# kahrendt/microWakeWord

Measured on AMD Instinct MI355X. Metric: spectrogram-windows/sec (train step) on default mixednet, higher is better.
Workload: dtype f32

## Files before the change

microwakeword_amd/csrc/block_engine.hip:

```cpp
#define MWW_BLOCK_TU 1
#include <cstring>

#include "engine.hip.h"
#include "block_launch.hip.h"
#include "kernels_bnre.hip.h"

#ifndef MWW_CONV1_X6_DEFAULT
#define MWW_CONV1_X6_DEFAULT 1
#endif
#ifndef MWW_CONV1_X6_FWD_DEFAULT
#define MWW_CONV1_X6_FWD_DEFAULT 0
#endif
#ifndef MWW_BWD_FIRST_WIDE_DEFAULT
#define MWW_BWD_FIRST_WIDE_DEFAULT 0
#endif
#ifndef MWW_BWD_WIDE_DEFAULT
#define MWW_BWD_WIDE_DEFAULT 1
#endif
#ifndef MWW_DP_COMMIT_LATE_BLOCK_DEFAULT
#define MWW_DP_COMMIT_LATE_BLOCK_DEFAULT 1
#endif
#ifndef MWW_DP_COMMIT_LATE_LAST_DEFAULT
#define MWW_DP_COMMIT_LATE_LAST_DEFAULT 0
#endif
#ifndef MWW_DP_COMMIT_LATE_FIRST_DEFAULT
#define MWW_DP_COMMIT_LATE_FIRST_DEFAULT 1
#endif

namespace mww {

__global__ void bn_fwd_finalize_kernel(BnFwdFinalizeArgs a);
__global__ void bn_eval_prepare_kernel(BnEvalPrepareArgs a);
__global__ void bn_bwd_finalize_kernel(BnBwdFinalizeArgs a);

namespace {

float* bn_slot(Layer& l, int i) { return l.bn + (size_t)i * l.cout; }
float b_inv_n(const Layer& l, int B) { return 1.0f / ((float)B * (float)l.tout); }
bool b_handover(const mww_ctx* c) { return c->bn_inline && !(c->hook && c->sync_bn); }

struct BlockModel : Model {
  mww_mixednet_desc d;
  std::vector<Layer> L;
  int64_t o_conv1 = 0;
  int grid_fwd = 0, grid_bwd = 0;
  float* a0 = nullptr;
  float* gbuf[2] = {nullptr, nullptr};
  bool conv1_x6 = MWW_CONV1_X6_DEFAULT != 0;
  bool conv1_x6_fwd = MWW_CONV1_X6_FWD_DEFAULT != 0;
  bool bwd_first_wide = MWW_BWD_FIRST_WIDE_DEFAULT != 0;
  bool bwd_wide = MWW_BWD_WIDE_DEFAULT != 0;
  int dp_commit_late = -1;
  bool pw_bf16 = false;
  bool st_bf16 = false;
  int ablate = 0;
  unsigned long long* phase_clk = nullptr;

  ~BlockModel() override {
    for (Layer& l : L) {
      if (gbuf[0] || gbuf[1]) l.g = nullptr;
      tensor_free(&l);
    }
    void* own[] = {gbuf[0], gbuf[1], a0, phase_clk};
    for (void* p : own) if (p) (void)hipFree(p);
  }
  int layout(mww_ctx* c) override;
  int alloc(mww_ctx* c, std::vector<BnSlots>* bn) override;
  int enqueue_forward(mww_ctx* c, int B, bool training, bool update_moving, bool loss, bool metrics) override;
  int enqueue_backward(mww_ctx* c, int B, bool fuse_adam) override;
  int enqueue_bn_collect(mww_ctx* c, int B) override;
  std::vector<int> stat_widths() const override {
    std::vector<int> w;
    for (const Layer& l : L) w.push_back(l.cout);
    return w;
  }
  bool lazy_ok(const mww_ctx*, int B) const override {
    const int per_fwd = (B + std::min(B, grid_fwd) - 1) / std::min(B, grid_fwd);
    const int per_bwd = (B + std::min(B, grid_bwd) - 1) / std::min(B, grid_bwd);
    return per_fwd <= kXMaxSamples && per_bwd <= kXMaxSamples;
  }
  unsigned replay_key(bool* handover) const override { *handover = true; return 0; }
  bool eval_fold_cached() const override { return true; }
  int debug_tensor(mww_ctx* c, const char* name, int B, DebugTensor* t) override;
  int set_option(mww_ctx* c, const OptionRow& o, int64_t v) override;

  int launch_fwd_first(mww_ctx* c, int k1, int c1, int cout, int k, int st, const FwdFirstArgs& a, int grid);
  int launch_bwd_first(mww_ctx* c, int k1, int c1, int cout, int k, int st, const BwdFirstArgs& a, int grid);
  int launch_fwd_block(mww_ctx* c, int cin, int cout, int k, const FwdBlockArgs& a, int grid);
  int launch_bwd_block(mww_ctx* c, int cin, int cout, int k, bool last, const BwdBlockArgs& a, int grid);
  int fwd_block_grid(const mww_ctx* c, const Layer& l, int B);
  void block_segments(int gbwd, int b0, int b1, GradReduceArgs* ga);
};

int BlockModel::launch_fwd_first(mww_ctx* c, int k1, int c1, int cout, int k, int st, const FwdFirstArgs& a, int grid) {
  if (k_launch_fwd_first(c->stream, st_bf16 ? 2 : (pw_bf16 ? 1 : 0), k1, c1, cout, k, st, a, grid, conv1_x6_fwd)) return MWW_OK;
  return fail(MWW_ERR_UNSUPPORTED, "no first-block kernel for this (conv1 kernel, filters, pointwise, depthwise) shape");
}

int BlockModel::launch_bwd_first(mww_ctx* c, int k1, int c1, int cout, int k, int st, const BwdFirstArgs& a, int grid) {
  const bool late = dp_commit_late < 0 ? MWW_DP_COMMIT_LATE_FIRST_DEFAULT != 0 : dp_commit_late != 0;
  if (bwd_wide && !pw_bf16 && !st_bf16 && k_launch_bwd_firstw(c->stream, k1, c1, cout, k, st, a, grid, conv1_x6 && bwd_first_wide, late)) return MWW_OK;
  if (k_launch_bwd_first(c->stream, st_bf16 ? 2 : (pw_bf16 ? 1 : 0), k1, c1, cout, k, st, a, grid, conv1_x6, late)) return MWW_OK;
  return fail(MWW_ERR_UNSUPPORTED, "no first-block backward kernel for this shape");
}

int BlockModel::launch_fwd_block(mww_ctx* c, int cin, int cout, int k, const FwdBlockArgs& a, int grid) {
  if (k_launch_fwd_block(c->stream, st_bf16 ? 2 : (pw_bf16 ? 1 : 0), cin, cout, k, a, grid)) return MWW_OK;
  return fail(MWW_ERR_UNSUPPORTED, "no block kernel for this (cin, cout, depthwise) shape");
}

int BlockModel::launch_bwd_block(mww_ctx* c, int cin, int cout, int k, bool last, const BwdBlockArgs& a, int grid) {
  const int mode = st_bf16 ? 2 : (pw_bf16 ? 1 : 0);
  const bool late = dp_commit_late < 0 ? (last ? MWW_DP_COMMIT_LATE_LAST_DEFAULT : MWW_DP_COMMIT_LATE_BLOCK_DEFAULT) != 0 : dp_commit_late != 0;
  if (bwd_wide && k_launch_bwd_blockw(c->stream, mode, cin, cout, k, last, a, grid, late)) return MWW_OK;
  if (k_launch_bwd_block(c->stream, st_bf16 ? 2 : (pw_bf16 ? 1 : 0), cin, cout, k, last, a, grid)) return MWW_OK;
  return fail(MWW_ERR_UNSUPPORTED, "no block backward kernel for this shape");
}

}

bool shape_supported(const mww_mixednet_desc& d, std::string* why, bool bf16) {
  if (d.n_blocks < 2 || d.n_blocks > MWW_MAX_BLOCKS) { *why = "the block kernels serve 2.." + std::to_string(MWW_MAX_BLOCKS) + " blocks"; return false; }
  bool ok = false;
#define X(K1, C1, CO, K, S) ok = ok || (d.conv1_kernel == K1 && d.conv1_filters == C1 && d.block_filters[0] == CO && d.block_kernel[0] == K && d.conv1_stride == S);
  if (bf16) { MWW_FIRST_SHAPES_BF16(X) } else { MWW_FIRST_SHAPES(X) }
#undef X
  if (!ok) { *why = "first block (conv1 kernel/filters/stride, pointwise filters, depthwise kernel) not instantiated"; return false; }
  for (int i = 1; i < d.n_blocks; ++i) {
    ok = false;
#define X(CI, CO, K) ok = ok || (d.block_filters[i - 1] == CI && d.block_filters[i] == CO && d.block_kernel[i] == K);
    if (bf16) { MWW_BLOCK_SHAPES_BF16(X) } else { MWW_BLOCK_SHAPES(X) }
#undef X
    if (!ok) { *why = "block " + std::to_string(i) + " (cin, cout, depthwise kernel) not instantiated"; return false; }
  }
  const int cl = d.block_filters[d.n_blocks - 1];
  if (cl != 32 && cl != 48 && cl != 64) { *why = "head kernel needs 32, 48 or 64 channels"; return false; }
  int t = d.frames >= d.conv1_kernel && d.conv1_stride > 0 ? (d.frames - d.conv1_kernel) / d.conv1_stride + 1 : 0;
  for (int i = 0; i < d.n_blocks; ++i) t -= d.block_kernel[i] - 1;
  if (t > head_frame_limit(cl)) {
    *why = "head kernel holds at most " + std::to_string(head_frame_limit(cl)) + " final frames at " + std::to_string(cl) + " channels (" + std::to_string(t) + " here)";
    return false;
  }
  return true;
}

namespace {

int BlockModel::fwd_block_grid(const mww_ctx* c, const Layer& l, int B) {
  const int per_cu = l.cin > 48 ? 2 : (l.k > 13 ? 3 : 4);
  const long long items = (long long)B * ((l.tout + TT - 1) / TT);
  return (int)std::min<long long>(items, std::min(grid_fwd, c->n_cu * per_cu));
}

int BlockModel::enqueue_forward(mww_ctx* c, int B, bool training, bool update_moving, bool loss, bool metrics) {
  Launcher lp{c};
  const int nb = d.n_blocks;
  if (!training && !c->bn_eval_ready) {
    for (int i = 0; i < nb; ++i) {
      Layer& l = L[i];
      BnEvalPrepareArgs a{fwd_params(c) + l.o_gamma, fwd_params(c) + l.o_beta, eval_bn_state(c) + l.o_mm, eval_bn_state(c) + l.o_mv,
                          bn_slot(l, BN_SCALE), bn_slot(l, BN_SHIFT), l.cout};
      lp.begin("bn_eval_prepare", i);
      hipLaunchKernelGGL(bn_eval_prepare_kernel, dim3(1), dim3(64), 0, c->stream, a);
      lp.end();
    }
  }
  const bool inl = training && b_handover(c);
  auto fold_of = [&](Layer& pl) {
    BnFoldArgs f;
    memset(&f, 0, sizeof(f));
    if (!inl) return f;
    f.acc = fwd_rows(c, pl).acc;
    f.inv_n = b_inv_n(pl, B);
    f.update_moving = update_moving ? 1 : 0;
    f.gamma = fwd_params(c) + pl.o_gamma;
    f.beta = fwd_params(c) + pl.o_beta;
    f.moving_mean = c->bn_state + pl.o_mm;
    f.moving_var = c->bn_state + pl.o_mv;
    f.scale = bn_slot(pl, BN_SCALE);
    f.shift = bn_slot(pl, BN_SHIFT);
    f.mean = bn_slot(pl, BN_MEAN);
    f.rstd = bn_slot(pl, BN_RSTD);
    return f;
  };
  for (int i = 0; i < nb; ++i) {
    Layer& l = L[i];
    const int grid = i == 0 ? std::min(B, grid_fwd) : fwd_block_grid(c, l, B);
    const StatAcc sacc = inl ? fwd_rows(c, l) : StatAcc{nullptr, nullptr};
    if (i == 0) {
      FwdFirstArgs a{c->x, fwd_params(c) + o_conv1, fwd_params(c) + l.o_dw_w, fwd_params(c) + l.o_dw_b, fwd_params(c) + l.o_pw_w,
                     l.p, l.stat_part, B, d.frames, l.tout, 0, sacc, x_gather(c), training ? a0 : nullptr};
      lp.begin("fwd_block", i);
      int rc = launch_fwd_first(c, d.conv1_kernel, d.conv1_filters, l.cout, l.k, d.conv1_stride, a, grid);
      lp.end();
      if (rc) return rc;
    } else {
      Layer& pl = L[i - 1];
      FwdBlockArgs a{pl.p, bn_slot(pl, BN_SCALE), bn_slot(pl, BN_SHIFT), fwd_params(c) + l.o_dw_w, fwd_params(c) + l.o_dw_b,
                     fwd_params(c) + l.o_pw_w, l.p, l.stat_part, B, l.tin, l.tout, ablate, phase_clk + (size_t)(2 * i) * 2048 * kClkSlots,
                     sacc, fold_of(pl)};
      lp.begin("fwd_block", i);
      int rc = launch_fwd_block(c, l.cin, l.cout, l.k, a, grid);
      lp.end();
      if (rc) return rc;
    }
    if (training && !inl) {
      StatSource ss;
      int rcs = exchange_stats(c, lp, "bn_stat_exchange", i, l.stat_part, grid, l.cout, 0, b_inv_n(l, B), &ss);
      if (rcs) return rcs;
      BnFwdFinalizeArgs f{ss.part, ss.G, l.cout, ss.inv_n, fwd_params(c) + l.o_gamma,
                          fwd_params(c) + l.o_beta, c->bn_state + l.o_mm, c->bn_state + l.o_mv, bn_slot(l, BN_SCALE),
                          bn_slot(l, BN_SHIFT), bn_slot(l, BN_MEAN), bn_slot(l, BN_RSTD), update_moving ? 1 : 0};
      lp.begin("bn_fwd_finalize", i);
      hipLaunchKernelGGL(bn_fwd_finalize_kernel, dim3(l.cout), dim3(kThreads), 0, c->stream, f);
      lp.end();
    }
  }
  Layer& ll = L[nb - 1];
  const BnFoldArgs hfold = fold_of(ll);
  if (inl) c->fpar ^= 1;
  const bool tail_late = loss && inl && c->tail_roles;
  const StatAcc hgacc = tail_late ? bwd_rows(c, ll) : StatAcc{nullptr, nullptr};
  int rc = enqueue_block_head(c, B, ll, ll.tout, ll.cout, st_bf16, hfold, hgacc, loss, metrics);
  if (rc) return rc;
  c->tail_src = DenseSource{ll.p, bn_slot(ll, BN_SCALE), bn_slot(ll, BN_SHIFT), nullptr, nullptr, nullptr, nullptr, 0, 0, st_bf16 ? 1 : 0};
  if (tail_late) {
    c->tail_in_reduce = true;
    c->tail_metrics = metrics;
    return MWW_OK;
  }
  if (loss && !(c->hook && c->sync_bn)) {
    c->tail_pending = true;
    c->tail_metrics = metrics;
    return MWW_OK;
  }
  return enqueue_side_work(c, B, metrics, loss, c->tail_src);
}

int BlockModel::enqueue_bn_collect(mww_ctx* c, int B) {
  const bool inl = b_handover(c);
  std::vector<BnreRow> rows(L.size());
  memset(rows.data(), 0, rows.size() * sizeof(BnreRow));
  for (size_t i = 0; i < L.size(); ++i) {
    Layer& l = L[i];
    BnreRow& r = rows[i];
    const float inv_n = b_inv_n(l, B);
    r.C = l.cout;
    r.groups = 1;
    r.o_mm = (int)l.o_mm;
    r.o_mv = (int)l.o_mv;
    if (inl) {
      r.form = BNRE_ROWS;
      r.acc[0] = l.facc[0];
      r.acc[1] = l.facc[1];
      r.inv_n = inv_n;
    } else {
      const int grid = i == 0 ? std::min(B, grid_fwd) : fwd_block_grid(c, l, B);
      const StatSource ss = forward_stat_source(c, (int)i, l.stat_part, grid, l.cout, inv_n);
      r.form = BNRE_PART_BLOCK;
      r.part = ss.part;
      r.G = ss.G;
      r.inv_n = ss.inv_n;
    }
  }
  return enqueue_bnre_collect(c, rows);
}

void BlockModel::block_segments(int gbwd, int b0, int b1, GradReduceArgs* ga) {
  memset(ga, 0, sizeof(*ga));
  for (int i = b0; i < b1; ++i) {
    Layer& l = L[i];
    GradSegment s;
    s.part = l.grad_part;
    s.G = gbwd;
    s.stride = l.grad_part_stride;
    s.n = l.grad_part_stride;
    s.dst = (int)(i == 0 ? o_conv1 : l.o_dw_w);
    ga->seg[ga->nseg++] = s;
  }
}

int BlockModel::enqueue_backward(mww_ctx* c, int B, bool fuse_adam) {
  Launcher lp{c};
  const int nb = d.n_blocks;
  const int gbwd = std::min(B, grid_bwd);
  const int ghead = std::min(B, c->grid_head);
  const bool inl = b_handover(c);
  const int split = nb >= 3 ? nb - 2 : 0;
  const bool bucketed = fuse_adam && c->hook && c->reduce_grads && !c->sync_bn && inl && c->tail_in_reduce && c->grad_buckets == 2 && split > 0;
  for (int i = nb - 1; i >= 0; --i) {
    Layer& l = L[i];
    const bool last = (i == nb - 1);
    const bool fold_here = inl && (!last || c->tail_in_reduce);
    StatSource ss{nullptr, 0, 0.f, 1.0f};
    if (!fold_here) {
      int rcs = exchange_stats(c, lp, "bn_gstat_exchange", i, l.gstat_part, last ? ghead : gbwd, l.cout, 1, b_inv_n(l, B), &ss);
      if (rcs) return rcs;
    }
    BnBwdFinalizeArgs f{ss.part, ss.G, l.cout, ss.inv_n,
                        fwd_params(c) + l.o_gamma, bn_slot(l, BN_RSTD), bn_slot(l, BN_C1), bn_slot(l, BN_MG),
                        bn_slot(l, BN_MGX), c->grads + l.o_gamma, c->grads + l.o_beta, ss.dscale};
    BnGradFoldArgs gf;
    memset(&gf, 0, sizeof(gf));
    if (fold_here) {
      gf.acc = bwd_rows(c, l).acc;
      gf.inv_n = b_inv_n(l, B);
      gf.dscale = 1.0f;
      gf.gamma = fwd_params(c) + l.o_gamma;
      gf.c1 = bn_slot(l, BN_C1);
      gf.mg = bn_slot(l, BN_MG);
      gf.mgx = bn_slot(l, BN_MGX);
      gf.dgamma = c->grads + l.o_gamma;
      gf.dbeta = c->grads + l.o_beta;
    }
    if (fold_here) {
    } else if (last && c->tail_pending) {
      c->tail_pending = false;
      int rch = enqueue_head_tail(c, B, f);
      if (rch) return rch;
    } else {
      lp.begin("bn_bwd_finalize", i);
      hipLaunchKernelGGL(bn_bwd_finalize_kernel, dim3(l.cout), dim3(kThreads), 0, c->stream, f);
      lp.end();
    }
    if (i > 0) {
      Layer& pl = L[i - 1];
      BwdBlockArgs a;
      a.in = pl.p;
      a.in_scale = bn_slot(pl, BN_SCALE);
      a.in_shift = bn_slot(pl, BN_SHIFT);
      a.in_mean = bn_slot(pl, BN_MEAN);
      a.in_rstd = bn_slot(pl, BN_RSTD);
      a.pk = l.p;
      a.gk = l.g;
      a.k_mean = bn_slot(l, BN_MEAN);
      a.k_rstd = bn_slot(l, BN_RSTD);
      a.k_c1 = bn_slot(l, BN_C1);
      a.k_mg = bn_slot(l, BN_MG);
      a.k_mgx = bn_slot(l, BN_MGX);
      a.k_scale = bn_slot(l, BN_SCALE);
      a.k_shift = bn_slot(l, BN_SHIFT);
      a.wd = fwd_params(c) + c->o_dense_w;
      a.dz = c->dz;
      a.dw_w = fwd_params(c) + l.o_dw_w;
      a.dw_b = fwd_params(c) + l.o_dw_b;
      a.pw_w = fwd_params(c) + l.o_pw_w;
      a.g_out = pl.g;
      a.gstat_part = pl.gstat_part;
      a.grad_part = l.grad_part;
      a.B = B;
      a.Tin = l.tin;
      a.Tout = l.tout;
      a.ablate = ablate;
      a.phase_clk = phase_clk + (size_t)(2 * i + 1) * 2048 * kClkSlots;
      a.gacc = inl ? bwd_rows(c, pl) : StatAcc{nullptr, nullptr};
      a.gfold = gf;
      lp.begin("bwd_block", i);
      int rc = launch_bwd_block(c, l.cin, l.cout, l.k, last, a, gbwd);
      lp.end();
      if (rc) return rc;
      if (bucketed && i == split) {
        GradReduceArgs gb;
        block_segments(gbwd, split, nb, &gb);
        rc = enqueue_grad_assembly(c, B, gb, fuse_adam, l.o_dw_w, c->P, false);
        if (rc) return rc;
      }
    } else {
      if (last) return fail(MWW_ERR_UNSUPPORTED, "single-block models are not supported");
      BwdFirstArgs a{c->x, a0, l.p, l.g, bn_slot(l, BN_MEAN), bn_slot(l, BN_RSTD), bn_slot(l, BN_C1),
                     bn_slot(l, BN_MG), bn_slot(l, BN_MGX), fwd_params(c) + l.o_dw_w, fwd_params(c) + l.o_dw_b,
                     fwd_params(c) + l.o_pw_w, l.grad_part, B, d.frames, l.tout, gf, x_gather(c), ablate,
                     phase_clk + (size_t)(2 * i + 1) * 2048 * kClkSlots};
      lp.begin("bwd_block", i);
      int rc = launch_bwd_first(c, d.conv1_kernel, d.conv1_filters, l.cout, l.k, d.conv1_stride, a, gbwd);
      lp.end();
      if (rc) return rc;
    }
  }
  if (inl) c->gpar ^= 1;
  GradReduceArgs ga;
  block_segments(gbwd, 0, bucketed ? split : nb, &ga);
  return enqueue_grad_assembly(c, B, ga, fuse_adam, 0, bucketed ? L[split].o_dw_w : c->P, true);
}

int BlockModel::layout(mww_ctx* c) {
  int64_t off = 0, soff = 0;
  o_conv1 = off;
  off += (int64_t)d.conv1_kernel * MWW_FEATURE_BINS * d.conv1_filters;
  int t = (d.frames - d.conv1_kernel) / d.conv1_stride + 1, ch = d.conv1_filters;
  L.resize(d.n_blocks);
  for (int i = 0; i < d.n_blocks; ++i) {
    Layer& l = L[i];
    l.cin = ch;
    l.cout = d.block_filters[i];
    l.k = d.block_kernel[i];
    l.tin = t;
    l.tout = t - (l.k - 1);
    if (l.tout <= 0) return fail(MWW_ERR_INVALID, "spectrogram too short for the kernel sizes");
    l.o_dw_w = off; off += (int64_t)l.k * l.cin;
    l.o_dw_b = off; off += l.cin;
    l.o_pw_w = off; off += (int64_t)l.cin * l.cout;
    l.o_gamma = off; off += l.cout;
    l.o_beta = off; off += l.cout;
    l.o_mm = soff; soff += l.cout;
    l.o_mv = soff; soff += l.cout;
    t = l.tout;
    ch = l.cout;
  }
  c->t_last = t;
  c->c_last = ch;
  c->o_dense_w = off; off += (int64_t)t * ch;
  c->o_dense_b = off; off += 1;
  c->P = off;
  c->S = soff;
  c->dwd_stride = t * ch + 4;
  grid_fwd = c->n_cu * 4;
  grid_bwd = c->n_cu * 2;
  bool wide64 = false;
  for (int i = 0; i < d.n_blocks; ++i) wide64 = wide64 || d.block_filters[i] > 48;
  if (wide64) {
    grid_fwd = c->n_cu * 2;
    grid_bwd = c->n_cu;
  }
  return MWW_OK;
}

int BlockModel::alloc(mww_ctx* c, std::vector<BnSlots>* bn) {
  const size_t mb = (size_t)d.max_batch;
  const int gmax_f = c->n_cu * 4, gmax_b = c->n_cu * 2;
  MWW_TRY(dev_alloc(&a0, mb * L[0].tin * d.conv1_filters));
#ifndef MWW_G_PINGPONG
#define MWW_G_PINGPONG 1
#endif
  if (MWW_G_PINGPONG) {
    size_t need[2] = {0, 0};
    for (int i = 0; i < d.n_blocks; ++i) need[i & 1] = std::max(need[i & 1], mb * L[i].tout * L[i].cout);
    for (int par = 0; par < 2; ++par)
      if (need[par]) MWW_TRY(dev_alloc(&gbuf[par], need[par]));
  }
  for (int i = 0; i < d.n_blocks; ++i) {
    Layer& l = L[i];
    MWW_TRY(dev_alloc(&l.p, mb * l.tout * l.cout));
    if (MWW_G_PINGPONG) l.g = gbuf[i & 1];
    else MWW_TRY(dev_alloc(&l.g, mb * l.tout * l.cout));
    l.grad_part_stride = (l.k + 1) * l.cin + l.cin * l.cout;
    if (i == 0) l.grad_part_stride += d.conv1_kernel * MWW_FEATURE_BINS * d.conv1_filters;
    MWW_TRY(tensor_alloc(&l, l.cout, gmax_f, std::max(gmax_b, c->n_cu * 4), (size_t)gmax_b * l.grad_part_stride));
    bn->push_back(BnSlots{l.o_gamma, l.o_beta, l.o_mv, l.cout});
  }
  MWW_TRY(dev_alloc(&phase_clk, (size_t)2 * MWW_MAX_BLOCKS * 2048 * kClkSlots));
  return MWW_OK;
}

int BlockModel::set_option(mww_ctx* c, const OptionRow& o, int64_t v) {
  if (o.owner != OPT_BLOCK) return MWW_OK;
  const std::string name = o.name;
  if (name == "pointwise_bf16" || name == "storage_bf16") {
    std::string why;
    if (v && !shape_supported(d, &why, true)) return fail(MWW_ERR_UNSUPPORTED, "no bf16 mode for this topology: " + why);
    if (name == "pointwise_bf16") { pw_bf16 = v != 0; if (!v) st_bf16 = false; }
    else { st_bf16 = v != 0; if (v) pw_bf16 = true; }
  }
  const std::pair<const char*, bool BlockModel::*> flags[] = {{"bwd_wide", &BlockModel::bwd_wide}, {"conv1_x6", &BlockModel::conv1_x6},
                                                              {"conv1_x6_fwd", &BlockModel::conv1_x6_fwd}, {"bwd_first_wide", &BlockModel::bwd_first_wide}};
  const std::pair<const char*, int BlockModel::*> ints[] = {{"ablate", &BlockModel::ablate}, {"dp_commit_late", &BlockModel::dp_commit_late},
                                                            {"grid_fwd", &BlockModel::grid_fwd}, {"grid_bwd", &BlockModel::grid_bwd}};
  for (auto& f : flags) if (name == f.first) this->*f.second = v != 0;
  for (auto& f : ints) if (name == f.first) this->*f.second = (int)v;
  return MWW_OK;
}

int BlockModel::debug_tensor(mww_ctx* c, const char* name, int B, DebugTensor* t) {
  const int nb = d.n_blocks;
  auto idx = [&](const char* prefix) -> int {
    const size_t pl = strlen(prefix);
    if (strncmp(name, prefix, pl) != 0) return -1;
    const int k = atoi(name + pl);
    return (k >= 1 && k <= nb && name[pl] >= '0' && name[pl] <= '9') ? k - 1 : -1;
  };
  int k;
  if ((k = idx("p")) >= 0 || (k = idx("g")) >= 0) {
    t->src = name[0] == 'p' ? L[k].p : L[k].g;
    t->n = (int64_t)B * L[k].tout * L[k].cout;
    t->bf16 = st_bf16;
  }
  else if ((k = idx("bn")) >= 0) { t->src = L[k].bn; t->n = (int64_t)9 * L[k].cout; }
  else if (!strcmp(name, "a0")) { t->src = a0; t->n = (int64_t)B * L[0].tin * d.conv1_filters; }
  else if (!strncmp(name, "clkf", 4) || !strncmp(name, "clkb", 4)) {
    const int kk = atoi(name + 4);
    if (kk < 1 || kk > nb) return fail(MWW_ERR_INVALID, "bad layer");
    t->src = reinterpret_cast<const float*>(phase_clk + (size_t)(2 * (kk - 1) + (name[3] == 'b' ? 1 : 0)) * 2048 * kClkSlots);
    t->n = 2048 * kClkSlots * 2;
  }
  else return 0;
  return 1;
}

}

int plan_mixednet(const mww_mixednet_desc& d, Model** out) {
  if (d.n_blocks < 2 || d.n_blocks > MWW_MAX_BLOCKS) return fail(MWW_ERR_INVALID, "n_blocks must be in [2, 8]");
  if (d.conv1_stride < 1 || d.frames < d.conv1_kernel) return fail(MWW_ERR_INVALID, "bad first-conv stride / kernel");
  if (d.conv1_filters <= 0) return fail(MWW_ERR_UNSUPPORTED, "first_conv_filters == 0 is not implemented");
  if (d.max_batch <= 0 || d.frames <= 0) return fail(MWW_ERR_INVALID, "frames and max_batch must be positive");
  std::string why;
  if (!shape_supported(d, &why)) return fail(MWW_ERR_UNSUPPORTED, why);
  BlockModel* m = new BlockModel();
  m->d = d;
  *out = m;
  return MWW_OK;
}

}
```

microwakeword_amd/csrc/bwd_first_body.inc:

```
  constexpr int CIN = C1;
  constexpr int CPI = pitch(CIN), CPO = pitch(COUT);
  constexpr int RA = TT + K - 1;
  constexpr int TAIL = S > 1 ? K - 1 : 0;
  constexpr int TAILK = (TAIL + 3) / 4 * 4;
  constexpr int XR = (TT + TAILK - 1) * S + K1;
  constexpr int NT1 = C1 / 16;
  constexpr int M1 = K1 * FBINS;
  constexpr int MT1 = (M1 + 15) / 16;
  constexpr int MPW = (MT1 + 3) / 4;
  constexpr int MT = CIN / 16, NT = COUT / 16, KSO = COUT / 4;
  constexpr int NCH = nchunks(CIN), L = chunk_len(CIN);
  constexpr int QI = CIN / 4;
  constexpr int RAP = halo_rows_padded(CIN, K), TTP = tile_rows_padded(CIN);
  constexpr int OFF_A = 0, OFF_DP = OFF_A + RAP * CPI, OFF_U = OFF_DP + TT * CPO, OFF_DU = OFF_U + TTP * CPI;
  constexpr int PB = 96, PLB = XR * PB, GPB = 2 * CIN, GPL = TT * GPB;
  static_assert(!X6 || (S == 1 && CIN == 32 && (K1 * FBINS) % 8 == 0 && 3 * GPL <= (TT * CPO + TTP * CPI) * 4 && TTP == TT), "the x6 form serves the stride-1 first convolutions");
  constexpr int OFF_G0 = OFF_DU + RAP * CPI, OFF_END = X6 ? OFF_G0 : OFF_G0 + (TTP + TAILK) * CPI;
  static_assert(TAIL <= NCH && TTP + TAIL <= RAP, "tail rows");
  constexpr int PX = FBINS + 1;
  static_assert(OFF_END >= 4 * CIN * COUT && OFF_END >= NCH * (K + 1) * CIN, "scratch aliasing");
  static_assert(TT >= K - 1, "shape");

  float* sA = smem + OFF_A;
  float* sDP = smem + OFF_DP;
  float* sU = smem + OFF_U;
  float* sDU = smem + OFF_DU;
  float* sG0 = smem + OFF_G0;

  const int tid = threadIdx.x, lane = tid & 63, wave = tid >> 6, r16 = lane & 15, g = lane >> 4;
  const int c = tid % CIN, chunk = tid / CIN;
  const bool dw_active = chunk < NCH;
  const int Ta = (a.T - K1) / S + 1;
  MWW_PC_DECL
  MWW_PC_AT(0);

  const bool tailmode = TAIL > 0 && Ta > TT && Ta <= TT + TAIL;
  const int ntiles = tailmode ? 1 : (Ta + TT - 1) / TT;
  const int nsamp = (int)blockIdx.x < a.B ? (a.B - (int)blockIdx.x + (int)gridDim.x - 1) / (int)gridDim.x : 0;
  const int nitems = nsamp * ntiles;
  XStage<XR, PX, MWW_AUX_LD_XB> xs;
  DpStage<COUT, false, SB> dps;
  constexpr int NA = (RA * QI + kThreads - 1) / kThreads;
  float4 pre_a[NA];
  auto issue_a = [&](int it, bool live) {
    const int s = live ? it / ntiles : nsamp - 1, b = blockIdx.x + s * gridDim.x, t0 = (it % ntiles) * TT;
    const int nrx = live ? ((tailmode ? Ta : min(TT, Ta - t0)) - 1) * S + K1 : 0;
    xs.issue(a.x, a.xg, sXg, s, b, a.T, t0 * S, nrx, tid);
    const BufRsrc ra = tile_rsrc(a.a0 + ((size_t)b * Ta + t0) * CIN, live ? min(RA, Ta - t0) * QI * 16 : 0);
#pragma unroll
    for (int j = 0; j < NA; ++j) pre_a[j] = tile_load4<MWW_AUX_LD_A0>(ra, (tid + j * kThreads) * 16);
  };
  auto issue_b = [&](int it, bool live) {
    const int b = blockIdx.x + (it / ntiles) * gridDim.x, t0 = (it % ntiles) * TT;
    const int nvk = live ? max(0, min(TT, a.Tout - t0)) * (COUT / 4) : 0;
    const size_t koff = ((size_t)b * a.Tout + t0) * COUT;
    dps.issue(elem_ptr<SB>(a.pk, koff), elem_ptr<SB>(a.gk, koff), nvk, tid);
  };
  int offm[MPW];
  bool okm[MPW];
  int xoff[MPW], goff[NT1];
  if constexpr (X6) {
    const int rowl = 4 * g + (r16 >> 2), cg = 4 * (r16 & 3);
#pragma unroll
    for (int mi = 0; mi < MPW; ++mi) {
      const int m = min((wave * MPW + mi) * 16 + cg, M1 - 4);
      xoff[mi] = (rowl + m / FBINS) * PB + (m % FBINS) * 2;
    }
#pragma unroll
    for (int nt = 0; nt < NT1; ++nt) goff[nt] = rowl * GPB + ((nt * 16 + cg) ^ ((rowl & 4) ? 16 : 0)) * 2;
  } else {
#pragma unroll
  for (int mi = 0; mi < MPW; ++mi) {
    const int m = (wave * MPW + mi) * 16 + r16;
    okm[mi] = m < M1;
    offm[mi] = okm[mi] ? (m / FBINS) * PX + (m % FBINS) : 0;
  }
  }
  if (a.xg.win) xgather_setup(a.xg, sXg, nsamp, tid);
  stagger_start<MWW_STAGGER_BWD>();
  if (nitems > 0) {
    issue_a(0, true);
    issue_b(0, true);
  }

  WeightStage<CIN, COUT, 0, pitch_wt(CIN, BF)> wst;
  wst.load(a.pw_w, nullptr, tid);
  float dww[K], accw[K];
  float accb = 0.f, dwb = 0.f;
#pragma unroll
  for (int i = 0; i < K; ++i) {
    dww[i] = dw_active ? a.dw_w[i * CIN + c] : 0.f;
    accw[i] = 0.f;
  }
  if (dw_active) dwb = a.dw_b[c];
  for (int i = tid; i < COUT; i += kThreads) {
    const float krs = a.k_rstd[i];
    const float kmean = a.k_mean[i];
    float c1, mg, mgx;
    if (a.gfold.acc) {
      bn_grad_fold_channel(a.gfold, COUT, i, krs, c1, mg, mgx);
    } else {
      c1 = a.k_c1[i];
      mg = a.k_mg[i];
      mgx = a.k_mgx[i];
    }
    const float kA = -c1 * krs * mgx;
    sKp[0 * COUT + i] = c1;
    sKp[1 * COUT + i] = kA;
    sKp[2 * COUT + i] = -c1 * mg - kA * kmean;
    sKp[5 * COUT + i] = 0.f;
    sKp[6 * COUT + i] = 0.f;
  }
  wst.store(sWt, nullptr, tid);
  for (int i = RA * CPI + tid; i < RAP * CPI; i += kThreads) {
    sA[i] = 0.f;
    sDU[i] = 0.f;
  }
  if constexpr (!X6)
    for (int i = TTP * CPI + tid; i < (TTP + TAILK) * CPI; i += kThreads) sG0[i] = 0.f;
#pragma unroll
  for (int i = 0; i < K; ++i) pin(dww[i]);
  pin(dwb);
  f32x4 dwacc[MT][NT];
#pragma unroll
  for (int mt = 0; mt < MT; ++mt)
#pragma unroll
    for (int nt = 0; nt < NT; ++nt) dwacc[mt][nt] = zero4();
  f32x4 w1acc[MPW][NT1];
#pragma unroll
  for (int mi = 0; mi < MPW; ++mi)
#pragma unroll
    for (int nt = 0; nt < NT1; ++nt) w1acc[mi][nt] = zero4();
  __syncthreads();

  MWW_PC_AT(1);
  MWW_PC_START(MWW_ABLATE(a, 16) && tid == 0);
  for (int it = 0; it < nitems; ++it) {
    rotate_priority(it, 2);
    const int t0 = (it % ntiles) * TT;
    const int nrows_new = max(0, min(TT, a.Tout - t0));
    const int rows_da = min(TT, Ta - t0);
    if constexpr (X6) xs.template commit_planes<PB, PLB>(reinterpret_cast<unsigned*>(sX), a.xg, sXg, it / ntiles, t0 * S, tid);
    else xs.commit(sX, a.xg, sXg, it / ntiles, t0 * S, tid);
#pragma unroll
    for (int j = 0; j < NA; ++j) {
      const int i = tid + j * kThreads;
      if (i < RA * QI) {
        const int r = i / QI, q = i - r * QI;
        *reinterpret_cast<float4*>(sA + r * CPI + q * 4) = pre_a[j];
      }
    }
    MWW_PC_MARK(0);
    if constexpr (!LATE) dps.commit(sDP, sKp, 0.f, nrows_new * (COUT / 4), tid);
    carry_du<K, CPI>(sDU, t0 == 0, tid);
    if constexpr (LATE) issue_a(it + 1, it + 1 < nitems);
    MWW_PC_MARK(LATE ? 0 : 8);
    __syncthreads();
    MWW_PC_MARK(1);
    if constexpr (!LATE) {
      if (it + 1 < nitems) {
        issue_a(it + 1, true);
        issue_b(it + 1, true);
      }
    }
    if (dw_active) {
      if (chunk * L < nrows_new) {
        float o[L];
        dw_chunk<K, L>(sA, CPI, chunk * L, c, dww, dwb, o);
#pragma unroll
        for (int t = 0; t < L; ++t) {
          const int tl = chunk * L + t;
          sU[tl * CPI + c] = (tl < nrows_new) ? o[t] : 0.f;
        }
      } else {
#pragma unroll
        for (int t = 0; t < L; ++t) sU[(chunk * L + t) * CPI + c] = 0.f;
      }
    }
    MWW_PC_MARK(2);
    if constexpr (LATE) {
      dps.commit(sDP, sKp, 0.f, nrows_new * (COUT / 4), tid);
      issue_b(it + 1, it + 1 < nitems);
      MWW_PC_MARK(8);
    }
    __syncthreads();
    MWW_PC_MARK(3);
    pointwise_backward_tile<CIN, COUT, K, BF>(sU, sDP, sDU, wave, r16, g, sWt, dwacc, wave * 16 < nrows_new);
    MWW_PC_MARK(4);
    __syncthreads();
    MWW_PC_MARK(5);
    if (dw_active) {
      float wdu[L + K - 1], wa[L + K - 1];
#pragma unroll
      for (int j = 0; j < L + K - 1; ++j) wdu[j] = sDU[(chunk * L + j) * CPI + c];
#pragma unroll
      for (int j = 0; j < L + K - 1; ++j) wa[j] = sA[(chunk * L + j) * CPI + c];
      lds_reads_first();
#pragma unroll
      for (int t = 0; t < L; ++t) {
        const int sl = chunk * L + t;
        float acc = 0.f;
#pragma unroll
        for (int i = 0; i < K; ++i) acc = fmaf(dww[K - 1 - i], wdu[t + i], acc);
        const float gv = (sl < rows_da && wa[t] > 0.f) ? acc : 0.f;
        if constexpr (X6) {
          unsigned h0, h1, h2;
          split3(gv, h0, h1, h2);
          unsigned short* gp = reinterpret_cast<unsigned short*>(sDP) + sl * CIN + (c ^ ((sl & 4) ? 16 : 0));
          gp[0] = (unsigned short)(h0 >> 16);
          gp[GPL / 2] = (unsigned short)(h1 >> 16);
          gp[GPL] = (unsigned short)(h2 >> 16);
        } else {
          sG0[sl * CPI + c] = gv;
        }
      }
      if (chunk * L < nrows_new) {
#pragma unroll
        for (int t = 0; t < L; ++t) {
          const float dut = wdu[K - 1 + t];
          accb += dut;
#pragma unroll
          for (int i = 0; i < K; ++i) accw[i] = fmaf(dut, wa[t + i], accw[i]);
        }
      }
      if constexpr (TAIL > 0) {
        if (tailmode && chunk < TAIL) {
          const int sl = TT + chunk;
          float acc = 0.f;
#pragma unroll
          for (int j = 0; j < K; ++j) acc = fmaf(dww[K - 1 - j], sl + j < RAP ? sDU[(sl + j) * CPI + c] : 0.f, acc);
          sG0[sl * CPI + c] = (sl < Ta && sA[sl * CPI + c] > 0.f) ? acc : 0.f;
        }
      }
    }
    MWW_PC_MARK(6);
    __syncthreads();
    if constexpr (X6) {
      const char* xb = reinterpret_cast<const char*>(sX);
      const char* gb = reinterpret_cast<const char*>(sDP);
#pragma unroll
      for (int kb = 0; kb < TT / 32; ++kb)
#pragma unroll
        for (int nt = 0; nt < NT1; ++nt) {
          u32x4v gq[3];
#pragma unroll
          for (int p = 0; p < 3; ++p) {
            const u32x2v lo = lds_read_tr16(gb + goff[nt] + p * GPL + (32 * kb) * GPB), hi = lds_read_tr16(gb + goff[nt] + p * GPL + (32 * kb + 16) * GPB);
            gq[p] = u32x4v{lo.x, lo.y, hi.x, hi.y};
          }
#pragma unroll
          for (int mi = 0; mi < MPW; ++mi) {
            u32x4v xq[3];
#pragma unroll
            for (int p = 0; p < 3; ++p) {
              const u32x2v lo = lds_read_tr16(xb + xoff[mi] + p * PLB + (32 * kb) * S * PB), hi = lds_read_tr16(xb + xoff[mi] + p * PLB + (32 * kb + 16) * S * PB);
              xq[p] = u32x4v{lo.x, lo.y, hi.x, hi.y};
            }
            w1acc[mi][nt] = mfma_x6(xq, gq, w1acc[mi][nt]);
          }
        }
    } else {
      float av[2][MPW], bv[2][NT1];
      auto load_w1 = [&](int kk, int sl) {
        const int s = kk * 4 + g;
#pragma unroll
        for (int nt = 0; nt < NT1; ++nt) bv[sl][nt] = sG0[s * CPI + nt * 16 + r16];
#pragma unroll
        for (int mi = 0; mi < MPW; ++mi) {
          const float v = sX[s * S * PX + offm[mi]];
          av[sl][mi] = okm[mi] ? v : 0.f;
        }
      };
      load_w1(0, 0);
#pragma unroll
      for (int kk = 0; kk < TT / 4; ++kk) {
        if (kk + 1 < TT / 4) load_w1(kk + 1, (kk + 1) & 1);
#pragma unroll
        for (int mi = 0; mi < MPW; ++mi)
#pragma unroll
          for (int nt = 0; nt < NT1; ++nt) w1acc[mi][nt] = mfma4(av[kk & 1][mi], bv[kk & 1][nt], w1acc[mi][nt]);
      }
      __builtin_amdgcn_sched_group_barrier(0x100, MPW + NT1, 0);
      sched_read_mfma_groups<TT / 4 - 1, MPW + NT1, MPW * NT1>();
      sched_read_mfma_groups<1, 0, MPW * NT1>();
      if constexpr (TAIL > 0) {
        if (tailmode) {
#pragma unroll
          for (int ks = 0; ks < TAILK / 4; ++ks) {
            load_w1(TT / 4 + ks, 0);
#pragma unroll
            for (int mi = 0; mi < MPW; ++mi)
#pragma unroll
              for (int nt = 0; nt < NT1; ++nt) w1acc[mi][nt] = mfma4(av[0][mi], bv[0][nt], w1acc[mi][nt]);
          }
        }
      }
    }
    MWW_PC_MARK(7);
    __syncthreads();
    MWW_PC_MARK(5);
  }
  MWW_PC_AT(2);
  float* gdst = a.grad_part + (size_t)blockIdx.x * (M1 * C1 + (K + 1) * CIN + CIN * COUT);
#pragma unroll
  for (int mi = 0; mi < MPW; ++mi)
#pragma unroll
    for (int nt = 0; nt < NT1; ++nt)
#pragma unroll
      for (int r = 0; r < 4; ++r) {
        const int m = (wave * MPW + mi) * 16 + g * 4 + r;
        if (m < M1) gdst[m * C1 + nt * 16 + r16] = w1acc[mi][nt][r];
      }
  write_block_grad_partials<CIN, COUT, K>(smem, gdst + M1 * C1, dwacc, accw, accb, dw_active, c, chunk, tid, wave, r16, g);
  MWW_PC_AT(3);
  MWW_PC_DUMP(a.phase_clk ? a.phase_clk + (size_t)blockIdx.x * kClkSlots : nullptr);
```

microwakeword_amd/csrc/common.hip.h:

```cpp
#pragma once
#include <hip/hip_runtime.h>
#include <stdint.h>

namespace mww {

typedef float f32x4 __attribute__((ext_vector_type(4)));

constexpr int kThreads = 256;
constexpr int TT = 64;
constexpr int FBINS = 40;
constexpr float kBnEps = 1e-3f;
constexpr float kBnMomentum = 0.99f;
constexpr float kKerasEps = 1e-7f;

constexpr int kHeadTraining = 1, kHeadClippedLoss = 2;
__device__ __forceinline__ float bce_value(float z, float pr, float yy, bool clipped_form) {
  if (!clipped_form) return fmaxf(z, 0.f) - z * yy + log1pf(expf(-fabsf(z)));
  const float pc = fminf(fmaxf(pr, kKerasEps), 1.0f - kKerasEps);
  return -(yy * logf(pc) + (1.0f - yy) * logf(1.0f - pc));
}
__device__ __forceinline__ float bce_dz(float pr, float yy, bool clipped_form) {
  if (clipped_form && ((pr < kKerasEps) || (pr > 1.0f - kKerasEps))) return 0.f;
  return pr - yy;
}

__device__ __forceinline__ f32x4 mfma4(float a, float b, f32x4 c) {
  return __builtin_amdgcn_mfma_f32_16x16x4f32(a, b, c, 0, 0, 0);
}

typedef __bf16 bf16x4 __attribute__((ext_vector_type(4)));
typedef short s16x4 __attribute__((ext_vector_type(4)));

__device__ __forceinline__ f32x4 mfma_bf16(bf16x4 a, bf16x4 b, f32x4 c) {
  return __builtin_amdgcn_mfma_f32_16x16x16bf16_1k(__builtin_bit_cast(s16x4, a), __builtin_bit_cast(s16x4, b), c, 0, 0, 0);
}

__device__ __forceinline__ bf16x4 to_bf16x4(float a, float b, float c, float d) {
  bf16x4 v = {(__bf16)a, (__bf16)b, (__bf16)c, (__bf16)d};
  return v;
}

typedef __bf16 bf16x8 __attribute__((ext_vector_type(8)));
typedef unsigned u32x4v __attribute__((ext_vector_type(4)));
typedef unsigned u32x2v __attribute__((ext_vector_type(2)));
__device__ __forceinline__ f32x4 mfma_bf16k32(u32x4v a, u32x4v b, f32x4 c) {
  return __builtin_amdgcn_mfma_f32_16x16x32_bf16(__builtin_bit_cast(bf16x8, a), __builtin_bit_cast(bf16x8, b), c, 0, 0, 0);
}
__device__ __forceinline__ void split3(float v, unsigned& h0, unsigned& h1, unsigned& h2) {
  h0 = __float_as_uint(v) & 0xffff0000u;
  const float r1 = v - __uint_as_float(h0);
  h1 = __float_as_uint(r1) & 0xffff0000u;
  const float r2 = r1 - __uint_as_float(h1);
  h2 = __float_as_uint(r2) & 0xffff0000u;
}
__device__ __forceinline__ unsigned pack_hi2(unsigned a, unsigned b) { return (a >> 16) | b; }
__device__ __forceinline__ void split3x8(const float (&v)[8], u32x4v (&q)[3]) {
  unsigned h[3][8];
#pragma unroll
  for (int e = 0; e < 8; ++e) split3(v[e], h[0][e], h[1][e], h[2][e]);
#pragma unroll
  for (int p = 0; p < 3; ++p)
#pragma unroll
    for (int d = 0; d < 4; ++d) q[p][d] = pack_hi2(h[p][2 * d], h[p][2 * d + 1]);
}
__device__ __forceinline__ f32x4 mfma_x6(const u32x4v (&xs)[3], const u32x4v (&ws)[3], f32x4 acc) {
  acc = mfma_bf16k32(xs[2], ws[0], acc);
  acc = mfma_bf16k32(xs[1], ws[1], acc);
  acc = mfma_bf16k32(xs[0], ws[2], acc);
  acc = mfma_bf16k32(xs[1], ws[0], acc);
  acc = mfma_bf16k32(xs[0], ws[1], acc);
  acc = mfma_bf16k32(xs[0], ws[0], acc);
  return acc;
}
__device__ __forceinline__ void pin4(u32x4v& v) { asm volatile("" : "+v"(v)); }
__device__ __forceinline__ u32x2v lds_read_tr16(const void* lds_ptr) {
  typedef short s16x4t __attribute__((ext_vector_type(4)));
  const s16x4t v = __builtin_amdgcn_ds_read_tr16_b64_v4i16((__attribute__((address_space(3))) s16x4t*)(lds_ptr));
  return __builtin_bit_cast(u32x2v, v);
}

__device__ __forceinline__ f32x4 zero4() {
  f32x4 z = {0.f, 0.f, 0.f, 0.f};
  return z;
}

__host__ __device__ constexpr int pitch(int c) { return c + 4; }
#ifndef MWW_FWD_PITCH_A
#define MWW_FWD_PITCH_A 1
#endif
#ifndef MWW_FWD_PITCH_U
#define MWW_FWD_PITCH_U 1
#endif
__host__ __device__ constexpr int pitch_fa(int c) { return (MWW_FWD_PITCH_A && c == 48) ? 48 : c + 4; }
__host__ __device__ constexpr int pitch_fu(int c, bool bf) { return (MWW_FWD_PITCH_U && !bf) ? c + 2 : c + 4; }

__host__ __device__ constexpr int pitch_wt(int c, bool bf) { return bf ? c + 4 : (c % 32 == 16 ? c : c + 16); }

__host__ __device__ constexpr int nchunks(int c) { return kThreads / c; }
__host__ __device__ constexpr int chunk_len(int c) { return (TT + nchunks(c) - 1) / nchunks(c); }
__host__ __device__ constexpr int tile_rows_padded(int c) { return nchunks(c) * chunk_len(c); }
__host__ __device__ constexpr int halo_rows_padded(int c, int k) { return tile_rows_padded(c) + k - 1; }

typedef __amdgpu_buffer_rsrc_t BufRsrc;
typedef unsigned u32x4 __attribute__((ext_vector_type(4)));
typedef unsigned u32x2 __attribute__((ext_vector_type(2)));

__device__ __forceinline__ BufRsrc tile_rsrc(const void* base, int bytes) {
  const int n = __builtin_amdgcn_readfirstlane(bytes > 0 ? bytes : 0);
  return __builtin_amdgcn_make_buffer_rsrc(const_cast<void*>(base), (short)0, n, 0x00020000);
}
#ifndef MWW_AUX_ST_P
#define MWW_AUX_ST_P 16
#endif
#ifndef MWW_AUX_ST_G
#define MWW_AUX_ST_G 16
#endif
#ifndef MWW_AUX_ST_A0
#define MWW_AUX_ST_A0 2
#endif
#ifndef MWW_AUX_LD_FP
#define MWW_AUX_LD_FP 0
#endif
#ifndef MWW_AUX_LD_BP
#define MWW_AUX_LD_BP 2
#endif
#ifndef MWW_AUX_LD_A0
#define MWW_AUX_LD_A0 2
#endif
#ifndef MWW_AUX_LD_PK
#define MWW_AUX_LD_PK 2
#endif
#ifndef MWW_AUX_LD_GK
#define MWW_AUX_LD_GK 2
#endif
#ifndef MWW_AUX_LD_XF
#define MWW_AUX_LD_XF 0
#endif
#ifndef MWW_AUX_LD_XB
#define MWW_AUX_LD_XB 0
#endif
#ifndef MWW_AUX_LD_HP
#define MWW_AUX_LD_HP 0
#endif
#ifndef MWW_AUX_ST_GP
#define MWW_AUX_ST_GP 1
#endif
#ifndef MWW_AUX_GR_ST_P
#define MWW_AUX_GR_ST_P 1
#endif
#ifndef MWW_AUX_GR_ST_G
#define MWW_AUX_GR_ST_G 0
#endif
#ifndef MWW_AUX_GR_LD_GOLD
#define MWW_AUX_GR_LD_GOLD 0
#endif
#ifndef MWW_AUX_GR_ST_GP
#define MWW_AUX_GR_ST_GP 0
#endif
#ifndef MWW_AUX_GR_LD_DP
#define MWW_AUX_GR_LD_DP 0
#endif
template <int WT>
__device__ __forceinline__ void store_stream(float* p, float v) {
  if constexpr (WT != 0) __hip_atomic_store(p, v, __ATOMIC_RELAXED, __HIP_MEMORY_SCOPE_AGENT);
  else *p = v;
}
template <int AUX = 0>
__device__ __forceinline__ float4 tile_load4(BufRsrc r, int byte_off) {
  const u32x4 v = __builtin_amdgcn_raw_buffer_load_b128(r, byte_off, 0, AUX);
  return make_float4(__uint_as_float(v.x), __uint_as_float(v.y), __uint_as_float(v.z), __uint_as_float(v.w));
}
template <int AUX = 0>
__device__ __forceinline__ uint2 tile_load2(BufRsrc r, int byte_off) {
  const u32x2 v = __builtin_amdgcn_raw_buffer_load_b64(r, byte_off, 0, AUX);
  uint2 o;
  o.x = v.x;
  o.y = v.y;
  return o;
}
template <int AUX = 0>
__device__ __forceinline__ float tile_load1(BufRsrc r, int byte_off) {
  return __uint_as_float(__builtin_amdgcn_raw_buffer_load_b32(r, byte_off, 0, AUX));
}
template <int AUX = 0>
__device__ __forceinline__ void tile_store1(BufRsrc r, int byte_off, float v) {
  __builtin_amdgcn_raw_buffer_store_b32(__float_as_uint(v), r, byte_off, 0, AUX);
}
template <bool SB, int AUX = 0>
__device__ __forceinline__ float4 tile_load4s(BufRsrc r, int group) {
  if constexpr (!SB) {
    return tile_load4<AUX>(r, group * 16);
  } else {
    const uint2 v = tile_load2<AUX>(r, group * 8);
    return make_float4(__uint_as_float(v.x << 16), __uint_as_float(v.x & 0xffff0000u), __uint_as_float(v.y << 16),
                       __uint_as_float(v.y & 0xffff0000u));
  }
}
template <bool SB, int AUX = 0>
__device__ __forceinline__ void tile_store1s(BufRsrc r, int elem, float v) {
  if constexpr (!SB) {
    tile_store1<AUX>(r, elem * 4, v);
  } else {
    const __bf16 h = (__bf16)v;
    __builtin_amdgcn_raw_buffer_store_b16(__builtin_bit_cast(unsigned short, h), r, elem * 2, 0, AUX);
  }
}
template <bool SB>
__device__ __forceinline__ float load_elem(const float* base, size_t elem) {
  if constexpr (!SB) {
    return base[elem];
  } else {
    const unsigned dw = reinterpret_cast<const unsigned*>(base)[elem >> 1];
    return __uint_as_float((elem & 1) ? (dw & 0xffff0000u) : (dw << 16));
  }
}
__host__ __device__ constexpr int elem_bytes(bool sb) { return sb ? 2 : 4; }
template <bool SB>
__device__ __forceinline__ const float* elem_ptr(const float* base, size_t elem) {
  return reinterpret_cast<const float*>(reinterpret_cast<const char*>(base) + elem * (SB ? 2 : 4));
}
template <bool SB>
__device__ __forceinline__ float* elem_ptr(float* base, size_t elem) {
  return reinterpret_cast<float*>(reinterpret_cast<char*>(base) + elem * (SB ? 2 : 4));
}

constexpr int kOobOffset = 0x40000000;

__device__ __forceinline__ void lds_reads_first() {
  __builtin_amdgcn_sched_group_barrier(0x100, 64, 0);
  __builtin_amdgcn_sched_group_barrier(0x002, 2048, 0);
}

__device__ __forceinline__ void rotate_priority(int item, int levels) {
  const int p = ((int)(blockIdx.x >> 8) + item) & (levels - 1);
  if (levels == 2) {
    if (p) __builtin_amdgcn_s_setprio(1);
    else __builtin_amdgcn_s_setprio(0);
  } else {
    if (p == 0) __builtin_amdgcn_s_setprio(0);
    else if (p == 1) __builtin_amdgcn_s_setprio(1);
    else if (p == 2) __builtin_amdgcn_s_setprio(2);
    else __builtin_amdgcn_s_setprio(3);
  }
}

#ifndef MWW_STAGGER_BWD
#define MWW_STAGGER_BWD 47
#endif
#ifndef MWW_STAGGER_FWD
#define MWW_STAGGER_FWD 0
#endif
#ifndef MWW_STAGGER_GRAPH
#define MWW_STAGGER_GRAPH 0
#endif
#ifndef MWW_G_FWD_DIRECT
#define MWW_G_FWD_DIRECT 1
#endif
#ifndef MWW_G_WGRAD_EVEN
#define MWW_G_WGRAD_EVEN 1
#endif
#ifndef MWW_G_STEM_BREG
#define MWW_G_STEM_BREG 0
#endif
#ifndef MWW_G_WGRAD_XG_NARROW
#define MWW_G_WGRAD_XG_NARROW 0
#endif
template <int UNITS>
__device__ __forceinline__ void stagger_start() {
  if constexpr (UNITS > 0) {
    const int pos = (int)(blockIdx.x >> 8);
    for (int i = 0; i < pos; ++i) __builtin_amdgcn_s_sleep(UNITS);
  }
}

__device__ __forceinline__ void pin(float& v) { asm volatile("" : "+v"(v)); }
__device__ __forceinline__ void pin(int& v) { asm volatile("" : "+v"(v)); }

#ifdef MWW_PROFILE
#define MWW_ABLATE(a, bits) ((a).ablate & (bits))
#else
#define MWW_ABLATE(a, bits) 0
#endif
#ifdef MWW_PROFILE
#define MWW_PC_DECL PhaseClock pc;
#define MWW_PC_START(en) pc.start(en)
#define MWW_PC_MARK(i) pc.mark(i)
#define MWW_PC_DUMP(p) do { if (p) pc.dump(p); } while (0)
#define MWW_PC_AT(i) pc.at(i)
#else
#define MWW_PC_AT(i) ((void)0)
#define MWW_PC_DECL
#define MWW_PC_START(en) ((void)0)
#define MWW_PC_MARK(i) ((void)0)
#define MWW_PC_DUMP(p) ((void)0)
#endif
constexpr int kClkPhases = 9;
constexpr int kClkSlots = kClkPhases + 4;
struct PhaseClock {
  unsigned long long last = 0, acc[kClkPhases] = {0, 0, 0, 0, 0, 0, 0, 0, 0}, stamp[4] = {0, 0, 0, 0};
  bool on = false;
  __device__ __forceinline__ void at(int i) { stamp[i] = __builtin_amdgcn_s_memtime(); }
  __device__ __forceinline__ void start(bool enable) {
    on = enable;
    if (on) last = __builtin_amdgcn_s_memtime();
  }
  __device__ __forceinline__ void mark(int slot) {
    if (on) {
      const unsigned long long t = __builtin_amdgcn_s_memtime();
      acc[slot] += t - last;
      last = t;
    }
  }
  __device__ __forceinline__ void dump(unsigned long long* dst) const {
    if (on) {
      for (int i = 0; i < kClkPhases; ++i) dst[i] = acc[i];
      for (int i = 0; i < 4; ++i) dst[kClkPhases + i] = stamp[i];
    }
  }
};

__device__ __forceinline__ void fast_divmod(int a, int b, int& q, int& r) {
  q = (int)((float)a * __frcp_rn((float)b));
  r = a - q * b;
  if (r >= b) {
    ++q;
    r -= b;
  } else if (r < 0) {
    --q;
    r += b;
  }
}
__device__ __forceinline__ int fast_div(int a, int b) {
  int q, r;
  fast_divmod(a, b, q, r);
  return q;
}

__device__ __forceinline__ int uniform_int(int v) { return __builtin_amdgcn_readfirstlane(v); }
__device__ __forceinline__ long long uniform_i64(long long v) {
  const unsigned lo = (unsigned)__builtin_amdgcn_readfirstlane((int)(unsigned)(unsigned long long)v);
  const unsigned hi = (unsigned)__builtin_amdgcn_readfirstlane((int)(unsigned)((unsigned long long)v >> 32));
  return (long long)(((unsigned long long)hi << 32) | lo);
}
__device__ __forceinline__ const void* uniform_ptr(const void* p) {
  return reinterpret_cast<const void*>((uintptr_t)uniform_i64((long long)(uintptr_t)p));
}

__device__ __forceinline__ float sum_over_groups(float v) {
  v += __shfl_xor(v, 16);
  v += __shfl_xor(v, 32);
  return v;
}

__device__ __forceinline__ float wave_sum(float v) {
  v += __shfl_xor(v, 1);
  v += __shfl_xor(v, 2);
  v += __shfl_xor(v, 4);
  v += __shfl_xor(v, 8);
  v += __shfl_xor(v, 16);
  v += __shfl_xor(v, 32);
  return v;
}

constexpr int kStatRows = 8;

struct StatAcc {
  double* acc;
  double* clear;
};

__device__ __forceinline__ void publish_stat(const StatAcc& s, float* row, int C2, int tid, float v) {
  if (s.acc) {
    unsafeAtomicAdd(s.acc + (size_t)(blockIdx.x % kStatRows) * C2 + tid, (double)v);
    for (int r = blockIdx.x; r < kStatRows; r += gridDim.x)
      __hip_atomic_store(s.clear + (size_t)r * C2 + tid, 0.0, __ATOMIC_RELAXED, __HIP_MEMORY_SCOPE_AGENT);
  } else {
    row[tid] = v;
  }
}

struct BnFoldArgs {
  const double* acc;
  float inv_n;
  int update_moving;
  const float* gamma;
  const float* beta;
  float* moving_mean;
  float* moving_var;
  float* scale;
  float* shift;
  float* mean;
  float* rstd;
};

__device__ __forceinline__ void bn_fold_channel(const BnFoldArgs& f, int C, int ch, float& sc, float& sh, float& meanf, float& rstd) {
  double s1 = 0.0, s2 = 0.0;
  double v1[kStatRows], v2[kStatRows];
#pragma unroll
  for (int j = 0; j < kStatRows; ++j) {
    v1[j] = f.acc[(size_t)j * 2 * C + ch];
    v2[j] = f.acc[(size_t)j * 2 * C + C + ch];
  }
  const float gam = f.gamma[ch], bet = f.beta[ch];
  float mm_old = 0.f, mv_old = 0.f;
  if (blockIdx.x == 0 && f.update_moving) {
    mm_old = f.moving_mean[ch];
    mv_old = f.moving_var[ch];
  }
#pragma unroll
  for (int j = 0; j < kStatRows; ++j) {
    s1 += v1[j];
    s2 += v2[j];
  }
  const double m = s1 * (double)f.inv_n;
  double var = s2 * (double)f.inv_n - m * m;
  if (var < 0.0) var = 0.0;
  meanf = (float)m;
  const float varf = (float)var;
  rstd = 1.0f / sqrtf(varf + kBnEps);
  sc = gam * rstd;
  sh = bet - meanf * sc;
  if (blockIdx.x == 0) {
    f.scale[ch] = sc;
    f.shift[ch] = sh;
    f.mean[ch] = meanf;
    f.rstd[ch] = rstd;
    if (f.update_moving) {
      f.moving_mean[ch] = mm_old * kBnMomentum + meanf * (1.0f - kBnMomentum);
      f.moving_var[ch] = mv_old * kBnMomentum + varf * (1.0f - kBnMomentum);
    }
  }
}

struct BnGradFoldArgs {
  const double* acc;
  float inv_n;
  float dscale;
  const float* gamma;
  float* c1;
  float* mg;
  float* mgx;
  float* dgamma;
  float* dbeta;
};

__device__ __forceinline__ void bn_grad_fold_channel(const BnGradFoldArgs& f, int C, int ch, float rstd, float& c1, float& mg, float& mgx) {
  double s1 = 0.0, s2 = 0.0;
  double v1[kStatRows], v2[kStatRows];
#pragma unroll
  for (int j = 0; j < kStatRows; ++j) {
    v1[j] = f.acc[(size_t)j * 2 * C + ch];
    v2[j] = f.acc[(size_t)j * 2 * C + C + ch];
  }
  const float gam = f.gamma[ch];
#pragma unroll
  for (int j = 0; j < kStatRows; ++j) {
    s1 += v1[j];
    s2 += v2[j];
  }
  c1 = gam * rstd;
  mg = (float)(s1 * (double)f.inv_n);
  mgx = (float)(s2 * (double)f.inv_n);
  if (blockIdx.x == 0) {
    f.dbeta[ch] = (float)s1 * f.dscale;
    f.dgamma[ch] = (float)s2 * f.dscale;
    f.c1[ch] = c1;
    f.mg[ch] = mg;
    f.mgx[ch] = mgx;
  }
}

}
```

microwakeword_amd/csrc/engine.hip.h:

```cpp
#pragma once
#include <hip/hip_runtime.h>

#include <map>
#include <string>
#include <utility>
#include <vector>

#include "../../include/mww.h"
#include "kernels_bwd.hip.h"
#include "kernels_data.hip.h"

namespace mww {

struct MetricState;
struct BnreRow;

int fail(int code, const std::string& msg);

#define HIPCHK(expr)                                                                              \
  do {                                                                                            \
    hipError_t e_ = (expr);                                                                       \
    if (e_ != hipSuccess)                                                                         \
      return fail(MWW_ERR_HIP, std::string(#expr) + ": " + hipGetErrorString(e_));                \
  } while (0)
#define MWW_TRY(call)                                                                             \
  do {                                                                                            \
    int rc_ = (call);                                                                             \
    if (rc_) return rc_;                                                                          \
  } while (0)

struct Tensor {
  float* p = nullptr;
  float* g = nullptr;
  float* stat_part = nullptr;
  float* gstat_part = nullptr;
  float* grad_part = nullptr;
  float* bn = nullptr;
  double* facc[2] = {nullptr, nullptr};
  double* gacc[2] = {nullptr, nullptr};
};
int tensor_alloc(Tensor* t, int cout, size_t rows_fwd, size_t rows_bwd, size_t grad_part);
void tensor_free(Tensor* t);

struct Layer : Tensor {
  int cin, cout, k, tin, tout;
  int64_t o_dw_w, o_dw_b, o_pw_w, o_gamma, o_beta, o_mm, o_mv;
  int grad_part_stride = 0;
};

struct GOp : Tensor {
  int n_src = 0, src[MWW_MAX_OP_SOURCES] = {0, 0, 0}, toff[MWW_MAX_OP_SOURCES] = {0, 0, 0};
  int sc0[MWW_MAX_OP_SOURCES] = {0, 0, 0}, scn[MWW_MAX_OP_SOURCES] = {0, 0, 0};
  bool src_first[MWW_MAX_OP_SOURCES] = {false, false, false}, src_last[MWW_MAX_OP_SOURCES] = {false, false, false};
  int k = 1, dil = 1, cin = 0, cout = 0, groups = 1, slots = 0, tin = 0, tout = 0;
  int kind = MWW_OP_CONV, stride = 1, norm = MWW_NORM_BN, act = MWW_ACT_RELU;
  int res_src = -1, res_drop = 0;
  std::vector<int> adders;
  int64_t o_w = 0, o_gamma = 0, o_beta = 0, o_mm = 0, o_mv = 0;
  bool needs_dx = false;
  bool twin_next = false;
  int planes = 1, pc = 0;
  size_t lds_fwd = 0, lds_dx = 0, lds_wg = 0;
  int first_consumer = -1;
};

struct ProfileEntry {
  std::string name;
  hipEvent_t a, b;
};

struct RcclApi {
  void* so = nullptr;
  struct UniqueId { char internal[128]; };
  int (*GetUniqueId)(UniqueId*) = nullptr;
  int (*CommInitRank)(void**, int, UniqueId, int) = nullptr;
  int (*AllReduce)(const void*, void*, size_t, int, int, void*, hipStream_t) = nullptr;
  int (*CommDestroy)(void*) = nullptr;
  int (*CommCount)(void*, int*) = nullptr;
  const char* (*GetErrorString)(int) = nullptr;
};

constexpr int kRing = 8;
constexpr int kDenseChunks = 32;

struct DenseSource {
  const float *p = nullptr, *scale = nullptr, *shift = nullptr, *keep = nullptr, *rp = nullptr, *rscale = nullptr, *rshift = nullptr;
  int rT = 0, rdrop = 0, bf16 = 0;
};

enum OptionOwner { OPT_CORE, OPT_BLOCK, OPT_GRAPH };
struct OptionRow { const char* name; OptionOwner owner; int64_t lo, hi; int hi_cu; const char* range_error; };

struct DebugTensor { const float* src = nullptr; int64_t n = 0; bool bf16 = false; int planes = 1, pc = 0, cout = 0; long long pstride = 0; };

struct BnSlots { int64_t o_gamma, o_beta, o_mv; int n; };

struct Model {
  Model() = default;
  Model(const Model&) = delete;
  virtual ~Model() {}
  virtual int layout(mww_ctx* c) = 0;
  virtual int alloc(mww_ctx* c, std::vector<BnSlots>* bn) = 0;
  virtual int enqueue_forward(mww_ctx* c, int B, bool training, bool update_moving, bool loss, bool metrics) = 0;
  virtual int enqueue_backward(mww_ctx* c, int B, bool fuse_adam) = 0;
  virtual int enqueue_bn_collect(mww_ctx* c, int B) = 0;
  virtual std::vector<int> stat_widths() const = 0;
  virtual bool lazy_ok(const mww_ctx* c, int B) const = 0;
  virtual bool step_counter(unsigned long long* n) { return false; }
  virtual unsigned replay_key(bool* handover) const = 0;
  virtual bool eval_fold_cached() const { return false; }
  virtual int debug_tensor(mww_ctx* c, const char* name, int B, DebugTensor* t) = 0;
  virtual int set_option(mww_ctx* c, const OptionRow& o, int64_t v) = 0;
  virtual int set_dropout_mask(mww_ctx* c, const uint8_t* keep, int B);
};

}

struct mww_ctx {
  mww::Model* model = nullptr;
  int frames = 0, max_batch = 0;
  int device = 0;
  hipStream_t stream = nullptr;
  bool own_stream = false;
  int n_cu = 256;
  int grid_head = 0;
  int64_t P = 0, S = 0;
  int64_t o_dense_w = 0, o_dense_b = 0;
  int t_last = 0, c_last = 0, dwd_stride = 0;
  int metric_launches = 0;
  mww_allreduce_fn hook = nullptr;
  void* hook_user = nullptr;
  int world = 1;
  bool sync_bn = false, reduce_grads = false;
  struct RcclState* rccl = nullptr;
  float* sync_buf = nullptr;
  std::vector<int64_t> sync_off;
  float *params = nullptr, *grads = nullptr, *adam_m = nullptr, *adam_v = nullptr, *mask = nullptr;
  bool weight_qat = false;
  const float* shadow_held = nullptr;
  float* shadow = nullptr;
  int *qat_start = nullptr, *qat_elem = nullptr, *qat_copy = nullptr;
  int qat_channels = 0, qat_n_copy = 0;
  float* ema = nullptr;
  double ema_decay = 0.0;
  int64_t ema_every = 1, ema_updates = 0;
  bool ema_forward = false, ema_src = false;
  float* ema_bn = nullptr;
  bool ema_bn_valid = false;
  double* bnre_acc = nullptr;
  int64_t bnre_batches = -1;
  mww::BnreRow* bnre_table = nullptr;
  int bnre_table_rows = 0;
  std::vector<char> bnre_table_host;
  double sam_rho = 0.0, clip_norm = 0.0;
  float* sam_w = nullptr;
  double* norm_scalars = nullptr;
  bool norms_valid = false;
  unsigned char* direct = nullptr;
  std::vector<unsigned char> direct_host;
  bool exchange_pending = false;
  int grad_buckets = 1;
  float* bn_state = nullptr;
  float *x = nullptr, *y = nullptr, *sw = nullptr, *z = nullptr, *prob = nullptr, *dz = nullptr, *loss_part = nullptr;
  float* dwd_part = nullptr;
  mww::MetricState* metrics = nullptr;
  char* mail_host[mww::kRing] = {};
  char* mail_dev[mww::kRing] = {};
  hipEvent_t mail_ev[mww::kRing] = {};
  int mail_cur = 0;
  bool mail_open = false;
  size_t mail_off_masks = 0, mail_off_y = 0, mail_off_sw = 0, mail_off_hyper = 0, mail_bytes = 0;
  int targets_in_mail = 0;
  hipStream_t copy_stream = nullptr;
  char* mail_hbm[mww::kRing] = {};
  hipEvent_t ev_copy[mww::kRing] = {};
  hipStream_t side = nullptr;
  hipEvent_t ev_fork = nullptr, ev_join = nullptr;
  bool side_pending = false;
  int asm_split = 2;
  bool fused_input = true;
  bool x_lazy = false;
  int lazy_slot = -1;
  mww::AssembleArgs lazy_a;
  const float* y_cur = nullptr;
  const float* sw_cur = nullptr;
  bool bn_inline = true;
  int fpar = 0, gpar = 0;
  bool tail_pending = false, tail_metrics = false;
  bool tail_in_reduce = false;
  mww::DenseSource tail_src;
  bool tail_roles = true;
  void* store[MWW_MAX_STORES] = {};
  int store_dtype[MWW_MAX_STORES] = {};
  int64_t store_elems[MWW_MAX_STORES] = {};
  int64_t step = 0;
  int have_batch = 0, have_targets = 0;
  bool use_graphs = false, profile = false;
  bool use_side = false;
  bool bce_clipped = false;
  bool bn_eval_ready = false;
  std::vector<mww::ProfileEntry> prof;
  struct GraphEntry { int B, flags, mail; unsigned core, model; hipGraphExec_t exec; };
  std::vector<GraphEntry> graphs;
};

namespace mww {

struct Launcher {
  mww_ctx* c;
  hipEvent_t ea = nullptr;
  const char* name = nullptr;
  size_t idx = 0;
  void begin(const char* n, int layer = -1) {
    if (!c->profile) return;
    name = n;
    idx = c->prof.size();
    ProfileEntry e;
    e.name = n;
    if (layer >= 0) e.name += std::to_string(layer + 1);
    (void)hipEventCreate(&e.a);
    (void)hipEventCreate(&e.b);
    (void)hipEventRecord(e.a, c->stream);
    c->prof.push_back(e);
  }
  void end() {
    if (!c->profile || idx >= c->prof.size()) return;
    (void)hipEventRecord(c->prof[idx].b, c->stream);
  }
  void cancel() {
    if (!c->profile) return;
    (void)hipEventDestroy(c->prof.back().a);
    (void)hipEventDestroy(c->prof.back().b);
    c->prof.pop_back();
  }
};

enum { BN_SCALE = 0, BN_SHIFT, BN_MEAN, BN_RSTD, BN_C1, BN_MG, BN_MGX };

inline StatAcc fwd_rows(const mww_ctx* c, const Tensor& t) { return StatAcc{t.facc[c->fpar], t.facc[c->fpar ^ 1]}; }
inline StatAcc bwd_rows(const mww_ctx* c, const Tensor& t) { return StatAcc{t.gacc[c->gpar], t.gacc[c->gpar ^ 1]}; }

inline float* fwd_source(const mww_ctx* c) { return c->ema_src ? c->ema : c->params; }
inline float* fwd_params(const mww_ctx* c) { return c->weight_qat ? c->shadow : fwd_source(c); }
inline float* eval_bn_state(const mww_ctx* c) { return (c->ema_src && c->ema_bn_valid) ? c->ema_bn : c->bn_state; }

template <typename T>
int dev_alloc(T** p, size_t n) {
  HIPCHK(hipMalloc((void**)p, std::max<size_t>(n, 1) * sizeof(T)));
  HIPCHK(hipMemset(*p, 0, std::max<size_t>(n, 1) * sizeof(T)));
  return MWW_OK;
}
int create_context(Model* m, int frames, int max_batch, int device, void* stream, mww_ctx** out);
const float* mail_hyper(mww_ctx* c);
int materialise_x(mww_ctx* c);
XGather x_gather(mww_ctx* c);
int enqueue_side_work(mww_ctx* c, int B, bool metrics, bool loss, const DenseSource& last);
struct StatSource { const float* part; int G; float inv_n; float dscale; };
int exchange_stats(mww_ctx* c, Launcher& lp, const char* what, int layer, const float* part, int G, int C, int bwd, float local_inv_n, StatSource* out);
StatSource forward_stat_source(const mww_ctx* c, int layer, const float* part, int G, int C, float local_inv_n);
int enqueue_bnre_collect(mww_ctx* c, std::vector<BnreRow>& rows);
int enqueue_grad_assembly(mww_ctx* c, int B, GradReduceArgs& ga, bool fuse_adam, int64_t lo = 0, int64_t hi = -1, bool last_range = true);
int head_frame_limit(int ch);
int enqueue_block_head(mww_ctx* c, int B, const Tensor& last, int T, int C, bool bf16, const BnFoldArgs& fold, const StatAcc& gacc, bool loss, bool metrics);
int enqueue_head_tail(mww_ctx* c, int B, const BnBwdFinalizeArgs& fin);

bool shape_supported(const mww_mixednet_desc& d, std::string* why, bool bf16 = false);
int plan_mixednet(const mww_mixednet_desc& d, Model** out);

int plan_convnet(const mww_convnet_desc& d, Model** out);

}
```

microwakeword_amd/csrc/kernels_bwd.hip.h:

```cpp
#pragma once
#include "kernels_fwd.hip.h"

namespace mww {

struct BwdBlockArgs {
  const float* in;
  const float* in_scale;
  const float* in_shift;
  const float* in_mean;
  const float* in_rstd;
  const float* pk;
  const float* gk;
  const float* k_mean;
  const float* k_rstd;
  const float* k_c1;
  const float* k_mg;
  const float* k_mgx;
  const float* k_scale;
  const float* k_shift;
  const float* wd;
  const float* dz;
  const float* dw_w;
  const float* dw_b;
  const float* pw_w;
  float* g_out;
  float* gstat_part;
  float* grad_part;
  int B, Tin, Tout;
  int ablate;
  unsigned long long* phase_clk;
  StatAcc gacc;
  BnGradFoldArgs gfold;
};

template <int COUT, bool LAST, bool SB = false>
struct DpStage {
  static constexpr int QO = COUT / 4, CPO = pitch(COUT), N = (TT * QO + kThreads - 1) / kThreads;
  float4 pk[N], gg[N];

  __device__ __forceinline__ void issue(const float* pk_base, const float* g_base, int nvalid, int tid) {
    constexpr bool SG = SB && !LAST;
    const BufRsrc rp = tile_rsrc(pk_base, nvalid * 4 * elem_bytes(SB)), rg = tile_rsrc(g_base, nvalid * 4 * elem_bytes(SG));
#pragma unroll
    for (int j = 0; j < N; ++j) {
      pk[j] = tile_load4s<SB, MWW_AUX_LD_PK>(rp, tid + j * kThreads);
      gg[j] = tile_load4s<SG, MWW_AUX_LD_GK>(rg, tid + j * kThreads);
    }
  }

  __device__ __forceinline__ void commit(float* sDP, const float* sKp, float dzb, int nvalid, int tid) const {
#pragma unroll
    for (int j = 0; j < N; ++j) {
      const int i = tid + j * kThreads;
      if (i < TT * QO) {
        const int r = i / QO, q = i - r * QO;
        float4 dp = make_float4(0.f, 0.f, 0.f, 0.f);
        if (i < nvalid) {
          const float4 p = pk[j];
          const float4 c1 = *reinterpret_cast<const float4*>(sKp + 0 * COUT + q * 4);
          const float4 kA = *reinterpret_cast<const float4*>(sKp + 1 * COUT + q * 4);
          const float4 kB = *reinterpret_cast<const float4*>(sKp + 2 * COUT + q * 4);
          float4 g = gg[j];
          if (LAST) {
            const float4 sc = *reinterpret_cast<const float4*>(sKp + 5 * COUT + q * 4);
            const float4 sh = *reinterpret_cast<const float4*>(sKp + 6 * COUT + q * 4);
            g.x = fmaf(p.x, sc.x, sh.x) > 0.f ? dzb * g.x : 0.f;
            g.y = fmaf(p.y, sc.y, sh.y) > 0.f ? dzb * g.y : 0.f;
            g.z = fmaf(p.z, sc.z, sh.z) > 0.f ? dzb * g.z : 0.f;
            g.w = fmaf(p.w, sc.w, sh.w) > 0.f ? dzb * g.w : 0.f;
          }
          dp.x = fmaf(g.x, c1.x, fmaf(p.x, kA.x, kB.x));
          dp.y = fmaf(g.y, c1.y, fmaf(p.y, kA.y, kB.y));
          dp.z = fmaf(g.z, c1.z, fmaf(p.z, kA.z, kB.z));
          dp.w = fmaf(g.w, c1.w, fmaf(p.w, kA.w, kB.w));
        }
        *reinterpret_cast<float4*>(sDP + r * CPO + q * 4) = dp;
      }
    }
  }
};

template <int CIN, int COUT, int KD, int PWT = pitch(CIN)>
struct WeightStage {
  static constexpr int CPI = PWT, NW = (CIN * COUT + kThreads - 1) / kThreads, ND = KD > 0 ? (KD * CIN + kThreads - 1) / kThreads : 1;
  float w[NW], d[ND];
  __device__ __forceinline__ void load(const float* pw_w, const float* dw_w, int tid) {
#pragma unroll
    for (int j = 0; j < NW; ++j) w[j] = (tid + j * kThreads < CIN * COUT) ? pw_w[tid + j * kThreads] : 0.f;
#pragma unroll
    for (int j = 0; j < ND; ++j) d[j] = (KD > 0 && tid + j * kThreads < KD * CIN) ? dw_w[tid + j * kThreads] : 0.f;
  }
  __device__ __forceinline__ void store(float* sWt, float* sDW, int tid) const {
#pragma unroll
    for (int j = 0; j < NW; ++j) {
      const int i = tid + j * kThreads;
      if (i < CIN * COUT) sWt[(i % COUT) * CPI + i / COUT] = w[j];
    }
    if (KD > 0) {
#pragma unroll
      for (int j = 0; j < ND; ++j)
        if (tid + j * kThreads < KD * CIN) sDW[tid + j * kThreads] = d[j];
    }
  }
};

template <int K, int CPI>
__device__ __forceinline__ void carry_du(float* sDU, bool first_tile, int tid) {
  for (int i = tid; i < (K - 1) * CPI; i += kThreads) sDU[i] = first_tile ? 0.f : sDU[TT * CPI + i];
}

template <int REPS, int READS, int MFMAS>
__device__ __forceinline__ void sched_read_mfma_groups() {
  if constexpr (REPS > 0) {
    if constexpr (READS > 0) __builtin_amdgcn_sched_group_barrier(0x100, READS, 0);
    __builtin_amdgcn_sched_group_barrier(0x008, MFMAS, 0);
    sched_read_mfma_groups<REPS - 1, READS, MFMAS>();
  }
}

template <int CIN, int COUT, int K, bool BF>
__device__ __forceinline__ void pointwise_backward_tile(const float* sU, const float* sDP, float* sDU, int wave, int r16,
                                                        int g, const float* sWt,
                                                        f32x4 (&dwacc)[CIN / 16][COUT / 16], bool live) {
  constexpr int CPI = pitch(CIN), CPO = pitch(COUT), MT = CIN / 16, NT = COUT / 16, KSO = COUT / 4;
  constexpr int PWT = pitch_wt(CIN, BF);
  f32x4 du[MT];
#pragma unroll
  for (int mt = 0; mt < MT; ++mt) du[mt] = zero4();
  if (!live) {
  } else if constexpr (!BF) {
    {
      float av[2][MT], bv[2][NT];
      auto load_dw = [&](int kk, int s) {
        const int row = wave * 16 + kk + 4 * g;
#pragma unroll
        for (int mt = 0; mt < MT; ++mt) av[s][mt] = sU[row * CPI + mt * 16 + r16];
#pragma unroll
        for (int nt = 0; nt < NT; ++nt) bv[s][nt] = sDP[row * CPO + nt * 16 + r16];
      };
      float a2[2], b2[2][MT];
      auto load_du = [&](int kk, int s) {
        a2[s] = sDP[(wave * 16 + r16) * CPO + kk * 4 + g];
#pragma unroll
        for (int mt = 0; mt < MT; ++mt) b2[s][mt] = sWt[(kk * 4 + g) * PWT + mt * 16 + r16];
      };
      load_dw(0, 0);
#pragma unroll
      for (int kk = 0; kk < 4; ++kk) {
        if (kk + 1 < 4) load_dw(kk + 1, (kk + 1) & 1);
        else load_du(0, 0);
#pragma unroll
        for (int mt = 0; mt < MT; ++mt)
#pragma unroll
          for (int nt = 0; nt < NT; ++nt) dwacc[mt][nt] = mfma4(av[kk & 1][mt], bv[kk & 1][nt], dwacc[mt][nt]);
      }
#pragma unroll
      for (int kk = 0; kk < KSO; ++kk) {
        if (kk + 1 < KSO) load_du(kk + 1, (kk + 1) & 1);
#pragma unroll
        for (int mt = 0; mt < MT; ++mt) du[mt] = mfma4(a2[kk & 1], b2[kk & 1][mt], du[mt]);
      }
      __builtin_amdgcn_sched_group_barrier(0x100, MT + NT, 0);
      sched_read_mfma_groups<3, MT + NT, MT * NT>();
      sched_read_mfma_groups<1, 1 + MT, MT * NT>();
      sched_read_mfma_groups<KSO - 1, 1 + MT, MT>();
      sched_read_mfma_groups<1, 0, MT>();
    }
  } else {
    const int row = wave * 16 + 4 * g;
    bf16x4 av[MT], bv[NT];
#pragma unroll
    for (int mt = 0; mt < MT; ++mt) {
      const float* col = sU + row * CPI + mt * 16 + r16;
      av[mt] = to_bf16x4(col[0], col[CPI], col[2 * CPI], col[3 * CPI]);
    }
#pragma unroll
    for (int nt = 0; nt < NT; ++nt) {
      const float* col = sDP + row * CPO + nt * 16 + r16;
      bv[nt] = to_bf16x4(col[0], col[CPO], col[2 * CPO], col[3 * CPO]);
    }
#pragma unroll
    for (int mt = 0; mt < MT; ++mt)
#pragma unroll
      for (int nt = 0; nt < NT; ++nt) dwacc[mt][nt] = mfma_bf16(av[mt], bv[nt], dwacc[mt][nt]);
#pragma unroll
    for (int kk = 0; kk < COUT / 16; ++kk) {
      const float4 v = *reinterpret_cast<const float4*>(sDP + (wave * 16 + r16) * CPO + kk * 16 + 4 * g);
      const bf16x4 a4 = to_bf16x4(v.x, v.y, v.z, v.w);
#pragma unroll
      for (int mt = 0; mt < MT; ++mt) {
        const float* col = sWt + (kk * 16 + 4 * g) * PWT + mt * 16 + r16;
        du[mt] = mfma_bf16(a4, to_bf16x4(col[0], col[PWT], col[2 * PWT], col[3 * PWT]), du[mt]);
      }
    }
  }
#pragma unroll
  for (int mt = 0; mt < MT; ++mt)
#pragma unroll
    for (int r = 0; r < 4; ++r) sDU[(K - 1 + wave * 16 + g * 4 + r) * CPI + mt * 16 + r16] = du[mt][r];
}

template <int CIN, int COUT, int K>
__device__ __forceinline__ void write_block_grad_partials(float* scratch, float* dst, const f32x4 (&dwacc)[CIN / 16][COUT / 16],
                                                          const float (&accw)[K], float accb, bool dw_active, int c,
                                                          int chunk, int tid, int wave, int r16, int g) {
  constexpr int MT = CIN / 16, NT = COUT / 16, NCH = nchunks(CIN);
  __syncthreads();
#pragma unroll
  for (int mt = 0; mt < MT; ++mt)
#pragma unroll
    for (int nt = 0; nt < NT; ++nt)
#pragma unroll
      for (int r = 0; r < 4; ++r)
        scratch[(wave * CIN + mt * 16 + g * 4 + r) * COUT + nt * 16 + r16] = dwacc[mt][nt][r];
  __syncthreads();
  for (int e = tid; e < CIN * COUT; e += kThreads)
    store_stream<MWW_AUX_ST_GP>(dst + (K + 1) * CIN + e, (scratch[e] + scratch[CIN * COUT + e]) + (scratch[2 * CIN * COUT + e] + scratch[3 * CIN * COUT + e]));
  __syncthreads();
  if (dw_active) {
#pragma unroll
    for (int i = 0; i < K; ++i) scratch[(chunk * (K + 1) + i) * CIN + c] = accw[i];
    scratch[(chunk * (K + 1) + K) * CIN + c] = accb;
  }
  __syncthreads();
  for (int e = tid; e < (K + 1) * CIN; e += kThreads) {
    float v = 0.f;
#pragma unroll
    for (int j = 0; j < NCH; ++j) v += scratch[j * (K + 1) * CIN + e];
    store_stream<MWW_AUX_ST_GP>(dst + e, v);
  }
  __syncthreads();
}


template <int CIN, int COUT, int K>
struct BwdBlockLds {
  static constexpr int CPI = pitch(CIN), CPO = pitch(COUT);
  static constexpr int RAP = halo_rows_padded(CIN, K), TTP = tile_rows_padded(CIN);
  static constexpr int OFF_END = RAP * CPI + TT * CPO + TTP * CPI + RAP * CPI;
  static constexpr int up4(int v) { return (v + 3) / 4 * 4; }
  static constexpr int KP = OFF_END, WT = KP + up4(7 * COUT), DW = WT + COUT * pitch_wt(CIN, false), ACT = DW + up4(K * CIN), END = ACT + 2 * CIN;
};
template <int K1, int C1, int COUT, int K, int S>
struct BwdFirstLds {
  static constexpr int CIN = C1, CPI = pitch(CIN), CPO = pitch(COUT);
  static constexpr int RAP = halo_rows_padded(CIN, K), TTP = tile_rows_padded(CIN);
  static constexpr int TAIL = S > 1 ? K - 1 : 0;
  static constexpr int TAILK = (TAIL + 3) / 4 * 4;
  static constexpr int OFF_END = RAP * CPI + TT * CPO + TTP * CPI + RAP * CPI + (TTP + TAILK) * CPI;
  static constexpr int XR = (TT + TAILK - 1) * S + K1, PX = FBINS + 1;
  static constexpr int up4(int v) { return (v + 3) / 4 * 4; }
  static constexpr int KP = OFF_END, WT = KP + up4(7 * COUT), X = WT + COUT * pitch_wt(CIN, false), XG = X + up4(XR * PX);
  static constexpr int END = XG + up4((int)(sizeof(XShared) + 3) / 4);
};

template <int CIN, int COUT, int K, bool LAST, bool BF, bool SB = false>
__global__ __launch_bounds__(kThreads, ((CIN > 48 || BwdBlockLds<CIN, COUT, K>::END * 4 > 80 * 1024) ? 1 : 2)) void bwd_block_kernel(BwdBlockArgs a) {
  typedef BwdBlockLds<CIN, COUT, K> Lds;
  __shared__ __attribute__((aligned(16))) float smem[Lds::OFF_END];
  __shared__ __attribute__((aligned(16))) float sKp[7 * COUT];
  __shared__ __attribute__((aligned(16))) float sWt[COUT * pitch_wt(CIN, BF)];
  __shared__ __attribute__((aligned(16))) float sDW[K * CIN];
  __shared__ __attribute__((aligned(16))) float sAct[2 * CIN];
#include "bwd_block_body.inc"
}

struct BwdFirstArgs {
  const float* x;
  const float* a0;
  const float* pk;
  const float* gk;
  const float* k_mean;
  const float* k_rstd;
  const float* k_c1;
  const float* k_mg;
  const float* k_mgx;
  const float* dw_w;
  const float* dw_b;
  const float* pw_w;
  float* grad_part;
  int B, T, Tout;
  BnGradFoldArgs gfold;
  XGather xg;
  int ablate;
  unsigned long long* phase_clk;
};

template <int K1, int C1, int COUT, int K, int S, bool BF, bool SB = false, bool X6 = false, bool LATE = false>
__global__ __launch_bounds__(kThreads, (S > 1 ? 1 : 2)) void bwd_first_kernel(BwdFirstArgs a) {
  typedef BwdFirstLds<K1, C1, COUT, K, S> Lds;
  __shared__ __attribute__((aligned(16))) float sX[X6 ? 3 * Lds::XR * 96 / 4 : Lds::XR * Lds::PX];
  __shared__ XShared sXg;
  __shared__ __attribute__((aligned(16))) float smem[X6 ? Lds::OFF_END - (Lds::TTP + Lds::TAILK) * Lds::CPI : Lds::OFF_END];
  __shared__ __attribute__((aligned(16))) float sKp[7 * COUT];
  __shared__ __attribute__((aligned(16))) float sWt[COUT * pitch_wt(C1, BF)];
#include "bwd_first_body.inc"
}

struct BnBwdFinalizeArgs {
  const float* gstat_part;
  int G, C;
  float inv_n;
  const float* gamma;
  const float* rstd;
  float* c1;
  float* mg;
  float* mgx;
  float* dgamma;
  float* dbeta;
  float dscale;
};

__device__ __forceinline__ void bn_bwd_finalize_body(const BnBwdFinalizeArgs& a, int c, double* sAcc, double* sOut, int tid) {
  float gam = 0.f, rs = 0.f;
  if (tid == 0) {
    gam = a.gamma[c];
    rs = a.rstd[c];
  }
  const double r = reduce_partials_256(a.gstat_part, a.G, a.C, c, sAcc, tid);
  if ((tid & 127) == 0) sOut[tid >> 7] = r;
  __syncthreads();
  if (tid == 0) {
    const double s1 = sOut[0], s2 = sOut[1];
    a.dbeta[c] = (float)s1 * a.dscale;
    a.dgamma[c] = (float)s2 * a.dscale;
    a.c1[c] = gam * rs;
    a.mg[c] = (float)(s1 * (double)a.inv_n);
    a.mgx[c] = (float)(s2 * (double)a.inv_n);
  }
}

#ifndef MWW_BLOCK_TU
__global__ __launch_bounds__(kThreads) void bn_bwd_finalize_kernel(BnBwdFinalizeArgs a) {
  __shared__ __attribute__((aligned(16))) double sAcc[256 + 16];
  __shared__ double sOut[2];
// ... 44 lines not shown
```

microwakeword_amd/csrc/kernels_bwdw.hip.h:

```cpp
#pragma once
#include "kernels_bwd.hip.h"

#ifndef MWW_WIDE_RELANE_K
#define MWW_WIDE_RELANE_K 15
#endif
#ifndef MWW_WIDE_TWO_GROUPS_UPTO
#define MWW_WIDE_TWO_GROUPS_UPTO 19
#endif

namespace mww {

template <int C, int NTH>
struct WidePitch;
template <>
struct WidePitch<48, 512> {
  static constexpr int P = 48, D = 1, PW = 52;
};
template <>
struct WidePitch<64, 512> {
  static constexpr int P = 72, D = 2, PW = 68;
};

template <int C, bool LAST, bool SB, int NTH, int P>
struct DpStageW {
  static constexpr int Q = C / 4, N = (TT * Q + NTH - 1) / NTH;
  float4 pk[N], gg[N];

  __device__ __forceinline__ void issue(const float* pk_base, const float* g_base, int nvalid, int tid) {
    constexpr bool SG = SB && !LAST;
    const BufRsrc rp = tile_rsrc(pk_base, nvalid * 4 * elem_bytes(SB)), rg = tile_rsrc(g_base, nvalid * 4 * elem_bytes(SG));
#pragma unroll
    for (int j = 0; j < N; ++j) {
      pk[j] = tile_load4s<SB, MWW_AUX_LD_PK>(rp, tid + j * NTH);
      gg[j] = tile_load4s<SG, MWW_AUX_LD_GK>(rg, tid + j * NTH);
    }
  }

  __device__ __forceinline__ void commit(float* sDP, const float* sKp, float dzb, int nvalid, int tid) const {
#pragma unroll
    for (int j = 0; j < N; ++j) {
      const int i = tid + j * NTH;
      if (i < TT * Q) {
        const int r = i / Q, q = i - r * Q;
        float4 dp = make_float4(0.f, 0.f, 0.f, 0.f);
        if (i < nvalid) {
          const float4 p = pk[j];
          const float4 c1 = *reinterpret_cast<const float4*>(sKp + 0 * C + q * 4);
          const float4 kA = *reinterpret_cast<const float4*>(sKp + 1 * C + q * 4);
          const float4 kB = *reinterpret_cast<const float4*>(sKp + 2 * C + q * 4);
          float4 g = gg[j];
          if (LAST) {
            const float4 sc = *reinterpret_cast<const float4*>(sKp + 5 * C + q * 4);
            const float4 sh = *reinterpret_cast<const float4*>(sKp + 6 * C + q * 4);
            g.x = fmaf(p.x, sc.x, sh.x) > 0.f ? dzb * g.x : 0.f;
            g.y = fmaf(p.y, sc.y, sh.y) > 0.f ? dzb * g.y : 0.f;
            g.z = fmaf(p.z, sc.z, sh.z) > 0.f ? dzb * g.z : 0.f;
            g.w = fmaf(p.w, sc.w, sh.w) > 0.f ? dzb * g.w : 0.f;
          }
          dp.x = fmaf(g.x, c1.x, fmaf(p.x, kA.x, kB.x));
          dp.y = fmaf(g.y, c1.y, fmaf(p.y, kA.y, kB.y));
          dp.z = fmaf(g.z, c1.z, fmaf(p.z, kA.z, kB.z));
          dp.w = fmaf(g.w, c1.w, fmaf(p.w, kA.w, kB.w));
        }
        *reinterpret_cast<float4*>(sDP + r * P + q * 4) = dp;
      }
    }
  }
};

template <int NTW, int NBLK, int BLK, int D, int PA, int PB = PA>
__device__ __forceinline__ void wide_dw_rows(const float* sU, const float* sDP, int row0, int nrows, int mcol, int ncol0,
                                             int r16, int g, f32x4 (&acc)[NTW]) {
  constexpr int KSB = BLK / 4;
  static_assert(BLK % (4 * D) == 0, "a block holds whole groups of 4 D rows");
  const float* pu = sU + (row0 + D * g) * PA + mcol + r16;
  const float* pd = sDP + (row0 + D * g) * PB + ncol0 + r16;
#pragma unroll
  for (int blk = 0; blk < NBLK; ++blk) {
    if (row0 + blk * BLK < nrows) {
      float av[2], bv[2][NTW];
      auto ld = [&](int kk, int s) {
        const int ro = blk * BLK + (kk / D) * 4 * D + (kk % D);
        av[s] = pu[ro * PA];
#pragma unroll
        for (int nt = 0; nt < NTW; ++nt) bv[s][nt] = pd[ro * PB + nt * 16];
      };
      ld(0, 0);
#pragma unroll
      for (int kk = 0; kk < KSB; ++kk) {
        if (kk + 1 < KSB) ld(kk + 1, (kk + 1) & 1);
#pragma unroll
        for (int nt = 0; nt < NTW; ++nt) acc[nt] = mfma4(av[kk & 1], bv[kk & 1][nt], acc[nt]);
      }
      __builtin_amdgcn_sched_group_barrier(0x100, 1 + NTW, 0);
      sched_read_mfma_groups<KSB - 1, 1 + NTW, NTW>();
      sched_read_mfma_groups<1, 0, NTW>();
    }
  }
}

template <int C, int NMU, int K, int P, int PW, int PD = P>
__device__ __forceinline__ void wide_du_tiles(const float* sDP, const float* sWt, float* sDU, int rt, int nrows, int mcol0,
                                              int r16, int g) {
  f32x4 du[NMU];
#pragma unroll
  for (int mu = 0; mu < NMU; ++mu) du[mu] = zero4();
  if (rt * 16 < nrows) {
    const float* pa = sDP + (rt * 16 + r16) * P + 4 * g;
    const float* pb = sWt + (4 * g) * PW + mcol0 + r16;
    float4 a4[2];
    a4[0] = *reinterpret_cast<const float4*>(pa);
#pragma unroll
    for (int kb = 0; kb < C / 16; ++kb) {
      if (kb + 1 < C / 16) a4[(kb + 1) & 1] = *reinterpret_cast<const float4*>(pa + (kb + 1) * 16);
      float bv[4][NMU];
#pragma unroll
      for (int s = 0; s < 4; ++s)
#pragma unroll
        for (int mu = 0; mu < NMU; ++mu) bv[s][mu] = pb[(kb * 16 + s) * PW + mu * 16];
      const float4 av = a4[kb & 1];
      const float as[4] = {av.x, av.y, av.z, av.w};
#pragma unroll
      for (int s = 0; s < 4; ++s)
#pragma unroll
        for (int mu = 0; mu < NMU; ++mu) du[mu] = mfma4(as[s], bv[s][mu], du[mu]);
    }
  }
  float* pd = sDU + (K - 1 + rt * 16 + g * 4) * PD + mcol0 + r16;
#pragma unroll
  for (int mu = 0; mu < NMU; ++mu)
#pragma unroll
    for (int r = 0; r < 4; ++r) pd[r * PD + mu * 16] = du[mu][r];
}

template <int NTW, int NBLK, int PA, int PB = PA>
__device__ __forceinline__ void wide_dw_rows_bf16(const float* sU, const float* sDP, int row0, int nrows, int mcol, int ncol0,
                                                  int r16, int g, f32x4 (&acc)[NTW]) {
  const float* pu = sU + (row0 + g) * PA + mcol + r16;
  const float* pd = sDP + (row0 + g) * PB + ncol0 + r16;
#pragma unroll
  for (int blk = 0; blk < NBLK; ++blk) {
    if (row0 + blk * 16 < nrows) {
      const float* cu = pu + blk * 16 * PA;
      const bf16x4 av = to_bf16x4(cu[0], cu[4 * PA], cu[8 * PA], cu[12 * PA]);
      bf16x4 bv[NTW];
#pragma unroll
      for (int nt = 0; nt < NTW; ++nt) {
        const float* cd = pd + blk * 16 * PB + nt * 16;
        bv[nt] = to_bf16x4(cd[0], cd[4 * PB], cd[8 * PB], cd[12 * PB]);
      }
#pragma unroll
      for (int nt = 0; nt < NTW; ++nt) acc[nt] = mfma_bf16(av, bv[nt], acc[nt]);
    }
  }
}

template <int C, int NMU, int K, int P, int PW, int PD = P>
__device__ __forceinline__ void wide_du_tiles_bf16(const float* sDP, const float* sWt, float* sDU, int rt, int nrows, int mcol0,
                                                   int r16, int g) {
  f32x4 du[NMU];
#pragma unroll
  for (int mu = 0; mu < NMU; ++mu) du[mu] = zero4();
  if (rt * 16 < nrows) {
    const float* pa = sDP + (rt * 16 + r16) * P + 4 * g;
    const float* pb = sWt + (4 * g) * PW + mcol0 + r16;
#pragma unroll
    for (int kb = 0; kb < C / 16; ++kb) {
      const float4 v = *reinterpret_cast<const float4*>(pa + kb * 16);
      const bf16x4 a4 = to_bf16x4(v.x, v.y, v.z, v.w);
#pragma unroll
      for (int mu = 0; mu < NMU; ++mu) {
        const float* col = pb + kb * 16 * PW + mu * 16;
        du[mu] = mfma_bf16(a4, to_bf16x4(col[0], col[PW], col[2 * PW], col[3 * PW]), du[mu]);
      }
    }
  }
  float* pd = sDU + (K - 1 + rt * 16 + g * 4) * PD + mcol0 + r16;
#pragma unroll
  for (int mu = 0; mu < NMU; ++mu)
#pragma unroll
    for (int r = 0; r < 4; ++r) pd[r * PD + mu * 16] = du[mu][r];
}

template <int K, int L, int I0, int I1, bool REV>
__device__ __forceinline__ void dw_tap_group(const float* src_c, int pitch, const float* taps_c, int tap_pitch, float (&acc)[L]) {
  constexpr int N = I1 - I0;
  float win[L + N - 1], w[N];
#pragma unroll
  for (int j = 0; j < L + N - 1; ++j) win[j] = src_c[(I0 + j) * pitch];
#pragma unroll
  for (int i = 0; i < N; ++i) w[i] = taps_c[(REV ? K - 1 - (I0 + i) : I0 + i) * tap_pitch];
#ifndef MWW_WIDE_NOREADSFIRST
  lds_reads_first();
#endif
#pragma unroll
  for (int t = 0; t < L; ++t)
#pragma unroll
    for (int i = 0; i < N; ++i) acc[t] = fmaf(w[i], win[t + i], acc[t]);
}
template <int K, int L, int I0, int I1>
__device__ __forceinline__ void dw_wgrad_group(const float* src_c, int pitch, const float (&du)[L], float (&accw)[K]) {
  constexpr int N = I1 - I0;
  float win[L + N - 1];
#pragma unroll
  for (int j = 0; j < L + N - 1; ++j) win[j] = src_c[(I0 + j) * pitch];
#ifndef MWW_WIDE_NOREADSFIRST
  lds_reads_first();
#endif
#pragma unroll
  for (int t = 0; t < L; ++t)
#pragma unroll
    for (int i = 0; i < N; ++i) accw[I0 + i] = fmaf(du[t], win[t + i], accw[I0 + i]);
}
template <int K>
struct TapGroups {
#ifdef MWW_WIDE_FEWGROUPS
  static constexpr int N = K <= 15 ? 1 : 2;
#else
  static constexpr int N = K <= 11 ? 1 : (K <= MWW_WIDE_TWO_GROUPS_UPTO ? 2 : 3);
#endif
  static constexpr int lo(int gidx) { return gidx * K / N; }
};
template <int K, int L, bool REV, int G = 0>
__device__ __forceinline__ void dw_all_groups(const float* src_c, int pitch, const float* taps_c, int tap_pitch, float (&acc)[L]) {
  if constexpr (G < TapGroups<K>::N) {
    dw_tap_group<K, L, TapGroups<K>::lo(G), TapGroups<K>::lo(G + 1), REV>(src_c, pitch, taps_c, tap_pitch, acc);
    if constexpr (G + 1 < TapGroups<K>::N) __builtin_amdgcn_sched_barrier(0);
    dw_all_groups<K, L, REV, G + 1>(src_c, pitch, taps_c, tap_pitch, acc);
  }
}
template <int K, int L, int G = 0>
__device__ __forceinline__ void dw_wgrad_all_groups(const float* src_c, int pitch, const float (&du)[L], float (&accw)[K]) {
  if constexpr (G < TapGroups<K>::N) {
    dw_wgrad_group<K, L, TapGroups<K>::lo(G), TapGroups<K>::lo(G + 1)>(src_c, pitch, du, accw);
    if constexpr (G + 1 < TapGroups<K>::N) __builtin_amdgcn_sched_barrier(0);
    dw_wgrad_all_groups<K, L, G + 1>(src_c, pitch, du, accw);
  }
}

template <int C, int NW>
struct WideRoles;
template <>
struct WideRoles<48, 8> {
  static constexpr int NTW = 3, NPART = 2;
  static __device__ __forceinline__ bool has_dw(int w) { return w < 6; }
  static __device__ __forceinline__ int part(int w) { return w / 3; }
  static __device__ __forceinline__ int mt(int w) { return w % 3; }
  static __device__ __forceinline__ int nt0(int) { return 0; }
};
template <>
struct WideRoles<64, 8> {
  static constexpr int NTW = 2, NPART = 1;
  static __device__ __forceinline__ bool has_dw(int) { return true; }
  static __device__ __forceinline__ int part(int) { return 0; }
  static __device__ __forceinline__ int mt(int w) { return w / 2; }
  static __device__ __forceinline__ int nt0(int w) { return 2 * (w % 2); }
};

template <int C, int K, int NTH>
struct BwdWideLds {
  typedef WidePitch<C, NTH> WP;
  static constexpr int NCH = NTH / C, L = (TT + NCH - 1) / NCH, TTP = NCH * L, RAP = TTP + K - 1;
  static constexpr int OFF_P = 0, OFF_DP = OFF_P + RAP * WP::P, OFF_U = OFF_DP + TT * WP::P, OFF_DU = OFF_U + TTP * WP::P;
  static constexpr int OFF_END = OFF_DU + RAP * WP::P;
  static constexpr int BYTES = (OFF_END + 7 * C + C * WP::PW + K * C + 2 * C) * 4;
};

template <int C, int K, int NTH>
constexpr int wide_waves_per_simd() {
  return (BwdWideLds<C, K, NTH>::BYTES <= 80 * 1024 ? 2 : 1) * (NTH / 64) / 4;
}

template <int CIN, int COUT, int K, bool LAST, int NTH, bool BF = false, bool SB = false, bool LATE = false>
__global__ __launch_bounds__(NTH, (wide_waves_per_simd<CIN, K, NTH>())) void bwd_blockw_kernel(BwdBlockArgs a) {
  static_assert(CIN == COUT, "the wide form is instantiated for square blocks");
  constexpr int C = CIN;
  typedef WidePitch<C, NTH> WP;
  typedef BwdWideLds<C, K, NTH> Lds;
  constexpr int NW = NTH / 64;
  typedef WideRoles<C, NW> Roles;
  constexpr int P = WP::P, PW = WP::PW, D = WP::D;
  constexpr int NCH = Lds::NCH, L = Lds::L, TTP = Lds::TTP, RA = TT + K - 1, RAP = Lds::RAP;
  constexpr int Q = C / 4, MT = C / 16;
  static_assert(NCH * L >= TT && TT >= K - 1, "tile geometry");
  static_assert(Lds::OFF_END >= Roles::NPART * C * C && Lds::OFF_END >= NCH * (K + 1) * C, "scratch aliasing");

  __shared__ __attribute__((aligned(16))) float smem[Lds::OFF_END];
  __shared__ __attribute__((aligned(16))) float sKp[7 * C];
  __shared__ __attribute__((aligned(16))) float sWt[C * PW];
  __shared__ __attribute__((aligned(16))) float sDW[K * C];
  __shared__ __attribute__((aligned(16))) float sAct[2 * C];
  float* sP = smem + Lds::OFF_P;
  float* sDP = smem + Lds::OFF_DP;
  float* sU = smem + Lds::OFF_U;
  float* sDU = smem + Lds::OFF_DU;

  const int tid = threadIdx.x, lane = tid & 63, wave = __builtin_amdgcn_readfirstlane(tid >> 6), r16_ = lane & 15, g_ = lane >> 4;
  const int c = tid % C, chunk = tid / C;
  const bool dw_active = chunk < NCH;
  MWW_PC_DECL
  MWW_PC_AT(0);

  const int ntiles = (a.Tin + TT - 1) / TT;
  const int nsamp = (int)blockIdx.x < a.B ? (a.B - (int)blockIdx.x + (int)gridDim.x - 1) / (int)gridDim.x : 0;
  const int nitems = nsamp * ntiles;
  constexpr int NP = (RA * Q + NTH - 1) / NTH;
  float4 pre_p[NP];
  DpStageW<C, LAST, SB, NTH, P> dps;
  float pre_dz = 0.f;
  auto issue_a = [&](int it, bool live) {
    const int b = blockIdx.x + (it / ntiles) * gridDim.x, t0 = (it % ntiles) * TT;
    const int nvp = live ? min(RA, a.Tin - t0) * Q : 0;
    const BufRsrc src = tile_rsrc(elem_ptr<SB>(a.in, ((size_t)b * a.Tin + t0) * C), nvp * 4 * elem_bytes(SB));
#pragma unroll
    for (int j = 0; j < NP; ++j) pre_p[j] = tile_load4s<SB, MWW_AUX_LD_BP>(src, tid + j * NTH);
  };
  auto issue_b = [&](int it, bool live) {
    const int b = blockIdx.x + (it / ntiles) * gridDim.x, t0 = (it % ntiles) * TT;
    const int nvk = live ? max(0, min(TT, a.Tout - t0)) * Q : 0;
    const size_t koff = ((size_t)b * a.Tout + t0) * C;
    dps.issue(elem_ptr<SB>(a.pk, koff), LAST ? a.wd + (size_t)t0 * C : elem_ptr<SB>(a.gk, koff), nvk, tid);
    if (LAST) pre_dz = tile_load1(tile_rsrc(a.dz, live ? a.B * 4 : 0), b * 4);
  };
  stagger_start<MWW_STAGGER_BWD>();
  if (nitems > 0) {
    issue_a(0, true);
    issue_b(0, true);
  }

  constexpr int NWL = (C * C + NTH - 1) / NTH, NDL = (K * C + NTH - 1) / NTH;
  float wl[NWL], dl[NDL];
#pragma unroll
  for (int j = 0; j < NWL; ++j) wl[j] = (tid + j * NTH < C * C) ? a.pw_w[tid + j * NTH] : 0.f;
#pragma unroll
  for (int j = 0; j < NDL; ++j) dl[j] = (tid + j * NTH < K * C) ? a.dw_w[tid + j * NTH] : 0.f;
  float accw[K];
  float accb = 0.f, gs1 = 0.f, gs2 = 0.f, dwb = 0.f;
  float sc_c = 0.f, sh_c = 0.f, mu_c = 0.f, rs_c = 0.f;
#pragma unroll
  for (int i = 0; i < K; ++i) accw[i] = 0.f;
  if (dw_active) {
    dwb = a.dw_b[c];
    sc_c = a.in_scale[c];
    sh_c = a.in_shift[c];
    mu_c = a.in_mean[c];
    rs_c = a.in_rstd[c];
  }
  for (int i = tid; i < C; i += NTH) {
    const float krs = a.k_rstd[i];
    const float kmean = a.k_mean[i];
    const float ksc = LAST ? a.k_scale[i] : 0.f, ksh = LAST ? a.k_shift[i] : 0.f;
    float c1, mg, mgx;
    if (a.gfold.acc) {
      bn_grad_fold_channel(a.gfold, C, i, krs, c1, mg, mgx);
    } else {
      c1 = a.k_c1[i];
      mg = a.k_mg[i];
      mgx = a.k_mgx[i];
    }
    const float kA = -c1 * krs * mgx;
    sKp[0 * C + i] = c1;
    sKp[1 * C + i] = kA;
    sKp[2 * C + i] = -c1 * mg - kA * kmean;
    sKp[5 * C + i] = ksc;
    sKp[6 * C + i] = ksh;
  }
#pragma unroll
  for (int j = 0; j < NWL; ++j) {
    const int i = tid + j * NTH;
    if (i < C * C) sWt[(i % C) * PW + i / C] = wl[j];
  }
#pragma unroll
  for (int j = 0; j < NDL; ++j)
    if (tid + j * NTH < K * C) sDW[tid + j * NTH] = dl[j];
  for (int i = RA * P + tid; i < RAP * P; i += NTH) {
    sP[i] = 0.f;
    sDU[i] = 0.f;
  }
  f32x4 dwacc[Roles::NTW];
#pragma unroll
  for (int nt = 0; nt < Roles::NTW; ++nt) dwacc[nt] = zero4();
  if (chunk == 0) {
    sAct[c] = sc_c;
    sAct[C + c] = sh_c;
  }
  float xk1 = sc_c != 0.f ? rs_c / sc_c : 0.f;
  float xk0 = -(sh_c + mu_c * sc_c) * xk1;
  pin(dwb); pin(xk1); pin(xk0);
  __syncthreads();

  MWW_PC_AT(1);
  MWW_PC_START(MWW_ABLATE(a, 16) && tid == 0);
  for (int it = 0; it < nitems; ++it) {
#ifndef MWW_WIDE_NOPRIO
    rotate_priority(it, 2);
#endif
    const int b = blockIdx.x + (it / ntiles) * gridDim.x, t0 = (it % ntiles) * TT;
    const int nrows_new = max(0, min(TT, a.Tout - t0));
    const int rows_da = min(TT, a.Tin - t0);
#pragma unroll
    for (int j = 0; j < NP; ++j) {
      const int i = tid + j * NTH;
      if (i < RA * Q) {
        const int r = i / Q, q = i - r * Q;
        const float4 s4 = *reinterpret_cast<const float4*>(sAct + q * 4), h4 = *reinterpret_cast<const float4*>(sAct + C + q * 4);
        float4 v = pre_p[j];
        v.x = fmaxf(fmaf(v.x, s4.x, h4.x), 0.f);
        v.y = fmaxf(fmaf(v.y, s4.y, h4.y), 0.f);
        v.z = fmaxf(fmaf(v.z, s4.z, h4.z), 0.f);
        v.w = fmaxf(fmaf(v.w, s4.w, h4.w), 0.f);
        *reinterpret_cast<float4*>(sP + r * P + q * 4) = v;
      }
    }
    MWW_PC_MARK(0);
    if constexpr (!LATE) dps.commit(sDP, sKp, pre_dz, nrows_new * Q, tid);
    for (int i = tid; i < (K - 1) * P; i += NTH) sDU[i] = (t0 == 0) ? 0.f : sDU[TT * P + i];
    if constexpr (LATE) issue_a(it + 1, it + 1 < nitems);
    MWW_PC_MARK(LATE ? 0 : 8);
    __syncthreads();
    MWW_PC_MARK(1);
    if constexpr (!LATE) {
      if (it + 1 < nitems) {
        issue_a(it + 1, true);
        issue_b(it + 1, true);
      }
    }
    if (dw_active) {
      if (chunk * L < nrows_new) {
        float o[L];
#pragma unroll
        for (int t = 0; t < L; ++t) o[t] = dwb;
        dw_all_groups<K, L, false>(sP + chunk * L * P + c, P, sDW + c, C, o);
#pragma unroll
        for (int t = 0; t < L; ++t) {
          const int tl = chunk * L + t;
          sU[tl * P + c] = (tl < nrows_new) ? o[t] : 0.f;
        }
      } else {
#pragma unroll
        for (int t = 0; t < L; ++t) sU[(chunk * L + t) * P + c] = 0.f;
      }
    }
    MWW_PC_MARK(2);
    if constexpr (LATE) {
      dps.commit(sDP, sKp, pre_dz, nrows_new * Q, tid);
      issue_b(it + 1, it + 1 < nitems);
      MWW_PC_MARK(8);
    }
    __syncthreads();
    MWW_PC_MARK(3);
    int r16 = r16_, g = g_;
    if constexpr (MWW_WIDE_RELANE_K > 0 && K >= MWW_WIDE_RELANE_K) {
      int lm = lane;
      pin(lm);
      r16 = lm & 15;
      g = lm >> 4;
    }
    if constexpr (C == 48 && NW == 8) {
      if (wave < 6) {
        if constexpr (BF) {
          wide_dw_rows_bf16<3, 2, P>(sU, sDP, 32 * (wave / 3), nrows_new, 16 * (wave % 3), 0, r16, g, dwacc);
          wide_du_tiles_bf16<C, 1, K, P, PW>(sDP, sWt, sDU, 2 + wave / 3, nrows_new, 16 * (wave % 3), r16, g);
        } else {
          wide_dw_rows<3, 2, 16, D, P>(sU, sDP, 32 * (wave / 3), nrows_new, 16 * (wave % 3), 0, r16, g, dwacc);
          wide_du_tiles<C, 1, K, P, PW>(sDP, sWt, sDU, 2 + wave / 3, nrows_new, 16 * (wave % 3), r16, g);
        }
      } else {
        if constexpr (BF) wide_du_tiles_bf16<C, 3, K, P, PW>(sDP, sWt, sDU, wave - 6, nrows_new, 0, r16, g);
        else wide_du_tiles<C, 3, K, P, PW>(sDP, sWt, sDU, wave - 6, nrows_new, 0, r16, g);
      }
    } else if constexpr (BF) {
      wide_dw_rows_bf16<2, 4, P>(sU, sDP, 0, nrows_new, 16 * (wave / 2), 32 * (wave % 2), r16, g, dwacc);
      wide_du_tiles_bf16<C, 2, K, P, PW>(sDP, sWt, sDU, wave / 2, nrows_new, 32 * (wave % 2), r16, g);
    } else {
      wide_dw_rows<2, 4, 16, D, P>(sU, sDP, 0, nrows_new, 16 * (wave / 2), 32 * (wave % 2), r16, g, dwacc);
      wide_du_tiles<C, 2, K, P, PW>(sDP, sWt, sDU, wave / 2, nrows_new, 32 * (wave % 2), r16, g);
    }
    MWW_PC_MARK(4);
    __syncthreads();
    MWW_PC_MARK(5);
    {
      const int cch = dw_active ? chunk : NCH - 1;
      const BufRsrc gtile = tile_rsrc(elem_ptr<SB>(a.g_out, ((size_t)b * a.Tin + t0) * C), rows_da * C * elem_bytes(SB));
      const int goff = (dw_active ? 0 : kOobOffset / 4) + cch * L * C + c;
      const float* wdu_p = sDU + cch * L * P + c;
      const float* wa_p = sP + cch * L * P + c;
      {
        float da[L], am[L];
#pragma unroll
        for (int t = 0; t < L; ++t) da[t] = 0.f;
        if (cch * L < rows_da) dw_all_groups<K, L, true>(wdu_p, P, sDW + c, C, da);
        __builtin_amdgcn_sched_barrier(0);
#pragma unroll
        for (int t = 0; t < L; ++t) am[t] = wa_p[t * P];
#pragma unroll
        for (int t = 0; t < L; ++t) {
          const int sl = cch * L + t;
          const float gg = (sl < rows_da && am[t] > 0.f) ? da[t] : 0.f;
          tile_store1s<SB, MWW_AUX_ST_G>(gtile, goff + t * C, gg);
          gs1 += gg;
          gs2 = fmaf(gg, fmaf(am[t], xk1, xk0), gs2);
        }
      }
      __builtin_amdgcn_sched_barrier(0);
      if (cch * L < nrows_new) {
        float duk[L];
#pragma unroll
        for (int t = 0; t < L; ++t) duk[t] = wdu_p[(K - 1 + t) * P];
#pragma unroll
        for (int t = 0; t < L; ++t) accb += duk[t];
        dw_wgrad_all_groups<K, L>(wa_p, P, duk, accw);
      }
    }
    MWW_PC_MARK(6);
    __syncthreads();
    MWW_PC_MARK(7);
  }
  MWW_PC_AT(2);

  float* gdst = a.grad_part + (size_t)blockIdx.x * ((K + 1) * C + C * C);
  float* scratch = smem;
  if (Roles::has_dw(wave)) {
    float* sp = scratch + Roles::part(wave) * C * C + (Roles::mt(wave) * 16 + g_ * 4) * C + Roles::nt0(wave) * 16 + r16_;
#pragma unroll
    for (int nt = 0; nt < Roles::NTW; ++nt)
#pragma unroll
      for (int r = 0; r < 4; ++r) sp[r * C + nt * 16] = dwacc[nt][r];
  }
  __syncthreads();
  for (int e = tid; e < C * C; e += NTH) {
    float v = scratch[e];
    if constexpr (Roles::NPART == 2) v += scratch[C * C + e];
    store_stream<MWW_AUX_ST_GP>(gdst + (K + 1) * C + e, v);
  }
  __syncthreads();
  if (dw_active) {
#pragma unroll
    for (int i = 0; i < K; ++i) scratch[(chunk * (K + 1) + i) * C + c] = accw[i];
    scratch[(chunk * (K + 1) + K) * C + c] = accb;
  }
  __syncthreads();
  for (int e = tid; e < (K + 1) * C; e += NTH) {
    float v = 0.f;
#pragma unroll
    for (int j = 0; j < NCH; ++j) v += scratch[j * (K + 1) * C + e];
    store_stream<MWW_AUX_ST_GP>(gdst + e, v);
  }
  __syncthreads();
  if (dw_active) {
    scratch[(chunk * 2 + 0) * C + c] = gs1;
    scratch[(chunk * 2 + 1) * C + c] = gs2;
  }
  __syncthreads();
  if (tid < 2 * C) {
    float v = 0.f;
#pragma unroll
    for (int j = 0; j < NCH; ++j) v += scratch[j * 2 * C + tid];
    publish_stat(a.gacc, a.gstat_part + (size_t)blockIdx.x * 2 * C, 2 * C, tid, v);
  }
  MWW_PC_AT(3);
  MWW_PC_DUMP(a.phase_clk ? a.phase_clk + (size_t)blockIdx.x * kClkSlots : nullptr);
}

template <int K1, int C1, int COUT, int K, int S, int NTH, bool X6 = false>
struct BwdFirstWideLds {
  static constexpr int PI = C1 + 4;
  static constexpr int PO = COUT + 4;
  static constexpr int PG = C1 + 5;
  static constexpr int PW = C1 + 4;
  static constexpr int PX = FBINS + 1;
  static constexpr int NCH = NTH / C1, L = (TT + NCH - 1) / NCH, TTP = NCH * L, RAP = TTP + K - 1;
  static constexpr int TAIL = S > 1 ? K - 1 : 0;
  static constexpr int TAILK = (TAIL + 3) / 4 * 4;
  static constexpr int XR = (TT + TAILK - 1) * S + K1;
  static constexpr int up4(int v) { return (v + 3) / 4 * 4; }
  static constexpr int OFF_A = 0, OFF_DP = OFF_A + up4(RAP * PI), OFF_U = OFF_DP + TT * PO, OFF_DU = OFF_U + up4(TTP * PI);
  static constexpr int PB = 96, PLB = XR * PB, GPB = 2 * C1, GPL = TT * GPB;
  static constexpr int XFLOATS = X6 ? 3 * PLB / 4 : up4(XR * PX);
  static constexpr int OFF_G0 = OFF_DU + up4(RAP * PI), OFF_END = X6 ? OFF_G0 : OFF_G0 + up4((TTP + TAILK) * PG);
  static constexpr int BYTES = (OFF_END + XFLOATS + 7 * COUT + COUT * PW) * 4 + (int)sizeof(XShared);
};

template <int K1, int C1, int COUT, int K, int S, int NTH, bool X6 = false>
constexpr int wide_first_waves_per_simd() {
  return (BwdFirstWideLds<K1, C1, COUT, K, S, NTH, X6>::BYTES <= 80 * 1024 ? 2 : 1) * (NTH / 64) / 4;
}

template <int K1, int C1, int COUT, int K, int S, int NTH, bool X6 = false, bool LATE = false>
__global__ __launch_bounds__(NTH, (wide_first_waves_per_simd<K1, C1, COUT, K, S, NTH, X6>())) void bwd_firstw_kernel(BwdFirstArgs a) {
  typedef BwdFirstWideLds<K1, C1, COUT, K, S, NTH, X6> Lds;
  constexpr bool SB = false;
  constexpr int CIN = C1;
  constexpr int PI = Lds::PI, PO = Lds::PO, PG = Lds::PG, PW = Lds::PW, PX = Lds::PX;
  constexpr int NW = NTH / 64, NCH = Lds::NCH, L = Lds::L, TTP = Lds::TTP, RA = TT + K - 1, RAP = Lds::RAP;
  constexpr int TAIL = Lds::TAIL, XR = Lds::XR;
  constexpr int NT1 = C1 / 16, M1 = K1 * FBINS, MT1 = (M1 + 15) / 16, MPW = (MT1 + NW - 1) / NW;
  constexpr int MT = CIN / 16, NT = COUT / 16, QI = CIN / 4, QO = COUT / 4;
  static_assert(NW == 8 && MT == 2 && NCH * L == TT && TT >= K - 1, "geometry of the wide first-block kernel");
  static_assert(TAIL <= NCH && TTP + TAIL <= RAP, "tail rows");
  static_assert(Lds::OFF_END >= 2 * CIN * COUT && Lds::OFF_END >= NCH * (K + 1) * CIN, "scratch aliasing");
  constexpr int PB = Lds::PB, PLB = Lds::PLB, GPB = Lds::GPB, GPL = Lds::GPL;
  static_assert(!X6 || (S == 1 && CIN == 32 && (K1 * FBINS) % 8 == 0 && 3 * GPL <= (TT * PO + TTP * PI) * 4 && TTP == TT), "the x6 form serves the stride-1 first convolutions");

  __shared__ __attribute__((aligned(16))) float sX[Lds::XFLOATS];
  __shared__ XShared sXg;
  __shared__ __attribute__((aligned(16))) float smem[Lds::OFF_END];
  __shared__ __attribute__((aligned(16))) float sKp[7 * COUT];
  __shared__ __attribute__((aligned(16))) float sWt[COUT * PW];
  float* sA = smem + Lds::OFF_A;
  float* sDP = smem + Lds::OFF_DP;
  float* sU = smem + Lds::OFF_U;
  float* sDU = smem + Lds::OFF_DU;
  float* sG0 = smem + Lds::OFF_G0;

  const int tid = threadIdx.x, lane = tid & 63, wave = __builtin_amdgcn_readfirstlane(tid >> 6), r16 = lane & 15, g = lane >> 4;
  const int c = tid % CIN, chunk = tid / CIN;
  const int Ta = (a.T - K1) / S + 1;

  const bool tailmode = TAIL > 0 && Ta > TT && Ta <= TT + TAIL;
  const int ntiles = tailmode ? 1 : (Ta + TT - 1) / TT;
  const int nsamp = (int)blockIdx.x < a.B ? (a.B - (int)blockIdx.x + (int)gridDim.x - 1) / (int)gridDim.x : 0;
  const int nitems = nsamp * ntiles;
  XStage<XR, PX, MWW_AUX_LD_XB, NTH> xs;
  DpStageW<COUT, false, SB, NTH, PO> dps;
  constexpr int NA = (RA * QI + NTH - 1) / NTH;
  float4 pre_a[NA];
  auto issue_a = [&](int it, bool live) {
    const int s = live ? it / ntiles : nsamp - 1, b = blockIdx.x + s * gridDim.x, t0 = (it % ntiles) * TT;
    const int nrx = live ? ((tailmode ? Ta : min(TT, Ta - t0)) - 1) * S + K1 : 0;
    xs.issue(a.x, a.xg, sXg, s, b, a.T, t0 * S, nrx, tid);
    const BufRsrc ra = tile_rsrc(a.a0 + ((size_t)b * Ta + t0) * CIN, live ? min(RA, Ta - t0) * QI * 16 : 0);
#pragma unroll
    for (int j = 0; j < NA; ++j) pre_a[j] = tile_load4<MWW_AUX_LD_A0>(ra, (tid + j * NTH) * 16);
  };
  auto issue_b = [&](int it, bool live) {
    const int b = blockIdx.x + (it / ntiles) * gridDim.x, t0 = (it % ntiles) * TT;
    const int nvk = live ? max(0, min(TT, a.Tout - t0)) * QO : 0;
    const size_t koff = ((size_t)b * a.Tout + t0) * COUT;
    dps.issue(elem_ptr<SB>(a.pk, koff), elem_ptr<SB>(a.gk, koff), nvk, tid);
  };
  int offm[MPW];
  bool okm[MPW];
  int xoff[MPW], goff[NT1];
  if constexpr (X6) {
    const int rowl = 4 * g + (r16 >> 2), cg = 4 * (r16 & 3);
#pragma unroll
    for (int mi = 0; mi < MPW; ++mi) {
      const int m = min((mi * NW + wave) * 16 + cg, M1 - 4);
      xoff[mi] = (rowl + m / FBINS) * PB + (m % FBINS) * 2;
    }
#pragma unroll
    for (int nt = 0; nt < NT1; ++nt) goff[nt] = rowl * GPB + ((nt * 16 + cg) ^ ((rowl & 4) ? 16 : 0)) * 2;
  } else {
#pragma unroll
  for (int mi = 0; mi < MPW; ++mi) {
    const int m = (mi * NW + wave) * 16 + r16;
    okm[mi] = m < M1;
    offm[mi] = okm[mi] ? (m / FBINS) * PX + (m % FBINS) : 0;
  }
  }
  if (a.xg.win) xgather_setup(a.xg, sXg, nsamp, tid);
  stagger_start<MWW_STAGGER_BWD>();
  if (nitems > 0) {
    issue_a(0, true);
    issue_b(0, true);
  }

  constexpr int NWL = (CIN * COUT + NTH - 1) / NTH;
  float wl[NWL];
#pragma unroll
  for (int j = 0; j < NWL; ++j) wl[j] = (tid + j * NTH < CIN * COUT) ? a.pw_w[tid + j * NTH] : 0.f;
  float accw[K];
  float accb = 0.f;
#pragma unroll
  for (int i = 0; i < K; ++i) accw[i] = 0.f;
  float dwb = a.dw_b[c];
  float dww[K];
#pragma unroll
  for (int i = 0; i < K; ++i) dww[i] = a.dw_w[i * CIN + c];
  for (int i = tid; i < COUT; i += NTH) {
    const float krs = a.k_rstd[i];
    const float kmean = a.k_mean[i];
    float c1, mg, mgx;
    if (a.gfold.acc) {
      bn_grad_fold_channel(a.gfold, COUT, i, krs, c1, mg, mgx);
    } else {
      c1 = a.k_c1[i];
      mg = a.k_mg[i];
      mgx = a.k_mgx[i];
    }
    const float kA = -c1 * krs * mgx;
    sKp[0 * COUT + i] = c1;
    sKp[1 * COUT + i] = kA;
    sKp[2 * COUT + i] = -c1 * mg - kA * kmean;
    sKp[5 * COUT + i] = 0.f;
    sKp[6 * COUT + i] = 0.f;
  }
#pragma unroll
  for (int j = 0; j < NWL; ++j) {
    const int i = tid + j * NTH;
    if (i < CIN * COUT) sWt[(i % COUT) * PW + i / COUT] = wl[j];
  }
  for (int i = RA * PI + tid; i < RAP * PI; i += NTH) {
    sA[i] = 0.f;
    sDU[i] = 0.f;
  }
  if constexpr (!X6)
    for (int i = TT * PG + tid; i < (TTP + Lds::TAILK) * PG; i += NTH) sG0[i] = 0.f;
#pragma unroll
  for (int i = 0; i < K; ++i) pin(dww[i]);
  pin(dwb);
  f32x4 dwacc[NT];
#pragma unroll
  for (int nt = 0; nt < NT; ++nt) dwacc[nt] = zero4();
  f32x4 w1acc[MPW][NT1];
#pragma unroll
  for (int mi = 0; mi < MPW; ++mi)
#pragma unroll
    for (int nt = 0; nt < NT1; ++nt) w1acc[mi][nt] = zero4();
  __syncthreads();

  for (int it = 0; it < nitems; ++it) {
#ifndef MWW_WIDE_NOPRIO
    rotate_priority(it, 2);
#endif
    const int t0 = (it % ntiles) * TT;
    const int nrows_new = max(0, min(TT, a.Tout - t0));
    const int rows_da = min(TT, Ta - t0);
    if constexpr (X6) xs.template commit_planes<PB, PLB>(reinterpret_cast<unsigned*>(sX), a.xg, sXg, it / ntiles, t0 * S, tid);
    else xs.commit(sX, a.xg, sXg, it / ntiles, t0 * S, tid);
#pragma unroll
    for (int j = 0; j < NA; ++j) {
      const int i = tid + j * NTH;
      if (i < RA * QI) {
        const int r = i / QI, q = i - r * QI;
        *reinterpret_cast<float4*>(sA + r * PI + q * 4) = pre_a[j];
      }
    }
    if constexpr (!LATE) dps.commit(sDP, sKp, 0.f, nrows_new * QO, tid);
    for (int i = tid; i < (K - 1) * PI; i += NTH) sDU[i] = (t0 == 0) ? 0.f : sDU[TT * PI + i];
    if constexpr (LATE) issue_a(it + 1, it + 1 < nitems);
    __syncthreads();
    if constexpr (!LATE) {
      if (it + 1 < nitems) {
        issue_a(it + 1, true);
        issue_b(it + 1, true);
      }
    }
    if (chunk * L < nrows_new) {
      float o[L];
      dw_chunk<K, L>(sA, PI, chunk * L, c, dww, dwb, o);
#pragma unroll
      for (int t = 0; t < L; ++t) {
        const int tl = chunk * L + t;
        sU[tl * PI + c] = (tl < nrows_new) ? o[t] : 0.f;
      }
    } else {
#pragma unroll
      for (int t = 0; t < L; ++t) sU[(chunk * L + t) * PI + c] = 0.f;
    }
    if constexpr (LATE) {
      dps.commit(sDP, sKp, 0.f, nrows_new * QO, tid);
      issue_b(it + 1, it + 1 < nitems);
    }
    __syncthreads();
    if (wave < 4) {
      wide_du_tiles<COUT, MT, K, PO, PW, PI>(sDP, sWt, sDU, wave, nrows_new, 0, r16, g);
    } else {
      const int v = wave - 4;
      wide_dw_rows<NT, 2, 16, 4, PI, PO>(sU, sDP, 32 * (v / 2), nrows_new, 16 * (v % 2), 0, r16, g, dwacc);
    }
    __syncthreads();
    {
      float wdu[L + K - 1], wa[L + K - 1];
#pragma unroll
      for (int j = 0; j < L + K - 1; ++j) wdu[j] = sDU[(chunk * L + j) * PI + c];
#pragma unroll
      for (int j = 0; j < L + K - 1; ++j) wa[j] = sA[(chunk * L + j) * PI + c];
      lds_reads_first();
#pragma unroll
      for (int t = 0; t < L; ++t) {
        const int sl = chunk * L + t;
        float acc = 0.f;
#pragma unroll
        for (int i = 0; i < K; ++i) acc = fmaf(dww[K - 1 - i], wdu[t + i], acc);
        const float gv = (sl < rows_da && wa[t] > 0.f) ? acc : 0.f;
        if constexpr (X6) {
          unsigned h0, h1, h2;
          split3(gv, h0, h1, h2);
          unsigned short* gp = reinterpret_cast<unsigned short*>(sDP) + sl * CIN + (c ^ ((sl & 4) ? 16 : 0));
          gp[0] = (unsigned short)(h0 >> 16);
          gp[GPL / 2] = (unsigned short)(h1 >> 16);
          gp[GPL] = (unsigned short)(h2 >> 16);
        } else {
          sG0[sl * PG + c] = gv;
        }
      }
      if (chunk * L < nrows_new) {
#pragma unroll
        for (int t = 0; t < L; ++t) {
          const float dut = wdu[K - 1 + t];
          accb += dut;
#pragma unroll
          for (int i = 0; i < K; ++i) accw[i] = fmaf(dut, wa[t + i], accw[i]);
        }
      }
      if constexpr (TAIL > 0) {
        if (tailmode && chunk < TAIL) {
          const int sl = TT + chunk;
          float acc = 0.f;
#pragma unroll
          for (int j = 0; j < K; ++j) acc = fmaf(dww[K - 1 - j], sl + j < RAP ? sDU[(sl + j) * PI + c] : 0.f, acc);
          sG0[sl * PG + c] = (sl < Ta && sA[sl * PI + c] > 0.f) ? acc : 0.f;
        }
      }
    }
    __syncthreads();
    if constexpr (X6) {
      const char* xb = reinterpret_cast<const char*>(sX);
      const char* gb = reinterpret_cast<const char*>(sDP);
#pragma unroll
      for (int kb = 0; kb < TT / 32; ++kb)
#pragma unroll
        for (int nt = 0; nt < NT1; ++nt) {
          u32x4v gq[3];
#pragma unroll
          for (int p = 0; p < 3; ++p) {
            const u32x2v lo = lds_read_tr16(gb + goff[nt] + p * GPL + (32 * kb) * GPB), hi = lds_read_tr16(gb + goff[nt] + p * GPL + (32 * kb + 16) * GPB);
            gq[p] = u32x4v{lo.x, lo.y, hi.x, hi.y};
          }
#pragma unroll
          for (int mi = 0; mi < MPW; ++mi)
            if (mi * NW + wave < MT1) {
              u32x4v xq[3];
#pragma unroll
              for (int p = 0; p < 3; ++p) {
                const u32x2v lo = lds_read_tr16(xb + xoff[mi] + p * PLB + (32 * kb) * S * PB), hi = lds_read_tr16(xb + xoff[mi] + p * PLB + (32 * kb + 16) * S * PB);
                xq[p] = u32x4v{lo.x, lo.y, hi.x, hi.y};
              }
              w1acc[mi][nt] = mfma_x6(xq, gq, w1acc[mi][nt]);
            }
        }
    } else {
      float av[2][MPW], bv[2][NT1];
      auto load_w1 = [&](int srow, int sl) {
#pragma unroll
        for (int nt = 0; nt < NT1; ++nt) bv[sl][nt] = sG0[srow * PG + nt * 16 + r16];
#pragma unroll
        for (int mi = 0; mi < MPW; ++mi) {
          const float v = sX[srow * S * PX + offm[mi]];
          av[sl][mi] = okm[mi] ? v : 0.f;
        }
      };
      load_w1(16 * g, 0);
#pragma unroll
      for (int kk = 0; kk < TT / 4; ++kk) {
        if (kk + 1 < TT / 4) load_w1(kk + 1 + 16 * g, (kk + 1) & 1);
#pragma unroll
        for (int mi = 0; mi < MPW; ++mi)
          if (mi * NW + wave < MT1) {
#pragma unroll
            for (int nt = 0; nt < NT1; ++nt) w1acc[mi][nt] = mfma4(av[kk & 1][mi], bv[kk & 1][nt], w1acc[mi][nt]);
          }
      }
      if constexpr (TAIL > 0) {
        if (tailmode) {
#pragma unroll
          for (int ks = 0; ks < Lds::TAILK / 4; ++ks) {
            load_w1(TT + 4 * ks + g, 0);
#pragma unroll
            for (int mi = 0; mi < MPW; ++mi)
              if (mi * NW + wave < MT1) {
#pragma unroll
                for (int nt = 0; nt < NT1; ++nt) w1acc[mi][nt] = mfma4(av[0][mi], bv[0][nt], w1acc[mi][nt]);
              }
          }
        }
      }
    }
    __syncthreads();
  }

  float* gdst = a.grad_part + (size_t)blockIdx.x * (M1 * C1 + (K + 1) * CIN + CIN * COUT);
#pragma unroll
  for (int mi = 0; mi < MPW; ++mi)
#pragma unroll
    for (int nt = 0; nt < NT1; ++nt)
#pragma unroll
      for (int r = 0; r < 4; ++r) {
        const int m = (mi * NW + wave) * 16 + g * 4 + r;
        if (m < M1) store_stream<MWW_AUX_ST_GP>(gdst + m * C1 + nt * 16 + r16, w1acc[mi][nt][r]);
      }
  float* gblk = gdst + M1 * C1;
  float* scratch = smem;
  if (wave >= 4) {
    const int v = wave - 4;
    float* sp = scratch + (v / 2) * CIN * COUT + ((v % 2) * 16 + g * 4) * COUT + r16;
#pragma unroll
    for (int nt = 0; nt < NT; ++nt)
#pragma unroll
      for (int r = 0; r < 4; ++r) sp[r * COUT + nt * 16] = dwacc[nt][r];
  }
  __syncthreads();
  for (int e = tid; e < CIN * COUT; e += NTH) store_stream<MWW_AUX_ST_GP>(gblk + (K + 1) * CIN + e, scratch[e] + scratch[CIN * COUT + e]);
  __syncthreads();
#pragma unroll
  for (int i = 0; i < K; ++i) scratch[(chunk * (K + 1) + i) * CIN + c] = accw[i];
  scratch[(chunk * (K + 1) + K) * CIN + c] = accb;
  __syncthreads();
  for (int e = tid; e < (K + 1) * CIN; e += NTH) {
    float v = 0.f;
#pragma unroll
    for (int j = 0; j < NCH; ++j) v += scratch[j * (K + 1) * CIN + e];
    store_stream<MWW_AUX_ST_GP>(gblk + e, v);
  }
}

}
```

microwakeword_amd/csrc/kernels_head.hip.h:

```cpp
#pragma once
#include <type_traits>

#include "common.hip.h"

namespace mww {

struct MetricState {
  unsigned long long hist101[2][101];
  unsigned long long hist200[2][200];
  unsigned long long n, correct, tp5, fp5, fn5, pos, neg;
  double bce_sum;
};

struct HeadArgs {
  const float* p;
  const float* scale;
  const float* shift;
  const float* mean;
  const float* rstd;
  const float* wd;
  const float* bd;
  const float* y;
  const float* sw;
  float* z;
  float* prob;
  float* dz;
  float* loss_part;
  float* gstat_part;
  int B, T;
  float inv_b;
  int training;
  BnFoldArgs fold;
  StatAcc gacc;
};

template <int C, int JMAX, bool SB = false>
__global__ __launch_bounds__(kThreads, 2) void head_kernel(HeadArgs a) {
  constexpr int Q = C / 4;
  constexpr int NRG = kThreads / Q;
  __shared__ __attribute__((aligned(16))) float sRed[8];
  __shared__ __attribute__((aligned(16))) float sBcast[2];
  __shared__ __attribute__((aligned(16))) float sStat[NRG * 2 * C];

  const int tid = threadIdx.x, lane = tid & 63, wave = tid >> 6;
  const int q = tid % Q, rg = tid / Q;
  const bool active = rg < NRG;
  float4 wdv[JMAX];
  {
    const BufRsrc wr = tile_rsrc(a.wd, active ? a.T * C * 4 : 0);
#pragma unroll
    for (int j = 0; j < JMAX; ++j) wdv[j] = tile_load4(wr, ((rg + NRG * j) * C + q * 4) * 4);
  }
  auto fetch = [&](int b, float4 (&dst)[JMAX], float& yy, float& ww) {
    const bool ok = b < a.B;
    const BufRsrc pr = tile_rsrc(elem_ptr<SB>(a.p, (size_t)(ok ? b : 0) * a.T * C), (ok && active) ? a.T * C * elem_bytes(SB) : 0);
#pragma unroll
    for (int j = 0; j < JMAX; ++j) dst[j] = tile_load4s<SB, MWW_AUX_LD_HP>(pr, (rg + NRG * j) * Q + q);
    yy = (ok && a.y != nullptr) ? a.y[b] : 0.f;
    ww = (ok && a.y != nullptr && (a.training & kHeadTraining)) ? a.sw[b] : 0.f;
  };
  float4 raw[JMAX], nxt[JMAX];
  float y_cur = 0.f, w_cur = 0.f, y_nxt = 0.f, w_nxt = 0.f;
  fetch(blockIdx.x, raw, y_cur, w_cur);
  float4 sc = make_float4(0, 0, 0, 0), sh = sc, mu = sc, rs = sc;
  if (a.fold.acc) {
    float* sFold = sStat;
    if (tid < C) bn_fold_channel(a.fold, C, tid, sFold[tid], sFold[C + tid], sFold[2 * C + tid], sFold[3 * C + tid]);
    __syncthreads();
    if (active) {
      sc = *reinterpret_cast<const float4*>(sFold + q * 4);
      sh = *reinterpret_cast<const float4*>(sFold + C + q * 4);
      mu = *reinterpret_cast<const float4*>(sFold + 2 * C + q * 4);
      rs = *reinterpret_cast<const float4*>(sFold + 3 * C + q * 4);
    }
    __syncthreads();
  } else if (active) {
    sc = *reinterpret_cast<const float4*>(a.scale + q * 4);
    sh = *reinterpret_cast<const float4*>(a.shift + q * 4);
    if (a.training & kHeadTraining) {
      mu = *reinterpret_cast<const float4*>(a.mean + q * 4);
      rs = *reinterpret_cast<const float4*>(a.rstd + q * 4);
    }
  }
  const float bias = a.bd[0];
  float4 g1 = make_float4(0, 0, 0, 0), g2 = g1;

  for (int b = blockIdx.x; b < a.B; b += gridDim.x) {
    float dot = 0.f;
    fetch(b + gridDim.x, nxt, y_nxt, w_nxt);
#pragma unroll
    for (int j = 0; j < JMAX; ++j) {
      dot = fmaf(fmaxf(fmaf(raw[j].x, sc.x, sh.x), 0.f), wdv[j].x, dot);
      dot = fmaf(fmaxf(fmaf(raw[j].y, sc.y, sh.y), 0.f), wdv[j].y, dot);
      dot = fmaf(fmaxf(fmaf(raw[j].z, sc.z, sh.z), 0.f), wdv[j].z, dot);
      dot = fmaf(fmaxf(fmaf(raw[j].w, sc.w, sh.w), 0.f), wdv[j].w, dot);
    }
    dot = wave_sum(dot);
    if (lane == 0) sRed[wave] = dot;
    __syncthreads();
    if (tid == 0) {
      const float zz = ((sRed[0] + sRed[1]) + (sRed[2] + sRed[3])) + bias;
      const float pr = 1.0f / (1.0f + expf(-zz));
      a.z[b] = zz;
      a.prob[b] = pr;
      float dzz = 0.f;
      if (a.y != nullptr) {
        const float yy = y_cur;
        const bool clipped_form = (a.training & kHeadClippedLoss) != 0;
        const float bce = bce_value(zz, pr, yy, clipped_form);
        if (a.training & kHeadTraining) {
          const float w = w_cur;
          a.loss_part[b] = w * bce * a.inv_b;
          dzz = w * bce_dz(pr, yy, clipped_form) * a.inv_b;
          a.dz[b] = dzz;
        }
      }
      sBcast[0] = dzz;
    }
    __syncthreads();
    if (a.training & kHeadTraining) {
      const float dzz = sBcast[0];
#pragma unroll
      for (int j = 0; j < JMAX; ++j) {
        const float gx = fmaf(raw[j].x, sc.x, sh.x) > 0.f ? dzz * wdv[j].x : 0.f;
        const float gy = fmaf(raw[j].y, sc.y, sh.y) > 0.f ? dzz * wdv[j].y : 0.f;
        const float gz = fmaf(raw[j].z, sc.z, sh.z) > 0.f ? dzz * wdv[j].z : 0.f;
        const float gw = fmaf(raw[j].w, sc.w, sh.w) > 0.f ? dzz * wdv[j].w : 0.f;
        g1.x += gx; g1.y += gy; g1.z += gz; g1.w += gw;
        g2.x = fmaf(gx, (raw[j].x - mu.x) * rs.x, g2.x);
        g2.y = fmaf(gy, (raw[j].y - mu.y) * rs.y, g2.y);
        g2.z = fmaf(gz, (raw[j].z - mu.z) * rs.z, g2.z);
        g2.w = fmaf(gw, (raw[j].w - mu.w) * rs.w, g2.w);
      }
    }
#pragma unroll
    for (int j = 0; j < JMAX; ++j) raw[j] = nxt[j];
    y_cur = y_nxt;
    w_cur = w_nxt;
  }
  if (a.training & kHeadTraining) {
    if (active) {
      *reinterpret_cast<float4*>(sStat + (rg * 2 + 0) * C + q * 4) = g1;
      *reinterpret_cast<float4*>(sStat + (rg * 2 + 1) * C + q * 4) = g2;
    }
    __syncthreads();
    if (tid < 2 * C) {
      float v = 0.f;
      for (int r = 0; r < NRG; ++r) v += sStat[r * 2 * C + tid];
      publish_stat(a.gacc, a.gstat_part + (size_t)blockIdx.x * 2 * C, 2 * C, tid, v);
    }
  }
}

struct MetricsArgs {
  const float* prob;
  const float* y;
  MetricState* m;
  int B;
  const float* z;
};

template <int NT>
__device__ __forceinline__ void metrics_body(const MetricsArgs& a, unsigned (*sH101)[101], unsigned (*sH200)[200], unsigned* sCnt,
                                             double* sBce, int tid) {
  constexpr int N101 = (202 + NT - 1) / NT, N200 = (400 + NT - 1) / NT;
  unsigned long long old101[N101], old200[N200], old_cnt = 0ull;
  double old_bce = 0.0;
#pragma unroll
  for (int k = 0; k < N101; ++k) old101[k] = tid + k * NT < 202 ? (&a.m->hist101[0][0])[tid + k * NT] : 0ull;
#pragma unroll
  for (int k = 0; k < N200; ++k) old200[k] = tid + k * NT < 400 ? (&a.m->hist200[0][0])[tid + k * NT] : 0ull;
  if (tid < 7) old_cnt = (&a.m->n)[tid];
  if (tid == 0) old_bce = a.m->bce_sum;
  for (int i = tid; i < 202; i += NT) (&sH101[0][0])[i] = 0u;
  for (int i = tid; i < 400; i += NT) (&sH200[0][0])[i] = 0u;
  if (tid < 8) sCnt[tid] = 0u;
  __syncthreads();
  double bce = 0.0;
  int cnt[7] = {0, 0, 0, 0, 0, 0, 0};
  for (int b = tid; b < a.B; b += NT) {
    const float pr = a.prob[b], yy = a.y[b];
    const int lab = yy > 0.5f ? 1 : 0;
    const float p01 = fminf(fmaxf(pr, 0.f), 1.f);
    const int b101 = (int)ceilf(p01 * 100.0f) - 1;
    int b200 = (int)ceilf(p01 * 199.0f) - 1;
    if (b200 < 0) b200 = 0;
    if (b101 >= 0) atomicAdd(&sH101[lab][b101], 1u);
    atomicAdd(&sH200[lab][b200], 1u);
    const bool ppos = pr > 0.5f;
    cnt[0] += 1;
    cnt[1] += (ppos == (lab == 1)) ? 1 : 0;
    cnt[2] += (ppos && lab) ? 1 : 0;
    cnt[3] += (ppos && !lab) ? 1 : 0;
    cnt[4] += (!ppos && lab) ? 1 : 0;
    cnt[5] += lab ? 1 : 0;
    cnt[6] += lab ? 0 : 1;
    bce += (double)bce_value(a.z ? a.z[b] : 0.f, pr, yy, a.z == nullptr);
  }
#pragma unroll
  for (int k = 0; k < 7; ++k) {
    int v = cnt[k];
#pragma unroll
    for (int m = 1; m < 64; m <<= 1) v += __shfl_xor(v, m);
    if ((tid & 63) == 0 && v) atomicAdd(&sCnt[k], (unsigned)v);
  }
#pragma unroll
  for (int m = 1; m < 64; m <<= 1) {
    union { double d; int i[2]; } u;
    u.d = bce;
    u.i[0] = __shfl_xor(u.i[0], m);
    u.i[1] = __shfl_xor(u.i[1], m);
    bce += u.d;
  }
  if ((tid & 63) == 0) sBce[tid >> 6] = bce;
  __syncthreads();
#pragma unroll
  for (int k = 0; k < N101; ++k) {
    const int i = tid + k * NT;
    const unsigned v = i < 202 ? (&sH101[0][0])[i] : 0u;
    if (v) (&a.m->hist101[0][0])[i] = old101[k] + v;
  }
#pragma unroll
  for (int k = 0; k < N200; ++k) {
    const int i = tid + k * NT;
    const unsigned v = i < 400 ? (&sH200[0][0])[i] : 0u;
    if (v) (&a.m->hist200[0][0])[i] = old200[k] + v;
  }
  if (tid < 7 && sCnt[tid]) (&a.m->n)[tid] = old_cnt + sCnt[tid];
  if (tid == 0) {
    double s = 0.0;
    for (int i = 0; i < NT / 64; ++i) s += sBce[i];
    a.m->bce_sum = old_bce + s;
  }
}

__global__ __launch_bounds__(1024) void metrics_kernel(MetricsArgs a) {
  __shared__ unsigned sH101[2][101];
  __shared__ unsigned sH200[2][200];
  __shared__ unsigned sCnt[8];
  __shared__ double sBce[1024];
  metrics_body<1024>(a, sH101, sH200, sCnt, sBce, threadIdx.x);
}

struct DenseGradArgs {
  const float* p;
  const float* scale;
  const float* shift;
  const float* dz;
  float* part;
  int B, n, C, stride, chunk;
  const float* keep;
  const float *rp, *rscale, *rshift;
  int rT, rdrop;
  int p_bf16;
};

__device__ __forceinline__ void dense_grad_body(const DenseGradArgs& a, int bx, int by, int tid) {
  const int e = bx * kThreads + tid;
  const int b0 = by * a.chunk, b1 = min(a.B, b0 + a.chunk);
  if (e < a.n) {
    const int c = e % a.C;
    const float sc = a.scale[c], sh = a.shift[c];
    const float rsc = a.rp ? a.rscale[c] : 0.f, rsh = a.rp ? a.rshift[c] : 0.f;
    const size_t roff = a.rp ? (size_t)a.rdrop * a.C + e : 0, rstride = (size_t)a.rT * a.C;
    float acc = 0.f;
    auto rows = [&](auto stored, auto has_res, auto has_keep) {
      constexpr bool SB = decltype(stored)::value, RES = decltype(has_res)::value, KEEP = decltype(has_keep)::value;
      for (int bb = b0; bb < b1; bb += 8) {
        float v[8], d[8], r[8];
#pragma unroll
        for (int u = 0; u < 8; ++u) {
          const size_t row = (size_t)min(bb + u, b1 - 1);
          v[u] = load_elem<SB>(a.p, row * a.n + e);
          d[u] = a.dz[row];
          r[u] = 0.f;
          if constexpr (RES) r[u] = a.rp[row * rstride + roff];
          if constexpr (KEEP) d[u] *= a.keep[row * a.n + e];
        }
#pragma unroll
        for (int u = 0; u < 8; ++u) {
          if constexpr (RES) r[u] = fmaf(r[u], rsc, rsh);
          if (bb + u >= b1) d[u] = 0.f;
          acc = fmaf(d[u], fmaxf(fmaf(v[u], sc, sh) + r[u], 0.f), acc);
        }
      }
    };
    auto pick_keep = [&](auto stored, auto has_res) {
      if (a.keep) rows(stored, has_res, std::true_type{});
      else rows(stored, has_res, std::false_type{});
    };
    auto pick_res = [&](auto stored) {
      if (a.rp) pick_keep(stored, std::true_type{});
      else pick_keep(stored, std::false_type{});
    };
    if (a.p_bf16) pick_res(std::true_type{});
    else pick_res(std::false_type{});
    a.part[(size_t)by * a.stride + e] = acc;
  } else if (e == a.n) {
    float s = 0.f;
    for (int b = b0; b < b1; ++b) s += a.dz[b];
    a.part[(size_t)by * a.stride + a.n] = s;
  }
}

__global__ __launch_bounds__(kThreads) void dense_grad_kernel(DenseGradArgs a) {
  dense_grad_body(a, blockIdx.x, blockIdx.y, threadIdx.x);
}

}
```

microwakeword_amd/csrc/mww_lib.hip:

```cpp
#include <hip/hip_runtime.h>

#include <dlfcn.h>

#include <cmath>
#include <cstdio>
#include <climits>
#include <cstring>
#include <map>
#include <string>
#include <vector>

#include "engine.hip.h"
#include "kernels_bnre.hip.h"
#include "kernels_data.hip.h"
#include "kernels_ema.hip.h"
#include "kernels_head.hip.h"
#include "kernels_qat.hip.h"
#include "kernels_sam.hip.h"
#include "kernels_tail.hip.h"

using namespace mww;

namespace {
thread_local std::string g_err;
}

int mww::fail(int code, const std::string& msg) {
  g_err = msg;
  return code;
}

namespace {

constexpr int kHeadMaxRows = 24;

int launch_head(mww_ctx* c, int ch, int jmax, bool bf16, const HeadArgs& a, int grid) {
#define X(C, J)                                                                                                \
  if (ch == C && jmax <= J) {                                                                                  \
    if (bf16)                                                                                                  \
      hipLaunchKernelGGL((head_kernel<C, J, true>), dim3(grid), dim3(kThreads), 0, c->stream, a);              \
    else                                                                                                       \
      hipLaunchKernelGGL((head_kernel<C, J>), dim3(grid), dim3(kThreads), 0, c->stream, a);                    \
    return MWW_OK;                                                                                             \
  }
  static_assert(kHeadMaxRows == 24, "the widest instantiation below");
  X(32, 2) X(32, 4) X(32, 8) X(32, 12) X(32, 16) X(32, 24) X(48, 2) X(48, 4) X(48, 8) X(48, 12) X(48, 16) X(48, 24) X(64, 2) X(64, 4) X(64, 8) X(64, 12) X(64, 16) X(64, 24)
#undef X
  return fail(MWW_ERR_UNSUPPORTED, "no head kernel for this (channels, frames) shape");
}

}

namespace mww {

int head_frame_limit(int ch) { return (kThreads / (ch / 4)) * kHeadMaxRows; }

int enqueue_block_head(mww_ctx* c, int B, const Tensor& last, int T, int C, bool bf16, const BnFoldArgs& fold, const StatAcc& gacc, bool loss, bool metrics) {
  float* const bn = last.bn;
  const HeadArgs h{last.p, bn + (size_t)BN_SCALE * C, bn + (size_t)BN_SHIFT * C, bn + (size_t)BN_MEAN * C, bn + (size_t)BN_RSTD * C,
                   fwd_params(c) + c->o_dense_w, fwd_params(c) + c->o_dense_b, (loss || metrics) ? c->y_cur : nullptr, c->sw_cur, c->z, c->prob, c->dz,
                   c->loss_part, last.gstat_part, B, T, 1.0f / (float)B, (loss ? kHeadTraining : 0) | (c->bce_clipped ? kHeadClippedLoss : 0), fold, gacc};
  const int q = C / 4, nrg = kThreads / q;
  Launcher lp{c};
  lp.begin("head");
  int rc = launch_head(c, C, (T + nrg - 1) / nrg, bf16, h, std::min(B, c->grid_head));
  lp.end();
  return rc;
}

const float* mail_hyper(mww_ctx* c) { return reinterpret_cast<const float*>(c->mail_dev[c->mail_cur] + c->mail_off_hyper); }

static int restamp_lazy_slot(mww_ctx* c) {
  if (c->lazy_slot >= 0 && c->lazy_slot != c->mail_cur) HIPCHK(hipEventRecord(c->mail_ev[c->lazy_slot], c->stream));
  return MWW_OK;
}

static int bring_targets(mww_ctx* c) {
  if (c->y_cur == c->y) return MWW_OK;
  const size_t n = (size_t)c->lazy_a.B * sizeof(float);
  HIPCHK(hipMemcpyAsync(c->y, c->y_cur, n, hipMemcpyDeviceToDevice, c->stream));
  HIPCHK(hipMemcpyAsync(c->sw, c->sw_cur, n, hipMemcpyDeviceToDevice, c->stream));
  c->y_cur = c->y;
  c->sw_cur = c->sw;
  return restamp_lazy_slot(c);
}

int materialise_x(mww_ctx* c) {
  int rc = bring_targets(c);
  if (rc || !c->x_lazy) return rc;
  AssembleArgs a = c->lazy_a;
  a.n_targets = 0;
  Launcher lp{c};
  lp.begin("assemble");
  hipLaunchKernelGGL(assemble_kernel, dim3(a.B * a.split), dim3(kThreads), 0, c->stream, a);
  lp.end();
  HIPCHK(hipGetLastError());
  c->x_lazy = false;
  return restamp_lazy_slot(c);
}

XGather x_gather(mww_ctx* c) {
  XGather g;
  memset(&g, 0, sizeof(g));
  if (!c->x_lazy) return g;
  const AssembleArgs& a = c->lazy_a;
  g.win = a.win;
  g.masks = a.masks;
  for (int i = 0; i < MWW_MAX_STORES; ++i) { g.store[i] = a.store[i]; g.dtype[i] = a.dtype[i]; }
  g.ntm = a.ntm;
  g.nfm = a.nfm;
  g.T = a.T;
  return g;
}

static int join_side(mww_ctx* c) {
  if (c->side_pending) {
    HIPCHK(hipStreamWaitEvent(c->stream, c->ev_join, 0));
    c->side_pending = false;
  }
  return MWW_OK;
}

static DenseGradArgs dense_args(mww_ctx* c, int B, const DenseSource& s, float* part, int stride) {
  return DenseGradArgs{s.p, s.scale, s.shift, c->dz, part, B, c->t_last * c->c_last, c->c_last, stride, (B + kDenseChunks - 1) / kDenseChunks,
                       s.keep, s.rp, s.rscale, s.rshift, s.rT, s.rdrop, s.bf16};
}

int enqueue_side_work(mww_ctx* c, int B, bool metrics, bool loss, const DenseSource& last) {
  Launcher lp{c};
  if (metrics || loss) {
    const bool inline_side = c->profile || !c->use_side;
    hipStream_t ss = inline_side ? c->stream : c->side;
    if (!inline_side) {
      HIPCHK(hipEventRecord(c->ev_fork, c->stream));
      HIPCHK(hipStreamWaitEvent(c->side, c->ev_fork, 0));
    }
    const bool one_launch = metrics && loss && inline_side;
    if (metrics && !one_launch) {
      MetricsArgs ma{c->prob, c->y_cur, c->metrics, B, c->bce_clipped ? nullptr : c->z};
      lp.begin("metrics");
      hipLaunchKernelGGL(metrics_kernel, dim3(1), dim3(1024), 0, ss, ma);
      c->metric_launches += 1;
      lp.end();
    }
    if (loss) {
      const DenseGradArgs dg = dense_args(c, B, last, c->dwd_part, c->dwd_stride);
      const int ndchunks = (B + dg.chunk - 1) / dg.chunk;
      if (one_launch) {
        HeadTailArgs ht;
        memset(&ht, 0, sizeof(ht));
        ht.dense = dg;
        ht.met = MetricsArgs{c->prob, c->y_cur, c->metrics, B, c->bce_clipped ? nullptr : c->z};
        ht.n_fin = 0;
        ht.ndx = (dg.n + 1 + kThreads - 1) / kThreads;
        ht.ndy = ndchunks;
        ht.do_metrics = 1;
        c->metric_launches += 1;
        lp.begin("dense_grad+metrics");
        hipLaunchKernelGGL(head_tail_kernel, dim3(ht.ndx * ht.ndy + 1), dim3(kThreads), 0, ss, ht);
        lp.end();
      } else {
        lp.begin("dense_grad");
        hipLaunchKernelGGL(dense_grad_kernel, dim3((dg.n + 1 + kThreads - 1) / kThreads, ndchunks), dim3(kThreads), 0, ss, dg);
        lp.end();
      }
    }
    if (!inline_side) {
      HIPCHK(hipEventRecord(c->ev_join, c->side));
      c->side_pending = true;
    }
  }
  return MWW_OK;
}


int exchange_stats(mww_ctx* c, Launcher& lp, const char* what, int layer, const float* part, int G, int C, int bwd,
                   float local_inv_n, StatSource* out) {
  out->part = part;
  out->G = G;
  out->inv_n = local_inv_n;
  out->dscale = 1.0f;
  if (!(c->hook && c->sync_bn)) return MWW_OK;
  float* buf = c->sync_buf + c->sync_off[layer] + (bwd ? 2 * C : 0);
  StatCollapseArgs a{part, G, C, buf};
  lp.begin(what, layer);
  hipLaunchKernelGGL(stat_collapse_kernel, dim3(C), dim3(kThreads), 0, c->stream, a);
  lp.end();
  if (c->hook(c->hook_user, buf, 2 * C, MWW_EXCHANGE_IN_ORDER) != 0) return fail(MWW_ERR_STATE, "all-reduce hook failed");
  out->part = buf;
  out->G = 1;
  out->inv_n = local_inv_n / (float)c->world;
  out->dscale = 1.0f / (float)c->world;
  return MWW_OK;
}

StatSource forward_stat_source(const mww_ctx* c, int layer, const float* part, int G, int C, float local_inv_n) {
  if (!(c->hook && c->sync_bn)) return StatSource{part, G, local_inv_n, 1.0f};
  return StatSource{c->sync_buf + c->sync_off[layer], 1, local_inv_n / (float)c->world, 1.0f / (float)c->world};
}

int enqueue_bnre_collect(mww_ctx* c, std::vector<BnreRow>& rows) {
  if (rows.empty()) return MWW_OK;
  int blocks = 0;
  for (BnreRow& r : rows) {
    r.nblocks = r.form == BNRE_ROWS ? 1 : (r.groups > 1 ? r.groups : r.C);
    r.block0 = blocks;
    blocks += r.nblocks;
  }
  const size_t bytes = rows.size() * sizeof(BnreRow);
  if (c->bnre_table_host.size() != bytes || memcmp(c->bnre_table_host.data(), rows.data(), bytes) != 0) {
    HIPCHK(hipStreamSynchronize(c->stream));
    if (c->bnre_table_rows < (int)rows.size()) {
      if (c->bnre_table) HIPCHK(hipFree(c->bnre_table));
      c->bnre_table = nullptr;
      c->bnre_table_rows = 0;
      MWW_TRY(dev_alloc(&c->bnre_table, rows.size()));
      c->bnre_table_rows = (int)rows.size();
    }
    c->bnre_table_host.clear();
    HIPCHK(hipMemcpy(c->bnre_table, rows.data(), bytes, hipMemcpyHostToDevice));
    c->bnre_table_host.assign(reinterpret_cast<const char*>(rows.data()), reinterpret_cast<const char*>(rows.data()) + bytes);
  }
  Launcher lp{c};
  lp.begin("bn_reestimate_collect");
  launch_bnre_collect(BnreCollectArgs{c->bnre_table, (int)rows.size(), c->fpar ^ 1, c->bnre_acc}, blocks, c->stream);
  lp.end();
  return MWW_OK;
}

}
namespace {

int enqueue_adam(mww_ctx* c);

int assemble_range(mww_ctx* c, int B, const GradReduceArgs& ga, int64_t lo, int64_t hi, bool tail_dense, bool metrics, bool apply_adam) {
  Launcher lp{c};
  std::vector<FinalSegment> segs;
  for (int i = 0; i < ga.nseg; ++i) {
    const GradSegment& g = ga.seg[i];
    if (g.dst < lo || g.dst >= hi) continue;
    if (g.dst + g.n > hi) return fail(MWW_ERR_STATE, "gradient segment straddles a bucket boundary");
    segs.push_back(FinalSegment{g.part, g.G, g.stride, g.n, g.dst, kSegPartials, 0});
  }
  GradFinalArgs a;
  memset(&a, 0, sizeof(a));
  if (tail_dense && c->o_dense_w >= lo && c->o_dense_w < hi) {
    a.dense = dense_args(c, B, c->tail_src, nullptr, 0);
    segs.push_back(FinalSegment{nullptr, B, 0, c->t_last * c->c_last + 1, (int)c->o_dense_w, kSegDense, 0});
  }
  std::sort(segs.begin(), segs.end(), [](const FinalSegment& x, const FinalSegment& y) { return x.dst < y.dst; });
  std::vector<FinalSegment> all;
  int64_t cur = lo;
  auto fill = [&](int64_t upto) {
    while (cur < upto) {
      const bool dir = c->direct_host[(size_t)cur] != 0;
      int64_t e = cur;
      while (e < upto && (c->direct_host[(size_t)e] != 0) == dir) ++e;
      all.push_back(FinalSegment{nullptr, 1, 0, (int)(e - cur), (int)cur, dir ? kSegDirect : kSegZero, 0});
      cur = e;
    }
  };
  for (const FinalSegment& sgm : segs) {
    if (sgm.dst < cur) return fail(MWW_ERR_STATE, "overlapping gradient segments");
    fill(sgm.dst);
    all.push_back(sgm);
    cur = sgm.dst + sgm.n;
  }
  fill(hi);
  a.met = MetricsArgs{c->prob, c->y_cur, c->metrics, B, c->bce_clipped ? nullptr : c->z};
  a.mask = c->mask;
  a.grad = c->grads;
  a.scale = 1.0f;
  a.adam = AdamArgs{c->params, c->grads, c->adam_m, c->adam_v, mail_hyper(c), (int)c->P, 0.9f, 0.999f, 1e-7f};
  a.apply_adam = apply_adam ? 1 : 0;
  for (size_t first = 0; first < all.size() || (metrics && first == 0); first += kMaxFinalSegments) {
    const int n = (int)std::min<size_t>(kMaxFinalSegments, all.size() - first);
    int nb = 0, ns = 0;
    for (int pass = 0; pass < 2; ++pass)
      for (int i = 0; i < n; ++i) {
        const FinalSegment& sg = all[first + i];
        if ((sg.kind == kSegDense) != (pass == 0)) continue;
        a.seg[ns] = sg;
        a.seg[ns].block0 = nb;
        a.block0[ns] = nb;
        nb += (sg.n + kFinalCols - 1) / kFinalCols;
        ++ns;
      }
    for (int i = ns; i < kMaxFinalSegments; ++i) a.block0[i] = INT_MAX;
    a.nseg = n;
    a.nblocks = nb;
    a.do_metrics = (metrics && first == 0) ? 1 : 0;
    if (nb + a.do_metrics == 0) break;
    c->metric_launches += a.do_metrics;
    lp.begin(apply_adam ? "grad_final+adam" : "grad_final");
    hipLaunchKernelGGL(grad_final_kernel, dim3(nb + a.do_metrics), dim3(kThreads), 0, c->stream, a);
    lp.end();
    if (all.empty()) break;
  }
  return MWW_OK;
}

int exchange_range(mww_ctx* c, int64_t lo, int64_t hi, int flags) {
  if (c->hook(c->hook_user, flags == MWW_EXCHANGE_FLUSH ? nullptr : c->grads + lo, flags == MWW_EXCHANGE_FLUSH ? 0 : hi - lo, flags) != 0)
    return fail(MWW_ERR_STATE, "all-reduce hook failed");
  return MWW_OK;
}

}

namespace mww {

int enqueue_grad_assembly(mww_ctx* c, int B, GradReduceArgs& ga, bool fuse_adam, int64_t lo, int64_t hi, bool last_range) {
  if (hi < 0) hi = c->P;
  int rcj = join_side(c);
  if (rcj) return rcj;
  const bool tail_here = c->tail_in_reduce && c->o_dense_w >= lo && c->o_dense_w < hi;
  if (tail_here) c->tail_in_reduce = false;
  if (!tail_here && c->o_dense_w >= lo && c->o_dense_w < hi) {
    const int dchunk = (B + kDenseChunks - 1) / kDenseChunks;
    GradSegment s;
    s.part = c->dwd_part;
    s.G = (B + dchunk - 1) / dchunk;
    s.stride = c->dwd_stride;
    s.n = c->t_last * c->c_last + 1;
    s.dst = (int)c->o_dense_w;
    ga.seg[ga.nseg++] = s;
  }
  const bool exchange = fuse_adam && c->hook && c->reduce_grads;
  int rc = assemble_range(c, B, ga, lo, hi, tail_here, tail_here && c->tail_metrics, fuse_adam && !exchange);
  if (rc || !exchange) return rc;
  rc = exchange_range(c, lo, hi, last_range ? MWW_EXCHANGE_IN_ORDER : MWW_EXCHANGE_DEFERRED);
  if (!last_range) c->exchange_pending = true;
  if (rc || !last_range) return rc;
  if (c->exchange_pending) {
    rc = exchange_range(c, 0, 0, MWW_EXCHANGE_FLUSH);
    c->exchange_pending = false;
    if (rc) return rc;
  }
  return enqueue_adam(c);
}

}

namespace mww {

int enqueue_head_tail(mww_ctx* c, int B, const BnBwdFinalizeArgs& fin) {
  const int dchunk = (B + kDenseChunks - 1) / kDenseChunks;
  HeadTailArgs ht;
  ht.fin = fin;
  ht.dense = dense_args(c, B, c->tail_src, c->dwd_part, c->dwd_stride);
  ht.met = MetricsArgs{c->prob, c->y_cur, c->metrics, B, c->bce_clipped ? nullptr : c->z};
  ht.n_fin = fin.C;
  ht.ndx = (ht.dense.n + 1 + kThreads - 1) / kThreads;
  ht.ndy = (B + dchunk - 1) / dchunk;
  ht.do_metrics = c->tail_metrics ? 1 : 0;
  c->metric_launches += ht.do_metrics;
  Launcher lp{c};
  lp.begin("head_tail");
  hipLaunchKernelGGL(head_tail_kernel, dim3(ht.n_fin + ht.ndx * ht.ndy + ht.do_metrics), dim3(kThreads), 0, c->stream, ht);
  lp.end();
  return MWW_OK;
}

}
// ... 844 lines not shown
  int B = 0, ntm = 0, nfm = 0;
  mww_prefetch_shape(p, &B, &ntm, &nfm);
  rc = mww_set_targets(c, y, w, B);
  if (!rc) rc = mww_assemble_batch(c, win, masks, B, ntm, nfm);
  if (!rc && out_labels) memcpy(out_labels, y, (size_t)B * sizeof(float));
  if (!rc && out_weights) memcpy(out_weights, w, (size_t)B * sizeof(float));
  mww_prefetch_release(p);
  return rc;
}

int mww_train_step(mww_ctx* c, int B, float lr, int flags) {
  if (!c || B <= 0 || B > c->max_batch) return fail(MWW_ERR_INVALID, "bad batch size");
  if (c->have_batch < B || c->have_targets < B) return fail(MWW_ERR_STATE, "train step needs a batch and targets of at least B rows");
  HIPCHK(hipSetDevice(c->device));
  int rc = batch_ready(c);
  if (rc) return rc;
  const bool apply = !(flags & MWW_STEP_NO_APPLY);
  if (apply) {
    c->step += 1;
    rc = push_hyper(c, adam_alpha(lr, c->step), (c->hook && c->reduce_grads) ? 1.0f / (float)c->world : 1.0f);
    if (rc) return rc;
  }
  const int ema = apply ? ema_due(c) : EMA_NONE;
  unsigned long long counter = 0;
  const bool gen_dropout = c->model->step_counter(&counter);
  if (gen_dropout) {
    rc = mail_begin(c);
    if (rc) return rc;
    unsigned* h = reinterpret_cast<unsigned*>(c->mail_host[c->mail_cur] + c->mail_off_hyper);
    h[2] = (unsigned)(counter & 0xFFFFFFFFull);
    h[3] = (unsigned)(counter >> 32);
  }
  const bool sharp = apply && (c->sam_rho > 0.0 || c->clip_norm > 0.0);
  if (c->use_graphs && !c->profile && !c->hook && !sharp) {
    const int mail = (apply || gen_dropout || c->x_lazy) ? c->mail_cur : -1;
    bool handover = false;
    const unsigned mkey = c->model->replay_key(&handover);
    const bool flips = c->bn_inline && handover;
    const unsigned ckey = (flips ? (4 | c->fpar | (c->gpar << 1)) : 0) | (c->x_lazy ? 8 : 0) | (c->y_cur != c->y ? 16 : 0) | (c->tail_roles ? 32 : 0) | ((unsigned)ema << 6);
    hipGraphExec_t exec = nullptr;
    for (auto& g : c->graphs)
      if (g.B == B && g.flags == flags && g.mail == mail && g.core == ckey && g.model == mkey) exec = g.exec;
    if (exec && flips) {
      c->fpar ^= 1;
      c->gpar ^= 1;
    }
    if (!exec) {
      hipGraph_t graph;
      HIPCHK(hipStreamBeginCapture(c->stream, hipStreamCaptureModeThreadLocal));
      rc = step_sequence(c, B, flags, ema);
      hipError_t e = hipStreamEndCapture(c->stream, &graph);
      if (rc) return rc;
      if (e != hipSuccess) return fail(MWW_ERR_HIP, std::string("hipStreamEndCapture: ") + hipGetErrorString(e));
      HIPCHK(hipGraphInstantiate(&exec, graph, nullptr, nullptr, 0));
      HIPCHK(hipGraphDestroy(graph));
      c->graphs.push_back({B, flags, mail, ckey, mkey, exec});
    }
    HIPCHK(hipGraphLaunch(exec, c->stream));
    if (ema) { c->ema_updates += 1; invalidate_ema_bn(c); }
    return mail_commit(c);
  }
  rc = step_sequence(c, B, flags, ema);
  if (rc) return rc;
  HIPCHK(hipGetLastError());
  if (ema) { c->ema_updates += 1; invalidate_ema_bn(c); }
  return mail_commit(c);
}

int mww_apply_gradients(mww_ctx* c, float lr, float gscale) {
  if (!c) return fail(MWW_ERR_INVALID, "null context");
  HIPCHK(hipSetDevice(c->device));
  c->step += 1;
  int rc = push_hyper(c, adam_alpha(lr, c->step), gscale);
  if (rc) return rc;
  if (c->clip_norm > 0.0) {
    rc = enqueue_final_norm(c, true);
    if (rc) return rc;
  }
  rc = enqueue_adam(c);
  if (rc) return rc;
  const int ema = ema_due(c);
  rc = enqueue_ema(c, ema);
  if (rc) return rc;
  HIPCHK(hipGetLastError());
  if (ema) { c->ema_updates += 1; invalidate_ema_bn(c); }
  return mail_commit(c);
}

int mww_forward(mww_ctx* c, int B, int training, int update_metrics) {
  if (!c || B <= 0 || B > c->max_batch) return fail(MWW_ERR_INVALID, "bad batch size");
  if (c->have_batch < B) return fail(MWW_ERR_STATE, "forward needs a batch of at least B rows");
  if (update_metrics && c->have_targets < B) return fail(MWW_ERR_STATE, "metric update needs targets");
  HIPCHK(hipSetDevice(c->device));
  int rc = batch_ready(c);
  if (rc) return rc;
  EmaSource source(c, training != 0);
  rc = refresh_shadow(c);
  if (rc) return rc;
  rc = c->model->enqueue_forward(c, B, training != 0, false, false, update_metrics != 0);
  if (rc) return rc;
  rc = join_side(c);
  if (rc) return rc;
  HIPCHK(hipGetLastError());
  return mail_commit(c);
}

int mww_bn_reestimate_begin(mww_ctx* c) {
  if (!c) return fail(MWW_ERR_INVALID, "null context");
  if (!c->ema || c->ema_updates == 0) return fail(MWW_ERR_INVALID, "bn_reestimate needs a weight average that has taken an update");
  HIPCHK(hipSetDevice(c->device));
  if (!c->ema_bn) MWW_TRY(dev_alloc(&c->ema_bn, (size_t)c->S));
  if (!c->bnre_acc) MWW_TRY(dev_alloc(&c->bnre_acc, (size_t)c->S));
  HIPCHK(hipMemsetAsync(c->bnre_acc, 0, (size_t)c->S * sizeof(double), c->stream));
  c->bnre_batches = 0;
  return MWW_OK;
}

int mww_bn_reestimate_batch(mww_ctx* c, int B) {
  if (!c || B <= 0 || B > c->max_batch) return fail(MWW_ERR_INVALID, "bad batch size");
  if (c->bnre_batches < 0) return fail(MWW_ERR_STATE, "bn_reestimate: no pass is open (call mww_bn_reestimate_begin; an update of the average closes a pass)");
  if (c->have_batch < B) return fail(MWW_ERR_STATE, "forward needs a batch of at least B rows");
  HIPCHK(hipSetDevice(c->device));
  int rc = batch_ready(c);
  if (rc) return rc;
  EmaSource source(c, true);
  c->ema_src = true;
  rc = refresh_shadow(c);
  if (rc) return rc;
  rc = c->model->enqueue_forward(c, B, true, false, false, false);
  if (rc) return rc;
  rc = join_side(c);
  if (rc) return rc;
  rc = c->model->enqueue_bn_collect(c, B);
  if (rc) return rc;
  HIPCHK(hipGetLastError());
  c->bnre_batches += 1;
  return mail_commit(c);
}

int mww_bn_reestimate_commit(mww_ctx* c) {
  if (!c) return fail(MWW_ERR_INVALID, "null context");
  if (c->bnre_batches <= 0) return fail(MWW_ERR_STATE, "bn_reestimate: commit without a collected batch");
  HIPCHK(hipSetDevice(c->device));
  Launcher lp{c};
  lp.begin("bn_reestimate_commit");
  launch_bnre_commit(BnreCommitArgs{c->bnre_acc, c->ema_bn, (double)c->bnre_batches, (int)c->S}, c->stream);
  lp.end();
  HIPCHK(hipGetLastError());
  c->bnre_batches = -1;
  c->ema_bn_valid = true;
  return MWW_OK;
}

int mww_bn_reestimate_windows(mww_ctx* c, const mww_window* windows, int64_t n, int batch) {
  if (!c || !windows || batch <= 0 || batch > c->max_batch) return fail(MWW_ERR_INVALID, "bad re-estimation arguments");
  if (n <= 0 || n % batch != 0) return fail(MWW_ERR_INVALID, "bn_reestimate: the window count must be a positive multiple of the batch size (every batch weighs the same)");
  if (!c->ema || c->ema_updates == 0) return fail(MWW_ERR_INVALID, "bn_reestimate needs a weight average that has taken an update");
  int rc = mww_assemble_batch(c, windows, nullptr, batch, 0, 0);
  if (!rc) rc = mww_bn_reestimate_begin(c);
  for (int64_t s = 0; s < n && !rc; s += batch) {
    if (s) rc = mww_assemble_batch(c, windows + s, nullptr, batch, 0, 0);
    if (!rc) rc = mww_bn_reestimate_batch(c, batch);
    c->shadow_held = c->ema;
  }
  c->shadow_held = nullptr;
  if (rc) { c->bnre_batches = -1; return rc; }
  return mww_bn_reestimate_commit(c);
}

int mww_get_ema_bn_state(mww_ctx* c, float* h, int64_t n, int* valid) {
  if (!c || !c->ema) return fail(MWW_ERR_INVALID, "no weight average installed: call mww_set_weight_ema first");
  if (n != c->S) return fail(MWW_ERR_INVALID, "BN state size mismatch");
  if (valid) *valid = c->ema_bn_valid ? 1 : 0;
  return h ? copy_out(c, h, c->ema_bn_valid ? c->ema_bn : c->bn_state, (size_t)n * sizeof(float)) : MWW_OK;
}
int mww_set_ema_bn_state(mww_ctx* c, const float* h, int64_t n) {
  if (!c || !c->ema) return fail(MWW_ERR_INVALID, "no weight average installed: call mww_set_weight_ema first");
  if (!h || n != c->S) return fail(MWW_ERR_INVALID, "BN state size mismatch");
  HIPCHK(hipSetDevice(c->device));
  if (!c->ema_bn) MWW_TRY(dev_alloc(&c->ema_bn, (size_t)c->S));
  MWW_TRY(copy_in(c, c->ema_bn, h, (size_t)n * sizeof(float)));
  c->bnre_batches = -1;
  c->ema_bn_valid = true;
  return MWW_OK;
}

int mww_evaluate_windows(mww_ctx* c, const mww_window* windows, const float* labels, int64_t n, int batch) {
  if (!c || !windows || !labels || n < 0 || batch <= 0 || batch > c->max_batch) return fail(MWW_ERR_INVALID, "bad evaluation arguments");
  std::vector<float> ones((size_t)batch, 1.0f);
  int rc = MWW_OK;
  for (int64_t s = 0; s < n && !rc; s += batch) {
    const int b = (int)std::min<int64_t>(batch, n - s);
    rc = mww_set_targets(c, labels + s, ones.data(), b);
    if (!rc) rc = mww_assemble_batch(c, windows + s, nullptr, b, 0, 0);
    if (!rc) rc = mww_forward(c, b, 0, 1);
    c->bn_eval_ready = c->model->eval_fold_cached();
    c->shadow_held = ema_serves(c) ? c->ema : c->params;
  }
  c->bn_eval_ready = false;
  c->shadow_held = nullptr;
  return rc;
}

int mww_read_outputs(mww_ctx* c, int B, float* probs, float* logits, float* loss) {
  if (!c || B <= 0 || B > c->max_batch) return fail(MWW_ERR_INVALID, "bad batch size");
  if (probs) HIPCHK(hipMemcpyAsync(probs, c->prob, (size_t)B * sizeof(float), hipMemcpyDeviceToHost, c->stream));
  if (logits) HIPCHK(hipMemcpyAsync(logits, c->z, (size_t)B * sizeof(float), hipMemcpyDeviceToHost, c->stream));
  std::vector<float> lp;
  if (loss) {
    lp.resize(B);
    HIPCHK(hipMemcpyAsync(lp.data(), c->loss_part, (size_t)B * sizeof(float), hipMemcpyDeviceToHost, c->stream));
  }
  HIPCHK(hipStreamSynchronize(c->stream));
  if (loss) {
    double s = 0.0;
    for (int i = 0; i < B; ++i) s += lp[i];
    *loss = (float)s;
  }
  return MWW_OK;
}

int mww_metrics_read(mww_ctx* c, mww_metrics* out) {
  if (!c || !out) return fail(MWW_ERR_INVALID, "null argument");
  static_assert(sizeof(mww_metrics) == sizeof(MetricState), "metric layouts must match");
  return copy_out(c, out, c->metrics, sizeof(MetricState));
}
int mww_metrics_reset(mww_ctx* c) {
  if (!c) return fail(MWW_ERR_INVALID, "null context");
  HIPCHK(hipMemsetAsync(c->metrics, 0, sizeof(MetricState), c->stream));
  return MWW_OK;
}

void* mww_device_ptr(mww_ctx* c, int which) {
  if (!c) return nullptr;
  switch (which) {
    case MWW_BUF_PARAMS: return c->params;
    case MWW_BUF_GRADS: return c->grads;
    case MWW_BUF_BN_STATE: return c->bn_state;
    case MWW_BUF_X: return c->x;
    case MWW_HANDLE_STREAM: return c->stream;
    default: return nullptr;
  }
}

int64_t mww_debug_read(mww_ctx* c, const char* name, int B, float* host, int64_t cap) {
  if (!c || !name || !host || B <= 0 || B > c->max_batch) return fail(MWW_ERR_INVALID, "bad debug_read arguments");
  DebugTensor t;
  const int found = c->model->debug_tensor(c, name, B, &t);
  if (found < 0) return found;
  if (!found) {
    if (!strcmp(name, "dz")) { t.src = c->dz; t.n = B; }
    else if (!strcmp(name, "x")) { t.src = c->x; t.n = (int64_t)B * c->frames * MWW_FEATURE_BINS; }
    else return fail(MWW_ERR_INVALID, std::string("unknown tensor name: ") + name);
  }
  const int64_t n = t.n;
  if (n > cap) return fail(MWW_ERR_INVALID, "host buffer too small");
  if (t.planes > 1) {
    const int64_t rows = n / t.cout;
    std::vector<float> tmp((size_t)rows * t.pc);
    for (int pl = 0; pl < t.planes; ++pl) {
      int rcp = copy_out(c, tmp.data(), t.src + (size_t)pl * t.pstride, tmp.size() * sizeof(float));
      if (rcp) return rcp;
      for (int64_t r = 0; r < rows; ++r)
        for (int cc = 0; cc < t.pc; ++cc) host[r * t.cout + pl * t.pc + cc] = tmp[(size_t)r * t.pc + cc];
    }
    return n;
  }
  if (t.bf16) {
    std::vector<unsigned short> half((size_t)n);
    int rch = copy_out(c, half.data(), t.src, (size_t)n * sizeof(unsigned short));
    if (rch) return rch;
    for (int64_t i = 0; i < n; ++i) {
      const unsigned bits = (unsigned)half[(size_t)i] << 16;
      memcpy(host + i, &bits, 4);
    }
    return n;
  }
  int rc = copy_out(c, host, t.src, (size_t)n * sizeof(float));
  return rc ? rc : n;
}

namespace {
const OptionRow kOptions[] = {
    {"graphs", OPT_CORE, 1, 0, 0, nullptr},
    {"profile", OPT_CORE, 1, 0, 0, nullptr},
    {"side_stream", OPT_CORE, 1, 0, 0, nullptr},
    {"bn_inline", OPT_CORE, 1, 0, 0, nullptr},
    {"tail_roles", OPT_CORE, 1, 0, 0, nullptr},
    {"bce_from_logits", OPT_CORE, 1, 0, 0, nullptr},
    {"grad_buckets", OPT_CORE, 1, 2, 0, "grad_buckets must be 1 or 2"},
    {"fused_input", OPT_CORE, 1, 0, 0, nullptr},
    {"assemble_split", OPT_CORE, 1, 8, 0, "assemble_split out of range"},
    {"grid_head", OPT_CORE, 1, 4, 1, "grid_head out of range"},
    {"weight_qat", OPT_CORE, 0, 1, 0, "weight_qat must be 0 or 1"},
    {"ema_forward", OPT_CORE, 0, 1, 0, "ema_forward must be 0 or 1"},
    {"ablate", OPT_BLOCK, 1, 0, 0, nullptr},
    {"pointwise_bf16", OPT_BLOCK, 1, 0, 0, nullptr},
    {"storage_bf16", OPT_BLOCK, 1, 0, 0, nullptr},
    {"bwd_wide", OPT_BLOCK, 1, 0, 0, nullptr},
    {"conv1_x6", OPT_BLOCK, 1, 0, 0, nullptr},
    {"conv1_x6_fwd", OPT_BLOCK, 1, 0, 0, nullptr},
    {"bwd_first_wide", OPT_BLOCK, 1, 0, 0, nullptr},
    {"dp_commit_late", OPT_BLOCK, -1, 1, 0, "dp_commit_late must be -1 (per-family defaults), 0 or 1"},
    {"grid_fwd", OPT_BLOCK, 1, 4, 1, "grid_fwd out of range"},
    {"grid_bwd", OPT_BLOCK, 1, 2, 1, "grid_bwd out of range"},
    {"graph_role_split", OPT_GRAPH, 1, 0, 0, nullptr},
    {"graph_static_shapes", OPT_GRAPH, 1, 0, 0, nullptr},
    {"graph_planar", OPT_GRAPH, 1, 0, 0, nullptr},
    {"graph_fwd_wg_per_cu", OPT_GRAPH, 1, 8, 0, "graph_fwd_wg_per_cu must be 1..8"},
    {"graph_bwd_wg_per_cu", OPT_GRAPH, 1, 8, 0, "graph_bwd_wg_per_cu must be 1..8"},
    {"graph_frame_chunks", OPT_GRAPH, 0, 4, 0, "graph_frame_chunks must be 0..4"},
    {"graph_dgrad_share", OPT_GRAPH, 10, 90, 0, "graph_dgrad_share must be 10..90"},
    {"profile_split", OPT_GRAPH, 1, 0, 0, nullptr},
    {"grid_graph", OPT_GRAPH, 0, 4, 1, "grid_graph out of range"},
    {"dropout_seed", OPT_GRAPH, 1, 0, 0, nullptr},
};

int set_core_option(mww_ctx* c, const std::string& name, int64_t v) {
  const std::pair<const char*, bool*> flags[] = {{"graphs", &c->use_graphs}, {"profile", &c->profile}, {"side_stream", &c->use_side}, {"bn_inline", &c->bn_inline},
                                                 {"tail_roles", &c->tail_roles}, {"fused_input", &c->fused_input}};
  const std::pair<const char*, int*> ints[] = {{"grad_buckets", &c->grad_buckets}, {"assemble_split", &c->asm_split}, {"grid_head", &c->grid_head}};
  for (auto& f : flags) if (name == f.first) *f.second = v != 0;
  for (auto& f : ints) if (name == f.first) *f.second = (int)v;
  if (name == "bce_from_logits") c->bce_clipped = v == 0;
  if (name == "weight_qat") {
    if (v && !c->shadow) return fail(MWW_ERR_INVALID, "weight_qat needs a channel map: call mww_set_weight_qat first");
    if (c->weight_qat != (v != 0)) invalidate_ema_bn(c);
    c->weight_qat = v != 0;
  }
  if (name == "ema_forward") {
    if (v && !c->ema) return fail(MWW_ERR_INVALID, "ema_forward needs the weight average: call mww_set_weight_ema first");
    c->ema_forward = v != 0;
  }
  if (name == "profile") {
    for (auto& e : c->prof) { (void)hipEventDestroy(e.a); (void)hipEventDestroy(e.b); }
    c->prof.clear();
  }
  return (name == "fused_input" && !v) ? materialise_x(c) : MWW_OK;
}
}

int mww_set_option(mww_ctx* c, const char* name, int64_t v) {
  if (!c || !name) return fail(MWW_ERR_INVALID, "null argument");
  const OptionRow* o = nullptr;
  for (const OptionRow& r : kOptions)
    if (!strcmp(name, r.name)) o = &r;
  if (!o) return fail(MWW_ERR_INVALID, std::string("unknown option: ") + name);
  if (o->lo <= o->hi && (v < o->lo || v > (o->hi_cu ? (int64_t)c->n_cu * o->hi : o->hi))) return fail(MWW_ERR_INVALID, o->range_error);
  MWW_TRY(o->owner == OPT_CORE ? set_core_option(c, name, v) : c->model->set_option(c, *o, v));
  drop_graphs(c);
  return MWW_OK;
}

int mww_profile_read(mww_ctx* c, char* names, int names_cap, float* ms, int cap) {
  if (!c) return fail(MWW_ERR_INVALID, "null context");
  HIPCHK(hipStreamSynchronize(c->stream));
  int n = 0, pos = 0;
  for (auto& e : c->prof) {
    if (n >= cap) break;
    float t = 0.f;
    (void)hipEventElapsedTime(&t, e.a, e.b);
    ms[n] = t;
    const int len = (int)e.name.size();
    if (names && pos + len + 1 < names_cap) {
      memcpy(names + pos, e.name.c_str(), len);
      names[pos + len] = '\n';
      pos += len + 1;
    }
    ++n;
  }
  if (names && names_cap > 0) names[pos < names_cap ? pos : names_cap - 1] = 0;
  for (auto& e : c->prof) { (void)hipEventDestroy(e.a); (void)hipEventDestroy(e.b); }
  c->prof.clear();
  return n;
}

}

namespace mww {
int ctx_borrow(mww_ctx* c, int* device, hipStream_t* stream, void** stores, int* dtypes, int64_t* elems, int* n_cu) {
  if (!c) return fail(MWW_ERR_INVALID, "no context");
  *device = c->device;
  *stream = c->stream;
  *n_cu = c->n_cu;
  for (int i = 0; i < MWW_MAX_STORES; ++i) { stores[i] = c->store[i]; dtypes[i] = c->store_dtype[i]; elems[i] = c->store_elems[i]; }
  return MWW_OK;
}
int set_error(int code, const char* msg) { return fail(code, msg); }
}
```

Measured before the change: 3.546 million.

## Prefetch next backward layer's first tiles during kernel drain to warm cache

During the final tile of each backward block kernel, the kernel issues buffer loads for the first input and activation tiles that the next backward kernel will read. The loaded values are then retired with empty asm so the compiler keeps the loads. The intent is to warm L2/MALL so the successor kernel's first tile does not stall on DRAM. The head kernel gets the same hook, but it is off by default. This adds extra loads and register pressure in the tail and may add traffic or change occupancy. Profiling stamps are also extended.

```diff
diff --git a/microwakeword_amd/csrc/block_engine.hip b/microwakeword_amd/csrc/block_engine.hip
--- a/microwakeword_amd/csrc/block_engine.hip
+++ b/microwakeword_amd/csrc/block_engine.hip
@@ -25,6 +25,15 @@
 #endif
 #ifndef MWW_DP_COMMIT_LATE_FIRST_DEFAULT
 #define MWW_DP_COMMIT_LATE_FIRST_DEFAULT 1
+#endif
+#ifndef MWW_DRAIN_PREFETCH_HEAD_DEFAULT
+#define MWW_DRAIN_PREFETCH_HEAD_DEFAULT 0
+#endif
+#ifndef MWW_DRAIN_PREFETCH_BLOCK_DEFAULT
+#define MWW_DRAIN_PREFETCH_BLOCK_DEFAULT 1
+#endif
+#ifndef MWW_DRAIN_PREFETCH_FIRST_DEFAULT
+#define MWW_DRAIN_PREFETCH_FIRST_DEFAULT 1
 #endif
 
 namespace mww {
@@ -51,6 +60,7 @@
   bool bwd_first_wide = MWW_BWD_FIRST_WIDE_DEFAULT != 0;
   bool bwd_wide = MWW_BWD_WIDE_DEFAULT != 0;
   int dp_commit_late = -1;
+  int drain_prefetch = -1;
   bool pw_bf16 = false;
   bool st_bf16 = false;
   int ablate = 0;
@@ -89,6 +99,7 @@
   int launch_fwd_block(mww_ctx* c, int cin, int cout, int k, const FwdBlockArgs& a, int grid);
   int launch_bwd_block(mww_ctx* c, int cin, int cout, int k, bool last, const BwdBlockArgs& a, int grid);
   int fwd_block_grid(const mww_ctx* c, const Layer& l, int B);
+  DrainPrefetch drain_prefetch_for(int succ, int B, int gbwd) const;
   void block_segments(int gbwd, int b0, int b1, GradReduceArgs* ga);
 };
 
@@ -145,6 +156,28 @@
 }
 
 namespace {
+
+DrainPrefetch BlockModel::drain_prefetch_for(int succ, int B, int gbwd) const {
+  DrainPrefetch pf;
+  memset(&pf, 0, sizeof(pf));
+  const int nb = d.n_blocks;
+  if (succ < 0) return pf;
+  const int dflt = succ == nb - 1 ? MWW_DRAIN_PREFETCH_HEAD_DEFAULT : (succ == 0 ? MWW_DRAIN_PREFETCH_FIRST_DEFAULT : MWW_DRAIN_PREFETCH_BLOCK_DEFAULT);
+  if (!(drain_prefetch < 0 ? dflt != 0 : drain_prefetch != 0) || pw_bf16 || st_bf16) return pf;
+  const Layer& l = L[succ];
+  const float* in = succ == 0 ? a0 : L[succ - 1].p;
+  const int rows[2] = {tile_rows(TT + l.k - 1, l.tin, 0), succ == nb - 1 ? 0 : tile_rows(TT, l.tout, 0)};
+  const float* base[2] = {in, l.p};
+  const int width[2] = {l.cin, l.cout}, len[2] = {l.tin, l.tout};
+  for (int i = 0; i < 2; ++i) {
+    if (rows[i] <= 0) continue;
+    pf.base[i] = base[i];
+    pf.stride[i] = len[i] * width[i] * 4;
+    pf.bytes[i] = rows[i] * width[i] * 4;
+  }
+  pf.nwin = std::min(B, gbwd);
+  return pf;
+}
 
 int BlockModel::fwd_block_grid(const mww_ctx* c, const Layer& l, int B) {
   const int per_cu = l.cin > 48 ? 2 : (l.k > 13 ? 3 : 4);
@@ -221,7 +254,8 @@
   if (inl) c->fpar ^= 1;
   const bool tail_late = loss && inl && c->tail_roles;
   const StatAcc hgacc = tail_late ? bwd_rows(c, ll) : StatAcc{nullptr, nullptr};
-  int rc = enqueue_block_head(c, B, ll, ll.tout, ll.cout, st_bf16, hfold, hgacc, loss, metrics);
+  const DrainPrefetch hpf = drain_prefetch_for(training && loss ? nb - 1 : -1, B, std::min(B, grid_bwd));
+  int rc = enqueue_block_head(c, B, ll, ll.tout, ll.cout, st_bf16, hfold, hgacc, loss, metrics, &hpf);
   if (rc) return rc;
   c->tail_src = DenseSource{ll.p, bn_slot(ll, BN_SCALE), bn_slot(ll, BN_SHIFT), nullptr, nullptr, nullptr, nullptr, 0, 0, st_bf16 ? 1 : 0};
   if (tail_late) {
@@ -355,6 +389,7 @@
       a.phase_clk = phase_clk + (size_t)(2 * i + 1) * 2048 * kClkSlots;
       a.gacc = inl ? bwd_rows(c, pl) : StatAcc{nullptr, nullptr};
       a.gfold = gf;
+      a.pf = drain_prefetch_for(i - 1, B, gbwd);
       lp.begin("bwd_block", i);
       int rc = launch_bwd_block(c, l.cin, l.cout, l.k, last, a, gbwd);
       lp.end();
@@ -463,7 +498,7 @@
   }
   const std::pair<const char*, bool BlockModel::*> flags[] = {{"bwd_wide", &BlockModel::bwd_wide}, {"conv1_x6", &BlockModel::conv1_x6},
                                                               {"conv1_x6_fwd", &BlockModel::conv1_x6_fwd}, {"bwd_first_wide", &BlockModel::bwd_first_wide}};
-  const std::pair<const char*, int BlockModel::*> ints[] = {{"ablate", &BlockModel::ablate}, {"dp_commit_late", &BlockModel::dp_commit_late},
+  const std::pair<const char*, int BlockModel::*> ints[] = {{"ablate", &BlockModel::ablate}, {"dp_commit_late", &BlockModel::dp_commit_late}, {"drain_prefetch", &BlockModel::drain_prefetch},
                                                             {"grid_fwd", &BlockModel::grid_fwd}, {"grid_bwd", &BlockModel::grid_bwd}};
   for (auto& f : flags) if (name == f.first) this->*f.second = v != 0;
   for (auto& f : ints) if (name == f.first) this->*f.second = (int)v;
diff --git a/microwakeword_amd/csrc/bwd_first_body.inc b/microwakeword_amd/csrc/bwd_first_body.inc
--- a/microwakeword_amd/csrc/bwd_first_body.inc
+++ b/microwakeword_amd/csrc/bwd_first_body.inc
@@ -46,13 +46,13 @@
     const int s = live ? it / ntiles : nsamp - 1, b = blockIdx.x + s * gridDim.x, t0 = (it % ntiles) * TT;
     const int nrx = live ? ((tailmode ? Ta : min(TT, Ta - t0)) - 1) * S + K1 : 0;
     xs.issue(a.x, a.xg, sXg, s, b, a.T, t0 * S, nrx, tid);
-    const BufRsrc ra = tile_rsrc(a.a0 + ((size_t)b * Ta + t0) * CIN, live ? min(RA, Ta - t0) * QI * 16 : 0);
+    const BufRsrc ra = tile_rsrc(a.a0 + ((size_t)b * Ta + t0) * CIN, live ? tile_rows(RA, Ta, t0) * QI * 16 : 0);
 #pragma unroll
     for (int j = 0; j < NA; ++j) pre_a[j] = tile_load4<MWW_AUX_LD_A0>(ra, (tid + j * kThreads) * 16);
   };
   auto issue_b = [&](int it, bool live) {
     const int b = blockIdx.x + (it / ntiles) * gridDim.x, t0 = (it % ntiles) * TT;
-    const int nvk = live ? max(0, min(TT, a.Tout - t0)) * (COUT / 4) : 0;
+    const int nvk = live ? max(0, tile_rows(TT, a.Tout, t0)) * (COUT / 4) : 0;
     const size_t koff = ((size_t)b * a.Tout + t0) * COUT;
     dps.issue(elem_ptr<SB>(a.pk, koff), elem_ptr<SB>(a.gk, koff), nvk, tid);
   };
@@ -137,6 +137,7 @@
   MWW_PC_START(MWW_ABLATE(a, 16) && tid == 0);
   for (int it = 0; it < nitems; ++it) {
     rotate_priority(it, 2);
+    MWW_PC_AT_ONCE(5, it + 1 == nitems);
     const int t0 = (it % ntiles) * TT;
     const int nrows_new = max(0, min(TT, a.Tout - t0));
     const int rows_da = min(TT, Ta - t0);
@@ -151,6 +152,7 @@
       }
     }
     MWW_PC_MARK(0);
+    MWW_PC_AT_ONCE(4, true);
     if constexpr (!LATE) dps.commit(sDP, sKp, 0.f, nrows_new * (COUT / 4), tid);
     carry_du<K, CPI>(sDU, t0 == 0, tid);
     if constexpr (LATE) issue_a(it + 1, it + 1 < nitems);
diff --git a/microwakeword_amd/csrc/common.hip.h b/microwakeword_amd/csrc/common.hip.h
--- a/microwakeword_amd/csrc/common.hip.h
+++ b/microwakeword_amd/csrc/common.hip.h
@@ -225,6 +225,29 @@
 }
 
 constexpr int kOobOffset = 0x40000000;
+
+__host__ __device__ constexpr int tile_rows(int span, int T, int t0) { return span < T - t0 ? span : T - t0; }
+
+struct DrainPrefetch {
+  const void* base[2];
+  int stride[2];
+  int bytes[2];
+  int nwin;
+};
+__device__ __forceinline__ BufRsrc drain_prefetch_rsrc(const DrainPrefetch& pf, int which, int b) {
+  const bool on = pf.base[which] != nullptr && b < pf.nwin;
+  return tile_rsrc(static_cast<const char*>(pf.base[which]) + (size_t)(on ? b : 0) * pf.stride[which], on ? pf.bytes[which] : 0);
+}
+template <int NTH, int N>
+__device__ __forceinline__ void drain_prefetch_issue(BufRsrc r, int tid, float4 (&dst)[N]) {
+#pragma unroll
+  for (int j = 0; j < N; ++j) dst[j] = tile_load4<0>(r, (tid + j * NTH) * 16);
+}
+template <int N>
+__device__ __forceinline__ void drain_prefetch_retire(const float4 (&dst)[N]) {
+#pragma unroll
+  for (int j = 0; j < N; ++j) asm volatile("" ::"v"(dst[j].x), "v"(dst[j].y), "v"(dst[j].z), "v"(dst[j].w));
+}
 
 __device__ __forceinline__ void lds_reads_first() {
   __builtin_amdgcn_sched_group_barrier(0x100, 64, 0);
@@ -287,19 +310,25 @@
 #define MWW_PC_MARK(i) pc.mark(i)
 #define MWW_PC_DUMP(p) do { if (p) pc.dump(p); } while (0)
 #define MWW_PC_AT(i) pc.at(i)
+#define MWW_PC_AT_ONCE(i, cond) pc.at_once(i, cond)
 #else
 #define MWW_PC_AT(i) ((void)0)
+#define MWW_PC_AT_ONCE(i, cond) ((void)0)
 #define MWW_PC_DECL
 #define MWW_PC_START(en) ((void)0)
 #define MWW_PC_MARK(i) ((void)0)
 #define MWW_PC_DUMP(p) ((void)0)
 #endif
 constexpr int kClkPhases = 9;
-constexpr int kClkSlots = kClkPhases + 4;
+constexpr int kClkStamps = 6;
+constexpr int kClkSlots = kClkPhases + kClkStamps;
 struct PhaseClock {
-  unsigned long long last = 0, acc[kClkPhases] = {0, 0, 0, 0, 0, 0, 0, 0, 0}, stamp[4] = {0, 0, 0, 0};
+  unsigned long long last = 0, acc[kClkPhases] = {0, 0, 0, 0, 0, 0, 0, 0, 0}, stamp[kClkStamps] = {0, 0, 0, 0, 0, 0};
   bool on = false;
   __device__ __forceinline__ void at(int i) { stamp[i] = __builtin_amdgcn_s_memtime(); }
+  __device__ __forceinline__ void at_once(int i, bool cond) {
+    if (cond && stamp[i] == 0) stamp[i] = __builtin_amdgcn_s_memtime();
+  }
   __device__ __forceinline__ void start(bool enable) {
     on = enable;
     if (on) last = __builtin_amdgcn_s_memtime();
@@ -314,7 +343,7 @@
   __device__ __forceinline__ void dump(unsigned long long* dst) const {
     if (on) {
       for (int i = 0; i < kClkPhases; ++i) dst[i] = acc[i];
-      for (int i = 0; i < 4; ++i) dst[kClkPhases + i] = stamp[i];
+      for (int i = 0; i < kClkStamps; ++i) dst[kClkPhases + i] = stamp[i];
     }
   }
 };
diff --git a/microwakeword_amd/csrc/engine.hip.h b/microwakeword_amd/csrc/engine.hip.h
--- a/microwakeword_amd/csrc/engine.hip.h
+++ b/microwakeword_amd/csrc/engine.hip.h
@@ -261,7 +261,8 @@
 int enqueue_bnre_collect(mww_ctx* c, std::vector<BnreRow>& rows);
 int enqueue_grad_assembly(mww_ctx* c, int B, GradReduceArgs& ga, bool fuse_adam, int64_t lo = 0, int64_t hi = -1, bool last_range = true);
 int head_frame_limit(int ch);
-int enqueue_block_head(mww_ctx* c, int B, const Tensor& last, int T, int C, bool bf16, const BnFoldArgs& fold, const StatAcc& gacc, bool loss, bool metrics);
+int enqueue_block_head(mww_ctx* c, int B, const Tensor& last, int T, int C, bool bf16, const BnFoldArgs& fold, const StatAcc& gacc, bool loss, bool metrics,
+                       const DrainPrefetch* pf = nullptr);
 int enqueue_head_tail(mww_ctx* c, int B, const BnBwdFinalizeArgs& fin);
 
 bool shape_supported(const mww_mixednet_desc& d, std::string* why, bool bf16 = false);
diff --git a/microwakeword_amd/csrc/kernels_bwd.hip.h b/microwakeword_amd/csrc/kernels_bwd.hip.h
--- a/microwakeword_amd/csrc/kernels_bwd.hip.h
+++ b/microwakeword_amd/csrc/kernels_bwd.hip.h
@@ -31,6 +31,7 @@
   unsigned long long* phase_clk;
   StatAcc gacc;
   BnGradFoldArgs gfold;
+  DrainPrefetch pf;
 };
 
 template <int COUT, bool LAST, bool SB = false>
diff --git a/microwakeword_amd/csrc/kernels_bwdw.hip.h b/microwakeword_amd/csrc/kernels_bwdw.hip.h
--- a/microwakeword_amd/csrc/kernels_bwdw.hip.h
+++ b/microwakeword_amd/csrc/kernels_bwdw.hip.h
@@ -33,6 +33,15 @@
     for (int j = 0; j < N; ++j) {
       pk[j] = tile_load4s<SB, MWW_AUX_LD_PK>(rp, tid + j * NTH);
       gg[j] = tile_load4s<SG, MWW_AUX_LD_GK>(rg, tid + j * NTH);
+    }
+  }
+
+  __device__ __forceinline__ void issue_prefetch(BufRsrc rp, int tid) {
+    const BufRsrc none = tile_rsrc(nullptr, 0);
+#pragma unroll
+    for (int j = 0; j < N; ++j) {
+      pk[j] = tile_load4<0>(rp, (tid + j * NTH) * 16);
+      gg[j] = tile_load4<0>(none, (tid + j * NTH) * 16);
     }
   }
 
@@ -310,18 +319,29 @@
   float pre_dz = 0.f;
   auto issue_a = [&](int it, bool live) {
     const int b = blockIdx.x + (it / ntiles) * gridDim.x, t0 = (it % ntiles) * TT;
-    const int nvp = live ? min(RA, a.Tin - t0) * Q : 0;
+    const int nvp = live ? tile_rows(RA, a.Tin, t0) * Q : 0;
     const BufRsrc src = tile_rsrc(elem_ptr<SB>(a.in, ((size_t)b * a.Tin + t0) * C), nvp * 4 * elem_bytes(SB));
 #pragma unroll
     for (int j = 0; j < NP; ++j) pre_p[j] = tile_load4s<SB, MWW_AUX_LD_BP>(src, tid + j * NTH);
   };
   auto issue_b = [&](int it, bool live) {
     const int b = blockIdx.x + (it / ntiles) * gridDim.x, t0 = (it % ntiles) * TT;
-    const int nvk = live ? max(0, min(TT, a.Tout - t0)) * Q : 0;
+    const int nvk = live ? tile_rows(TT, a.Tout, t0) * Q : 0;
     const size_t koff = ((size_t)b * a.Tout + t0) * C;
     dps.issue(elem_ptr<SB>(a.pk, koff), LAST ? a.wd + (size_t)t0 * C : elem_ptr<SB>(a.gk, koff), nvk, tid);
     if (LAST) pre_dz = tile_load1(tile_rsrc(a.dz, live ? a.B * 4 : 0), b * 4);
   };
+  constexpr bool PF = !BF && !SB;
+  auto prefetch_a = [&]() { drain_prefetch_issue<NTH>(drain_prefetch_rsrc(a.pf, 0, blockIdx.x), tid, pre_p); };
+  auto prefetch_b = [&]() {
+    if constexpr (LATE) {
+      drain_prefetch_issue<NTH>(drain_prefetch_rsrc(a.pf, 1, blockIdx.x), tid, dps.pk);
+    } else {
+      dps.issue_prefetch(drain_prefetch_rsrc(a.pf, 1, blockIdx.x), tid);
+      if (LAST) pre_dz = tile_load1(tile_rsrc(a.dz, 0), 0);
+    }
+  };
+  const int pf_tile = a.pf.nwin > 0 ? nitems - 1 : -1;
   stagger_start<MWW_STAGGER_BWD>();
   if (nitems > 0) {
     issue_a(0, true);
@@ -395,6 +415,7 @@
 #ifndef MWW_WIDE_NOPRIO
     rotate_priority(it, 2);
 #endif
+    MWW_PC_AT_ONCE(5, it + 1 == nitems);
     const int b = blockIdx.x + (it / ntiles) * gridDim.x, t0 = (it % ntiles) * TT;
     const int nrows_new = max(0, min(TT, a.Tout - t0));
     const int rows_da = min(TT, a.Tin - t0);
@@ -413,9 +434,14 @@
       }
     }
     MWW_PC_MARK(0);
+    MWW_PC_AT_ONCE(4, true);
     if constexpr (!LATE) dps.commit(sDP, sKp, pre_dz, nrows_new * Q, tid);
     for (int i = tid; i < (K - 1) * P; i += NTH) sDU[i] = (t0 == 0) ? 0.f : sDU[TT * P + i];
-    if constexpr (LATE) issue_a(it + 1, it + 1 < nitems);
+    if constexpr (LATE) {
+      issue_a(it + 1, it + 1 < nitems);
+      if constexpr (PF)
+        if (it == pf_tile) prefetch_a();
+    }
     MWW_PC_MARK(LATE ? 0 : 8);
     __syncthreads();
     MWW_PC_MARK(1);
@@ -423,6 +449,11 @@
       if (it + 1 < nitems) {
         issue_a(it + 1, true);
         issue_b(it + 1, true);
+      } else if constexpr (PF) {
+        if (it == pf_tile) {
+          prefetch_a();
+          prefetch_b();
+        }
       }
     }
     if (dw_active) {
@@ -445,6 +476,8 @@
     if constexpr (LATE) {
       dps.commit(sDP, sKp, pre_dz, nrows_new * Q, tid);
       issue_b(it + 1, it + 1 < nitems);
+      if constexpr (PF)
+        if (it == pf_tile) prefetch_b();
       MWW_PC_MARK(8);
     }
     __syncthreads();
@@ -557,6 +590,10 @@
 #pragma unroll
     for (int j = 0; j < NCH; ++j) v += scratch[j * 2 * C + tid];
     publish_stat(a.gacc, a.gstat_part + (size_t)blockIdx.x * 2 * C, 2 * C, tid, v);
+  }
+  if constexpr (PF) {
+    drain_prefetch_retire(pre_p);
+    drain_prefetch_retire(dps.pk);
   }
   MWW_PC_AT(3);
   MWW_PC_DUMP(a.phase_clk ? a.phase_clk + (size_t)blockIdx.x * kClkSlots : nullptr);
@@ -629,13 +666,13 @@
     const int s = live ? it / ntiles : nsamp - 1, b = blockIdx.x + s * gridDim.x, t0 = (it % ntiles) * TT;
     const int nrx = live ? ((tailmode ? Ta : min(TT, Ta - t0)) - 1) * S + K1 : 0;
     xs.issue(a.x, a.xg, sXg, s, b, a.T, t0 * S, nrx, tid);
-    const BufRsrc ra = tile_rsrc(a.a0 + ((size_t)b * Ta + t0) * CIN, live ? min(RA, Ta - t0) * QI * 16 : 0);
+    const BufRsrc ra = tile_rsrc(a.a0 + ((size_t)b * Ta + t0) * CIN, live ? tile_rows(RA, Ta, t0) * QI * 16 : 0);
 #pragma unroll
     for (int j = 0; j < NA; ++j) pre_a[j] = tile_load4<MWW_AUX_LD_A0>(ra, (tid + j * NTH) * 16);
   };
   auto issue_b = [&](int it, bool live) {
     const int b = blockIdx.x + (it / ntiles) * gridDim.x, t0 = (it % ntiles) * TT;
-    const int nvk = live ? max(0, min(TT, a.Tout - t0)) * QO : 0;
+    const int nvk = live ? max(0, tile_rows(TT, a.Tout, t0)) * QO : 0;
     const size_t koff = ((size_t)b * a.Tout + t0) * COUT;
     dps.issue(elem_ptr<SB>(a.pk, koff), elem_ptr<SB>(a.gk, koff), nvk, tid);
   };
diff --git a/microwakeword_amd/csrc/kernels_head.hip.h b/microwakeword_amd/csrc/kernels_head.hip.h
--- a/microwakeword_amd/csrc/kernels_head.hip.h
+++ b/microwakeword_amd/csrc/kernels_head.hip.h
@@ -32,6 +32,7 @@
   int training;
   BnFoldArgs fold;
   StatAcc gacc;
+  DrainPrefetch pf;
 };
 
 template <int C, int JMAX, bool SB = false>
@@ -138,6 +139,11 @@
     y_cur = y_nxt;
     w_cur = w_nxt;
   }
+  constexpr int NPF = 4;
+  float4 pfr[NPF];
+  const bool pf_on = !SB && a.pf.nwin > 0;
+  if (pf_on)
+    for (int b = blockIdx.x; b < a.pf.nwin; b += gridDim.x) drain_prefetch_issue<kThreads>(drain_prefetch_rsrc(a.pf, 0, b), tid, pfr);
   if (a.training & kHeadTraining) {
     if (active) {
       *reinterpret_cast<float4*>(sStat + (rg * 2 + 0) * C + q * 4) = g1;
@@ -150,6 +156,7 @@
       publish_stat(a.gacc, a.gstat_part + (size_t)blockIdx.x * 2 * C, 2 * C, tid, v);
     }
   }
+  if (pf_on) drain_prefetch_retire(pfr);
 }
 
 struct MetricsArgs {
diff --git a/microwakeword_amd/csrc/mww_lib.hip b/microwakeword_amd/csrc/mww_lib.hip
--- a/microwakeword_amd/csrc/mww_lib.hip
+++ b/microwakeword_amd/csrc/mww_lib.hip
@@ -55,11 +55,14 @@
 
 int head_frame_limit(int ch) { return (kThreads / (ch / 4)) * kHeadMaxRows; }
 
-int enqueue_block_head(mww_ctx* c, int B, const Tensor& last, int T, int C, bool bf16, const BnFoldArgs& fold, const StatAcc& gacc, bool loss, bool metrics) {
+int enqueue_block_head(mww_ctx* c, int B, const Tensor& last, int T, int C, bool bf16, const BnFoldArgs& fold, const StatAcc& gacc, bool loss, bool metrics,
+                       const DrainPrefetch* pf) {
   float* const bn = last.bn;
-  const HeadArgs h{last.p, bn + (size_t)BN_SCALE * C, bn + (size_t)BN_SHIFT * C, bn + (size_t)BN_MEAN * C, bn + (size_t)BN_RSTD * C,
+  HeadArgs h{last.p, bn + (size_t)BN_SCALE * C, bn + (size_t)BN_SHIFT * C, bn + (size_t)BN_MEAN * C, bn + (size_t)BN_RSTD * C,
                    fwd_params(c) + c->o_dense_w, fwd_params(c) + c->o_dense_b, (loss || metrics) ? c->y_cur : nullptr, c->sw_cur, c->z, c->prob, c->dz,
                    c->loss_part, last.gstat_part, B, T, 1.0f / (float)B, (loss ? kHeadTraining : 0) | (c->bce_clipped ? kHeadClippedLoss : 0), fold, gacc};
+  memset(&h.pf, 0, sizeof(h.pf));
+  if (pf && loss && !bf16) h.pf = *pf;
   const int q = C / 4, nrg = kThreads / q;
   Launcher lp{c};
   lp.begin("head");
@@ -1510,6 +1513,7 @@
     {"conv1_x6_fwd", OPT_BLOCK, 1, 0, 0, nullptr},
     {"bwd_first_wide", OPT_BLOCK, 1, 0, 0, nullptr},
     {"dp_commit_late", OPT_BLOCK, -1, 1, 0, "dp_commit_late must be -1 (per-family defaults), 0 or 1"},
+    {"drain_prefetch", OPT_BLOCK, -1, 1, 0, "drain_prefetch must be -1 (per-pair defaults), 0 or 1"},
     {"grid_fwd", OPT_BLOCK, 1, 4, 1, "grid_fwd out of range"},
     {"grid_bwd", OPT_BLOCK, 1, 2, 1, "grid_bwd out of range"},
     {"graph_role_split", OPT_GRAPH, 1, 0, 0, nullptr},
```

After: 3.561 million (median of 6 runs). About the same (+0.4%).
